# kiliant/zklaim

Hardware: AMD Instinct MI355X
Metric: Groth16 proofs/sec (zklaim gadget, alt_bn128) + G1 MSM GB/s vs HBM roofline (higher is better)
Workload: dtype u32 limbs, Montgomery (254-bit Fq/Fr: 9 x 29-bit in the accumulation, reduction and NTT kernels, 8 x 32-bit elsewhere)

## Files before the change

include/zkg.h:

```cpp
#ifndef ZKG_H
#define ZKG_H

#include <stddef.h>
#include <stdint.h>

#ifdef __cplusplus
extern "C" {
#endif

#define ZKG_OK 0
#define ZKG_ERROR 1
#define ZKG_UNSATISFIED 2
#define ZKG_PROOF_BYTES 134

typedef struct zkg_r1cs {
    uint32_t num_variables;
    uint32_t num_inputs;
    uint32_t num_constraints;
    uint32_t reserved;
    const uint32_t *a_rowptr, *a_col; const uint64_t *a_val;
    const uint32_t *b_rowptr, *b_col; const uint64_t *b_val;
    const uint32_t *c_rowptr, *c_col; const uint64_t *c_val;
} zkg_r1cs;

typedef struct zkg_pk {
    zkg_r1cs cs;
    uint32_t log_m;
    uint32_t domain_size;
    const uint64_t *alpha_g1, *beta_g1, *delta_g1;
    const uint64_t *beta_g2, *delta_g2;
    const uint64_t *A_query;
    const uint64_t *B_g1;
    const uint64_t *B_g2;
    const uint64_t *H_query;
    const uint64_t *L_query;
} zkg_pk;

typedef struct zkg_crs zkg_crs;

int  zkg_init(int device);
void zkg_shutdown(void);
const char *zkg_last_error(void);
int  zkg_device_info(char *name, size_t name_len, int *compute_units);

int zkg_ntt(uint64_t *a, unsigned logN, int inverse, int coset);
int zkg_ntt_dev(void *d_a, unsigned logN, int inverse, int coset, void *stream);

int zkg_evaluation_domain_size(size_t min_size, size_t *m, int *is_step);
int zkg_ntt_domain(uint64_t *a, size_t m, int inverse, int coset);
int zkg_ntt_domain_dev(void *d_a, size_t m, int inverse, int coset, void *stream);

typedef struct zkg_domain zkg_domain;
zkg_domain *zkg_domain_new(size_t m);
void   zkg_domain_free(zkg_domain *d);
size_t zkg_domain_size(const zkg_domain *d);
size_t zkg_domain_batch_max(const zkg_domain *d);
void   zkg_domain_set_batch_max(zkg_domain *d, size_t k);
int zkg_domain_ntt_async(zkg_domain *d, void *d_a, size_t stride , size_t count,
                         int inverse, int coset, void *stream);
int zkg_domain_lagrange_async(zkg_domain *d, const uint64_t t[4], void *d_u, void *d_z, void *stream);
void zkg_domain_stats(size_t out[3]);

typedef struct zkg_qap zkg_qap;
zkg_qap *zkg_qap_new(const zkg_r1cs *cs);
void     zkg_qap_free(zkg_qap *q);
size_t   zkg_qap_domain_size(const zkg_qap *q);
uint32_t zkg_qap_num_variables(const zkg_qap *q);
size_t   zkg_qap_batch_max(const zkg_qap *q);
void     zkg_qap_set_batch_max(zkg_qap *q, size_t k);
int      zkg_qap_witness_h_async(zkg_qap *q, const void *d_witnesses, size_t stride , size_t count,
                                 void *d_h, size_t h_stride , uint32_t *d_unsat ,
                                 void *stream);
void     zkg_qap_stats(size_t out[3]);
int      zkg_qap_instance_async(zkg_qap *q, const uint64_t t[4] , void *d_abc ,
                                size_t stride , void *d_z , void *stream);
void     zkg_qap_set_column_segment(zkg_qap *q, size_t k);
void     zkg_qap_instance_stats(size_t out[2]);

int zkg_msm_g1(const uint64_t *bases, const uint64_t *scalars, size_t n, uint64_t out_jac[12]);
int zkg_msm_g2(const uint64_t *bases, const uint64_t *scalars, size_t n, uint64_t out_jac[24]);
#define ZKG_SCALARS_MONT 1
#define ZKG_SCALARS_MOSTLY_BITS 2
int zkg_msm_g1_dev(const void *d_bases, const void *d_scalars, size_t n, int scalars_mont,
                   uint64_t out_jac[12], void *stream);
int zkg_msm_g2_dev(const void *d_bases, const void *d_scalars, size_t n, int scalars_mont,
                   uint64_t out_jac[24], void *stream);
int zkg_msm_g1_host_scalars(const void *d_bases, const uint64_t *scalars, size_t n, int scalars_mont, uint64_t out_jac[12], void *stream);
typedef struct zkg_msm_bases zkg_msm_bases;
zkg_msm_bases *zkg_msm_g1_bases_upload(const void *d_bases, size_t n);
int zkg_msm_g1_resident(zkg_msm_bases *bases, const void *d_scalars, size_t n, int scalars_mont, uint64_t out_jac[12], void *stream);
void zkg_msm_g1_bases_free(zkg_msm_bases *bases);
int zkg_msm_g1_resident_async(zkg_msm_bases *bases, const void *d_scalars, size_t n, size_t stride , size_t count,
                              int scalars_mont, void *d_out_jac , void *stream);
size_t zkg_msm_g1_resident_batch_max(const zkg_msm_bases *bases);
void zkg_msm_resident_async_stats(size_t out[3]);
int zkg_msm_combine_gpu(const uint64_t *records_jac, size_t cpw, int slots , int chunk_log, size_t vectors, uint64_t *out_jac);
typedef struct zkg_msm_g2_bases zkg_msm_g2_bases;
zkg_msm_g2_bases *zkg_msm_g2_bases_upload(const void *d_bases , size_t n);
void   zkg_msm_g2_bases_free(zkg_msm_g2_bases *bases);
int    zkg_msm_g2_resident(zkg_msm_g2_bases *bases, const void *d_scalars, size_t n, int scalars_mont, uint64_t out_jac[24], void *stream);
int    zkg_msm_g2_resident_async(zkg_msm_g2_bases *bases, const void *d_scalars, size_t n, size_t stride, size_t count,
                                 int scalars_mont, void *d_out_jac , void *stream);
size_t zkg_msm_g2_resident_batch_max(const zkg_msm_g2_bases *bases);
int    zkg_msm_combine_g2_gpu(const uint64_t *records_jac, size_t cpw, int chunk_log, size_t vectors, uint64_t *out_jac);
int zkg_msm_g1_windows_dev(const void *d_bases, const void *d_scalars, size_t n, int scalars_mont,
                           unsigned first_window, unsigned window_stride, uint64_t out_jac[12], void *stream);
int zkg_g1_sum(const uint64_t *points_jac, size_t count, uint64_t out_jac[12]);
int zkg_g2_sum(const uint64_t *points_jac, size_t count, uint64_t out_jac[24]);

typedef struct zkg_msm_shards zkg_msm_shards;
int zkg_init_multi(const int *devices, int ndev);
zkg_msm_shards *zkg_msm_g1_shards_upload(const uint64_t *bases, size_t n, const int *devices, int ndev);
void zkg_msm_g1_shards_free(zkg_msm_shards *shards);
size_t zkg_msm_g1_shards_count(const zkg_msm_shards *shards, size_t *points);
int zkg_msm_g1_multi(const zkg_msm_shards *shards, const uint64_t *scalars, uint64_t out_jac[12], uint64_t *partials_jac);
unsigned zkg_multi_rccl_calls(void);

int zkg_g1_fixed_base_dev(const uint64_t base[8], const void *d_scalars, size_t n, void *d_out_affine, void *stream);
int zkg_g2_fixed_base_dev(const uint64_t base[16], const void *d_scalars, size_t n, void *d_out_affine, void *stream);

zkg_crs *zkg_crs_upload(const zkg_pk *pk);
zkg_crs *zkg_crs_upload_blob(const void *pk_blob, size_t len);
int zkg_pk_blob_inspect(const void *pk_blob, size_t len, uint64_t out[8]);
void     zkg_crs_free(zkg_crs *crs);
int zkg_crs_shard_h(zkg_crs *crs, const int *devices, int ndev);
uint32_t zkg_crs_num_variables(const zkg_crs *crs);

int zkg_groth16_prove(const zkg_crs *crs, const uint64_t *witness, const uint64_t r[4],
                      const uint64_t s[4], int check_satisfied, uint8_t *proof_out, size_t *proof_len);
int zkg_groth16_prove_sparse(const zkg_crs *crs, const uint8_t *tags, const uint32_t *full_index, const uint64_t *full_values, size_t count,
                             const uint64_t r[4], const uint64_t s[4], int check_satisfied, uint8_t *proof_out, size_t *proof_len);
typedef struct zkg_prove_item {
    const uint64_t *witness;
    const uint8_t  *tags; const uint32_t *full_index; const uint64_t *full_values; size_t count;
    const uint64_t *r, *s;
} zkg_prove_item;
int zkg_groth16_prove_batch(const zkg_crs *crs, const zkg_prove_item *items, size_t count, int check_satisfied,
                            uint8_t *proofs_out , int *status );
void zkg_prove_batch_stats(size_t out[3]);
size_t zkg_prove_batch_chunk(const zkg_crs *crs);
int zkg_groth16_prove_dev(const zkg_crs *crs, const void *d_witness, const uint64_t r[4], const uint64_t s[4], int check_satisfied,
                          uint8_t *proof_out, size_t *proof_len, void *stream);
int zkg_groth16_prove_batch_dev(const zkg_crs *crs, const void *d_witnesses, size_t stride , size_t count,
                                const uint64_t *rs , int check_satisfied,
                                uint8_t *proofs_out , int *status , void *stream);
void zkg_prove_dev_stats(size_t out[2]);
struct zklaim_ctx;
int zkg_groth16_prove_batch_zklaim(const zkg_crs *crs, const struct zklaim_ctx *const *ctxs, size_t count, const uint64_t *rs ,
                                   int check_satisfied, uint8_t *proofs_out , int *status );
void zkg_zklaim_witness_stats(size_t out[2]);
size_t zkg_zklaim_witness_size(size_t payloads, size_t *cap_listed);
int zkg_zklaim_witness_gpu(const struct zklaim_ctx *const *ctxs, size_t count, uint8_t *tags_out , uint32_t *index_out,
                           uint64_t *values_out, size_t cap_listed , size_t *listed_counts);
int zkg_zklaim_witness_mirror(const struct zklaim_ctx *ctx, uint8_t *tags_out , uint32_t *index_out, uint64_t *values_out, size_t cap_listed,
                              size_t *listed_count);
int zkg_groth16_prove_zklaim(const zkg_crs *crs, const struct zklaim_ctx *ctx, const uint64_t r[4], const uint64_t s[4],
                             int check_satisfied, uint8_t *proof_out, size_t *proof_len);
void zkg_prove_zklaim_stats(size_t out[2]);
int zkg_zklaim_witness_gpu_parallel(const struct zklaim_ctx *const *ctxs, size_t count, uint8_t *tags_out , uint32_t *index_out,
                                    uint64_t *values_out, size_t cap_listed , size_t *listed_counts);
int zkg_zklaim_witness_mirror_parallel(const struct zklaim_ctx *ctx, uint8_t *tags_out , uint32_t *index_out, uint64_t *values_out,
                                       size_t cap_listed, size_t *listed_count);
int zkg_qap_witness_h(const zkg_crs *crs, const uint64_t *witness, uint64_t *h_out);
int zkg_prove_stage_ms(const zkg_crs *crs, float ms[8]);
int zkg_prover_peak_in_flight(int reset);

struct zklaim_ctx;
typedef struct zkg_circuit zkg_circuit;
#define ZKG_CIRCUIT_WITH_WITNESS 1
#define ZKG_CIRCUIT_REFERENCE_QUIRK 2
zkg_circuit *zkg_zklaim_circuit_new(const struct zklaim_ctx *ctx, int flags);
zkg_circuit *zkg_zklaim_witness_new(const struct zklaim_ctx *ctx);
uint32_t zkg_circuit_num_variables(const zkg_circuit *c);
void zkg_circuit_free(zkg_circuit *c);
int zkg_circuit_r1cs(const zkg_circuit *c, zkg_r1cs *out);
const uint64_t *zkg_circuit_witness(const zkg_circuit *c);
int zkg_circuit_sparse_witness(const zkg_circuit *c, const uint8_t **tags, const uint32_t **full_index, const uint64_t **full_values, size_t *count);
int zkg_circuit_is_satisfied(const zkg_circuit *c);
long zkg_circuit_first_unsatisfied(const zkg_circuit *c);
size_t zkg_zklaim_input_map(const struct zklaim_ctx *ctx, uint64_t *out, size_t cap_elems);

typedef struct zkg_keypair zkg_keypair;
zkg_keypair *zkg_groth16_setup(const zkg_r1cs *cs, const uint64_t *trapdoor);
zkg_keypair *zkg_groth16_setup_dev(const zkg_r1cs *cs, const uint64_t *trapdoor );
void zkg_keypair_free(zkg_keypair *kp);
const zkg_pk *zkg_keypair_pk(const zkg_keypair *kp);
int zkg_keypair_swapped(const zkg_keypair *kp);
size_t zkg_keypair_pk_blob(const zkg_keypair *kp, uint8_t *out, size_t cap);
size_t zkg_keypair_vk_blob(const zkg_keypair *kp, uint8_t *out, size_t cap);
int zkg_groth16_verify(const uint8_t *vk_blob, size_t vk_len, const uint64_t *primary_input, size_t n_inputs,
                       const uint8_t *proof, size_t proof_len);
int zkg_pairing_probe(const uint64_t a[4], const uint64_t b[4], uint8_t out[384]);
typedef struct zkg_verify_item {
    const uint8_t  *vk_blob;       size_t vk_len;
    const uint64_t *primary_input; size_t n_inputs;
    const uint8_t  *proof;         size_t proof_len;
} zkg_verify_item;
int zkg_groth16_verify_batch(const zkg_verify_item *items, size_t count, uint8_t *verdicts);
void zkg_verify_batch_stats(size_t out[3]);
int zkg_pairing_product(const uint64_t *g1_affine, const uint64_t *g2_affine, size_t n, uint8_t out[384]);
int  zkg_groth16_verify_each(const zkg_verify_item *items, size_t count, uint8_t *verdicts);
void zkg_verify_each_stats(size_t out[3]);
void zkg_verify_each_set_chunk(size_t positions);
int  zkg_pairing_each(const uint64_t *g1_affine, const uint64_t *g2_affine, size_t items, size_t pairs, uint8_t *out);
int  zkg_final_exp(const uint8_t *in, size_t n, int where, uint8_t *out);
int zkg_pairing_selfcheck(const uint32_t *e, int nlimbs);

int libsnark_trusted_setup(struct zklaim_ctx *ctx);
int libsnark_prove(struct zklaim_ctx *ctx);
int libsnark_verify(struct zklaim_ctx *ctx);
void zkg_compat_reset(void);
int zkg_zklaim_prove_batch(struct zklaim_ctx *const *ctxs, size_t count, int *rc);
int zkg_zklaim_verify_batch(struct zklaim_ctx *const *ctxs, size_t count, int *rc);
void zkg_zklaim_verify_batch_stats(size_t out[4]);
int zkg_proof_decode_gpu(const uint8_t *proofs, size_t count, uint64_t *A, uint64_t *B, uint64_t *C, uint8_t *ok);
int zkg_zklaim_input_sums_gpu(const struct zklaim_ctx *const *ctxs, size_t count, const uint32_t *weights, const uint8_t *mask,
                              size_t lo, size_t hi, uint64_t *sums_out, size_t cap_elems, size_t *n_elems);
size_t zkg_zklaim_input_map_mirror(const struct zklaim_ctx *ctx, uint64_t *out, size_t cap_elems);
int  zkg_zklaim_verify_each(struct zklaim_ctx *const *ctxs, size_t count, int *rc);
void zkg_zklaim_verify_each_stats(size_t out[4]);
int zkg_zklaim_ic_each(const uint64_t *ic0, const uint64_t *ic, const struct zklaim_ctx *const *ctxs, size_t count, int where, uint64_t *out);

int zkg_point_decompress(const uint8_t *records, size_t stride, size_t offset, size_t n, int g2, int where, uint64_t *out, uint32_t *flag);
int zkg_point_compress(const uint64_t *g1, const uint64_t *g2, const uint32_t *idx, size_t npoints, size_t n, int rec, int where, uint8_t *out,
                       uint8_t guard[16]);

int zkg_field_op(int field, int op, const uint64_t *a, const uint64_t *b, size_t n, uint64_t *out);

int zkg_fr29_op(int op, const uint32_t *in, size_t n, uint32_t *out);

int zkg_fq29_op(int op, const uint32_t *in, size_t n, uint32_t *out);
int zkg_fq29_op_chain(int op, int chain, const uint32_t *in, size_t n, uint32_t *out);

int zkg_fq12_op(int op, const uint32_t *a, const uint32_t *b, size_t n, int where, uint32_t *out);

int zkg_g1_add_quad29(const uint64_t *a_jac, const uint64_t *b_jac, size_t n, int chain, uint64_t *out_jac);
int zkg_g1_add_pair29(const uint64_t *a_jac, const uint64_t *b_jac, size_t n, int chain, uint64_t *out_jac);

int zkg_curve_op(int group, int op, const uint32_t *a, const uint32_t *b, const uint32_t *k, size_t n, int chain, uint32_t *out);

// ... 8 lines not shown
```

zklaim_amd/__init__.py:

```python
from .api import (ZkgError, device_info, evaluation_domain_size, fixed_base_g1_dev, fixed_base_g2_dev, g1_sum, g2_sum, init, lib, msm_g1, msm_g1_dev, msm_g1_windows_dev,
                  msm_g2, msm_g2_dev, ntt, ntt_dev, shutdown, timing_dominant_ms, timing_reset, Crs, PK, R1CS, make_r1cs, make_pk,
                  DECLARED_SYMBOLS, ZklaimCircuit, ZklaimCtx, make_ctx, zklaim_input_map, OPS, Keypair, groth16_verify, groth16_verify_batch, verify_batch_stats, groth16_prove_batch, prove_batch_stats, groth16_prove_batch_dev, prove_dev_stats, groth16_prove_batch_zklaim, zklaim_witness_stats, zklaim_witness_size, zklaim_witness_mirror, zklaim_witness_gpu, zklaim_witness_mirror_parallel, zklaim_witness_gpu_parallel, prove_zklaim_stats, pairing_product, pairing_probe, pairing_selfcheck,
                  libsnark_trusted_setup, libsnark_prove, libsnark_verify, zklaim_prove_batch, zklaim_verify_batch, zklaim_verify_batch_stats, proof_decode_gpu, zklaim_input_sums_gpu, zklaim_input_map_mirror, ctx_blob, COMPAT_SYMBOLS, field_op, fr29_op, FR29_OPS, fq29_op, FQ29_OPS, g1_add_quad29, g1_add_pair29, curve_op, CURVE_OPS, OK, ERROR, UNSATISFIED, init_multi, MsmShards, pk_blob_inspect, ResidentBases, msm_g1_host_scalars, msm_resident_async_stats, msm_combine_gpu, ResidentBasesG2, msm_combine_g2_gpu,
                  groth16_verify_each, verify_each_stats, verify_each_set_chunk, pairing_each, final_exp, fq12_op, FQ12_OPS,
                  point_decompress, point_compress, zklaim_verify_each, zklaim_verify_each_stats, zklaim_ic_each,
                  Domain, domain_stats, Qap, qap_stats, qap_instance_stats)
```

zklaim_amd/api.py:

```python
import ctypes as C
import os
import sys

import numpy as np

_HERE = os.path.dirname(os.path.abspath(__file__))
_SO = os.path.join(_HERE, "libzkg.so")

DECLARED_SYMBOLS = [
    "zkg_init", "zkg_shutdown", "zkg_last_error", "zkg_device_info", "zkg_ntt", "zkg_ntt_dev", "zkg_evaluation_domain_size", "zkg_ntt_domain", "zkg_ntt_domain_dev", "zkg_msm_g1", "zkg_msm_g2",
    "zkg_msm_g1_dev", "zkg_msm_g2_dev", "zkg_msm_g1_windows_dev", "zkg_g1_sum", "zkg_g2_sum", "zkg_g1_fixed_base_dev", "zkg_g2_fixed_base_dev",
    "zkg_groth16_prove_batch_zklaim", "zkg_zklaim_witness_stats", "zkg_zklaim_witness_size", "zkg_zklaim_witness_gpu", "zkg_zklaim_witness_mirror",
    "zkg_crs_upload", "zkg_crs_upload_blob", "zkg_pk_blob_inspect", "zkg_crs_free", "zkg_crs_num_variables", "zkg_groth16_prove", "zkg_groth16_prove_sparse", "zkg_circuit_sparse_witness", "zkg_qap_witness_h", "zkg_prove_stage_ms", "zkg_timing_reset",
    "zkg_timing_dominant_ms", "zkg_zklaim_circuit_new", "zkg_zklaim_witness_new", "zkg_circuit_num_variables", "zkg_circuit_free", "zkg_circuit_r1cs", "zkg_circuit_witness",
    "zkg_circuit_is_satisfied", "zkg_circuit_first_unsatisfied", "zkg_zklaim_input_map", "zkg_groth16_setup", "zkg_keypair_free",
    "zkg_keypair_pk", "zkg_keypair_swapped", "zkg_keypair_pk_blob", "zkg_keypair_vk_blob", "zkg_groth16_verify", "zkg_pairing_probe", "zkg_pairing_selfcheck",
    "zkg_compat_reset", "zkg_field_op", "zkg_init_multi", "zkg_msm_g1_shards_upload", "zkg_msm_g1_shards_free", "zkg_msm_g1_shards_count",
    "zkg_msm_g1_multi", "zkg_g1_add_quad29", "zkg_crs_shard_h", "zkg_msm_g1_bases_upload", "zkg_msm_g1_resident", "zkg_msm_g1_bases_free",
    "zkg_prover_peak_in_flight", "zkg_msm_g1_host_scalars", "zkg_multi_rccl_calls", "zkg_g1_add_pair29",
    "zkg_groth16_verify_batch", "zkg_pairing_product", "zkg_verify_batch_stats",
    "zkg_groth16_prove_batch", "zkg_prove_batch_stats", "zkg_prove_batch_chunk", "zkg_zklaim_prove_batch",
    "zkg_groth16_prove_zklaim", "zkg_prove_zklaim_stats", "zkg_zklaim_witness_gpu_parallel", "zkg_zklaim_witness_mirror_parallel",
    "zkg_fr29_op", "zkg_fq29_op", "zkg_fq29_op_chain",
    "zkg_zklaim_verify_batch", "zkg_zklaim_verify_batch_stats", "zkg_proof_decode_gpu", "zkg_zklaim_input_sums_gpu", "zkg_zklaim_input_map_mirror",
    "zkg_groth16_prove_dev", "zkg_groth16_prove_batch_dev", "zkg_prove_dev_stats",
    "zkg_msm_g1_resident_async", "zkg_msm_g1_resident_batch_max", "zkg_msm_resident_async_stats", "zkg_msm_combine_gpu",
    "zkg_groth16_verify_each", "zkg_verify_each_stats", "zkg_verify_each_set_chunk", "zkg_pairing_each", "zkg_final_exp",
    "zkg_fq12_op", "zkg_point_decompress", "zkg_point_compress",
    "zkg_zklaim_verify_each", "zkg_zklaim_verify_each_stats", "zkg_zklaim_ic_each",
    "zkg_curve_op",
    "zkg_domain_new", "zkg_domain_free", "zkg_domain_size", "zkg_domain_batch_max", "zkg_domain_set_batch_max", "zkg_domain_ntt_async",
    "zkg_domain_lagrange_async", "zkg_domain_stats",
    "zkg_msm_g2_bases_upload", "zkg_msm_g2_bases_free", "zkg_msm_g2_resident", "zkg_msm_g2_resident_async", "zkg_msm_g2_resident_batch_max",
    "zkg_msm_combine_g2_gpu",
    "zkg_qap_new", "zkg_qap_free", "zkg_qap_domain_size", "zkg_qap_num_variables", "zkg_qap_batch_max", "zkg_qap_set_batch_max",
    "zkg_qap_witness_h_async", "zkg_qap_stats",
    "zkg_qap_instance_async", "zkg_qap_set_column_segment", "zkg_qap_instance_stats", "zkg_groth16_setup_dev",
]
COMPAT_SYMBOLS = ["libsnark_trusted_setup", "libsnark_prove", "libsnark_verify"]


OK, ERROR, UNSATISFIED = 0, 1, 2


class ZkgError(RuntimeError):
    pass


class R1CS(C.Structure):
    _fields_ = [("num_variables", C.c_uint32), ("num_inputs", C.c_uint32), ("num_constraints", C.c_uint32), ("reserved", C.c_uint32)] + \
        [(f"{m}_{f}", C.c_void_p) for m in "abc" for f in ("rowptr", "col", "val")]


class PK(C.Structure):
    _fields_ = [("cs", R1CS), ("log_m", C.c_uint32), ("domain_size", C.c_uint32)] + \
        [(k, C.c_void_p) for k in ("alpha_g1", "beta_g1", "delta_g1", "beta_g2", "delta_g2", "A_query", "B_g1", "B_g2", "H_query", "L_query")]


_lib = None


def lib():
    global _lib
    if _lib is None:
        if not os.path.exists(_SO):
            raise ZkgError(f"{_SO} is missing: build it with `python -m zklaim_amd.build` (hipcc, gfx950)")
        if "torch" not in sys.modules and not os.environ.get("ZKG_NO_TORCH"):
            try:
                import torch
            except Exception:
                pass
        _lib = C.CDLL(_SO)
        _lib.zkg_last_error.restype = C.c_char_p
        _lib.zkg_timing_dominant_ms.restype = C.c_float
        _lib.zkg_crs_upload.restype = C.c_void_p
        _lib.zkg_crs_upload.argtypes = [C.c_void_p]
        _lib.zkg_crs_upload_blob.restype = C.c_void_p
        _lib.zkg_crs_upload_blob.argtypes = [C.c_void_p, C.c_size_t]
        _lib.zkg_crs_free.argtypes = [C.c_void_p]
    return _lib


def _check(rc, what):
    if rc != 0:
        raise ZkgError(f"{what} failed (rc={rc}): {lib().zkg_last_error().decode()}")


def _p(a):
    return None if a is None else a.ctypes.data_as(C.c_void_p)


def _u64(a):
    return np.ascontiguousarray(a, dtype=np.uint64)


def _vp(x):
    return C.c_void_p(int(x) if x else 0)


_initialised = False


def init(device=0):
    global _initialised
    _check(lib().zkg_init(int(device)), "zkg_init")
    _initialised = True


def shutdown():
    global _initialised
    if _initialised:
        lib().zkg_shutdown()
    _initialised = False


def device_info():
    name = C.create_string_buffer(128); cus = C.c_int(0)
    _check(lib().zkg_device_info(name, C.c_size_t(128), C.byref(cus)), "zkg_device_info")
    return name.value.decode(), cus.value


def field_op(field, op, a, b=None):
    a = _u64(a); limbs = 8 if field == 2 else 4
    out = np.zeros_like(a)
    bb = None if b is None else _u64(b)
    _check(lib().zkg_field_op(int(field), int(op), _p(a), _p(bb), C.c_size_t(a.size // limbs), _p(out)), "zkg_field_op")
    return out


FR29_OPS = {"mul": (0, 2, 1), "mul2": (1, 4, 2), "norm": (2, 1, 1), "add_norm": (3, 2, 1), "sub_norm": (4, 2, 1), "add_lazy": (5, 2, 1), "sub_lazy": (6, 2, 1),
            "slice": (7, 1, 1), "unslice_reduce": (8, 1, 1), "r4": (9, 7, 4), "r4_stage0": (10, 7, 4), "r4_norm_stores": (11, 7, 4),
            "r4_stage0_norm_stores": (12, 7, 4), "r2_tail": (13, 3, 2), "r2_tail_stage0": (14, 3, 2)}


def fr29_op(name, x):
    op, k, m = FR29_OPS[name]
    x = np.ascontiguousarray(x, dtype=np.uint32)
    if x.ndim != 3 or x.shape[1:] != (k, 9):
        raise ZkgError(f"fr29_op {name}: input must be (n, {k}, 9), got {x.shape}")
    out = np.zeros((x.shape[0], m, 9), np.uint32)
    _check(lib().zkg_fr29_op(int(op), _p(x), C.c_size_t(x.shape[0]), _p(out)), "zkg_fr29_op")
    return out


FQ29_OPS = {"mul": (0, 2, 1), "mul2": (1, 4, 2), "sqr": (2, 1, 1), "sqr2": (3, 2, 2), "norm": (4, 1, 1), "add": (5, 2, 1), "dbl": (6, 1, 1),
            "sub_S2_1": (7, 2, 1), "sub_S4_1": (8, 2, 1), "sub_S6_1": (9, 2, 1), "sub_S4_3": (10, 2, 1), "neg_S2_1": (11, 1, 1), "is_zero": (12, 1, 1),
            "unpack": (13, 1, 1), "to29": (14, 1, 1), "from29": (15, 1, 1), "rec64": (16, 3, 3), "bucket29": (17, 5, 4), "inverse": (18, 1, 1),
            "madd": (19, 7, 5), "add_lane": (20, 8, 4), "add_pair": (21, 8, 4), "add_quad": (22, 8, 4)}


def fq29_op(name, x, chain=0):
    op, k, m = FQ29_OPS[name]
    x = np.ascontiguousarray(x, dtype=np.uint32)
    if x.ndim != 3 or x.shape[1:] != (k, 9):
        raise ZkgError(f"fq29_op {name}: input must be (n, {k}, 9), got {x.shape}")
    out = np.zeros((x.shape[0], m, 9), np.uint32)
    _check(lib().zkg_fq29_op_chain(int(op), int(chain), _p(x), C.c_size_t(x.shape[0]), _p(out)), "zkg_fq29_op")
    return out


def g1_add_quad29(a_jac, b_jac, chain=0):
    a = _u64(a_jac); b = _u64(b_jac); out = np.zeros_like(a)
    _check(lib().zkg_g1_add_quad29(_p(a), _p(b), C.c_size_t(a.size // 12), int(chain), _p(out)), "zkg_g1_add_quad29")
    return out.reshape(-1, 12)


def g1_add_pair29(a_jac, b_jac, chain=0):
    a = _u64(a_jac); b = _u64(b_jac); out = np.zeros_like(a)
    _check(lib().zkg_g1_add_pair29(_p(a), _p(b), C.c_size_t(a.size // 12), int(chain), _p(out)), "zkg_g1_add_pair29")
    return out.reshape(-1, 12)


CURVE_OPS = {"madd": 0, "add": 1, "add_quad": 2, "dbl": 3, "dbl_affine": 4, "to_affine": 5, "mul": 6}


def curve_op(group, name, a, b=None, k=None, chain=0):
    op = CURVE_OPS[name]; w = 16 if group else 8
    a = np.ascontiguousarray(a, dtype=np.uint32)
    need_a = 2 if name == "dbl_affine" else 4
    if a.ndim != 3 or a.shape[1:] != (need_a, w):
        raise ZkgError(f"curve_op {name}: a must be (n, {need_a}, {w}), got {a.shape}")
    n = a.shape[0]
    if name in ("madd", "add", "add_quad"):
        need_b = 2 if name == "madd" else 4
        b = np.ascontiguousarray(b, dtype=np.uint32)
        if b.shape != (n, need_b, w):
            raise ZkgError(f"curve_op {name}: b must be ({n}, {need_b}, {w}), got {b.shape}")
    else:
        b = None
    if name == "mul":
# ... 66 lines not shown
        t = _u64(t).reshape(4)
        _check(lib().zkg_domain_lagrange_async(C.c_void_p(self._h), _p(t), _vp(d_u_ptr), _vp(d_z_ptr), _vp(stream)), "zkg_domain_lagrange_async")

    def batch_max(self):
        return int(lib().zkg_domain_batch_max(C.c_void_p(self._h)))

    def set_batch_max(self, k):
        lib().zkg_domain_set_batch_max(C.c_void_p(self._h), C.c_size_t(k))

    def size(self):
        return int(lib().zkg_domain_size(C.c_void_p(self._h)))

    def free(self):
        if self._h:
            lib().zkg_domain_free(C.c_void_p(self._h)); self._h = None


def domain_stats():
    out = (C.c_size_t * 3)()
    lib().zkg_domain_stats(out)
    return tuple(int(v) for v in out)


class Qap:

    def __init__(self, cs):
        L = lib()
        L.zkg_qap_new.restype = C.c_void_p
        L.zkg_qap_new.argtypes = [C.c_void_p]
        L.zkg_qap_free.argtypes = [C.c_void_p]
        for name in ("zkg_qap_domain_size", "zkg_qap_batch_max"):
            getattr(L, name).restype = C.c_size_t
            getattr(L, name).argtypes = [C.c_void_p]
        L.zkg_qap_num_variables.restype = C.c_uint32
        L.zkg_qap_num_variables.argtypes = [C.c_void_p]
        L.zkg_qap_set_batch_max.argtypes = [C.c_void_p, C.c_size_t]
        L.zkg_qap_witness_h_async.argtypes = [C.c_void_p, C.c_void_p, C.c_size_t, C.c_size_t, C.c_void_p, C.c_size_t, C.c_void_p, C.c_void_p]
        L.zkg_qap_instance_async.argtypes = [C.c_void_p, C.c_void_p, C.c_void_p, C.c_size_t, C.c_void_p, C.c_void_p]
        L.zkg_qap_set_column_segment.argtypes = [C.c_void_p, C.c_size_t]
        self._h = L.zkg_qap_new(C.byref(cs))
        if not self._h:
            raise ZkgError("zkg_qap_new failed: " + L.zkg_last_error().decode())
        self.m, self.n = self.domain_size(), self.num_variables()

    def witness_h_async(self, d_w_ptr, count, stride, d_h_ptr, h_stride, d_unsat_ptr=0, stream=0):
        _check(lib().zkg_qap_witness_h_async(C.c_void_p(self._h), _vp(d_w_ptr), C.c_size_t(stride), C.c_size_t(count), _vp(d_h_ptr), C.c_size_t(h_stride),
                                             _vp(d_unsat_ptr), _vp(stream)), "zkg_qap_witness_h_async")

    def instance_async(self, t, d_abc_ptr, stride=None, d_z_ptr=0, stream=0):
        tt = None if t is None else _u64(t).reshape(-1)
        if tt is not None and tt.size != 4:
            raise ZkgError("zkg_qap_instance_async: t is 4 limbs")
        _check(lib().zkg_qap_instance_async(C.c_void_p(self._h), _p(tt), _vp(d_abc_ptr), C.c_size_t(self.n + 1 if stride is None else stride), _vp(d_z_ptr),
                                            _vp(stream)), "zkg_qap_instance_async")

    def set_column_segment(self, k):
        lib().zkg_qap_set_column_segment(C.c_void_p(self._h), C.c_size_t(k))

    def domain_size(self):
        return int(lib().zkg_qap_domain_size(C.c_void_p(self._h)))

    def num_variables(self):
        return int(lib().zkg_qap_num_variables(C.c_void_p(self._h)))

    def batch_max(self):
        return int(lib().zkg_qap_batch_max(C.c_void_p(self._h)))

    def set_batch_max(self, k):
        lib().zkg_qap_set_batch_max(C.c_void_p(self._h), C.c_size_t(k))

    def free(self):
        if self._h:
            lib().zkg_qap_free(C.c_void_p(self._h)); self._h = None


def qap_stats():
    out = (C.c_size_t * 3)()
    lib().zkg_qap_stats(out)
    return tuple(int(v) for v in out)


def qap_instance_stats():
    out = (C.c_size_t * 2)()
    lib().zkg_qap_instance_stats(out)
    return tuple(int(v) for v in out)


def msm_g1(bases, scalars):
    bases = _u64(bases); scalars = _u64(scalars); out = np.zeros(12, np.uint64)
    _check(lib().zkg_msm_g1(_p(bases), _p(scalars), C.c_size_t(scalars.size // 4), _p(out)), "zkg_msm_g1")
    return out


def msm_g2(bases, scalars):
    bases = _u64(bases); scalars = _u64(scalars); out = np.zeros(24, np.uint64)
    _check(lib().zkg_msm_g2(_p(bases), _p(scalars), C.c_size_t(scalars.size // 4), _p(out)), "zkg_msm_g2")
    return out


def init_multi(devices):
    global _initialised
    d = (C.c_int * len(devices))(*devices)
    _check(lib().zkg_init_multi(d, len(devices)), "zkg_init_multi")
    _initialised = True


class MsmShards:

    def __init__(self, bases, devices):
        bases = _u64(bases)
        L = lib()
        L.zkg_msm_g1_shards_upload.restype = C.c_void_p
        L.zkg_msm_g1_shards_upload.argtypes = [C.c_void_p, C.c_size_t, C.c_void_p, C.c_int]
        L.zkg_msm_g1_shards_free.argtypes = [C.c_void_p]
        L.zkg_msm_g1_multi.argtypes = [C.c_void_p, C.c_void_p, C.c_void_p, C.c_void_p]
        d = (C.c_int * len(devices))(*devices)
        self.n = bases.size // 8; self.ndev = len(devices)
        self._h = L.zkg_msm_g1_shards_upload(_p(bases), self.n, d, len(devices))
        if not self._h:
            raise ZkgError("zkg_msm_g1_shards_upload failed: " + L.zkg_last_error().decode())

    def msm(self, scalars, with_partials=False):
        scalars = _u64(scalars); out = np.zeros(12, np.uint64); parts = np.zeros((self.ndev, 12), np.uint64)
        assert scalars.size // 4 == self.n
        _check(lib().zkg_msm_g1_multi(C.c_void_p(self._h), _p(scalars), _p(out), _p(parts)), "zkg_msm_g1_multi")
        return (out, parts) if with_partials else out

    def free(self):
        if self._h:
            lib().zkg_msm_g1_shards_free(C.c_void_p(self._h)); self._h = None

    def __del__(self):
        try:
            self.free()
        except Exception:
            pass


SCALARS_MONT, SCALARS_MOSTLY_BITS = 1, 2


def msm_g1_dev(d_bases, d_scalars, n, scalars_mont=False, stream=0, mostly_bits=False):
    out = np.zeros(12, np.uint64)
    flags = (SCALARS_MONT if scalars_mont else 0) | (SCALARS_MOSTLY_BITS if mostly_bits else 0)
    _check(lib().zkg_msm_g1_dev(_vp(d_bases), _vp(d_scalars), C.c_size_t(n), flags, _p(out), _vp(stream)), "zkg_msm_g1_dev")
    return out


def msm_g1_host_scalars(d_bases, scalars_host_ptr, n, scalars_mont=False, stream=0):
    out = np.zeros(12, np.uint64)
    lib().zkg_msm_g1_host_scalars.argtypes = [C.c_void_p, C.c_void_p, C.c_size_t, C.c_int, C.c_void_p, C.c_void_p]
    _check(lib().zkg_msm_g1_host_scalars(_vp(d_bases), _vp(scalars_host_ptr), C.c_size_t(n), SCALARS_MONT if scalars_mont else 0, _p(out), _vp(stream)), "zkg_msm_g1_host_scalars")
    return out


class _ResidentBases:
    _PREFIX = None
    _LIMBS = 0

    def _fn(self, suffix, argtypes, restype=C.c_int):
        fn = getattr(lib(), self._PREFIX + suffix)
        fn.argtypes = argtypes; fn.restype = restype
        return fn

    def __init__(self, d_bases, n):
        self._h = self._fn("_bases_upload", [C.c_void_p, C.c_size_t], C.c_void_p)(_vp(d_bases), C.c_size_t(n))
        if not self._h:
            raise ZkgError(self._PREFIX + "_bases_upload failed: " + last_error())
        self.n = n

    def msm(self, d_scalars, scalars_mont=False, stream=0):
        out = np.zeros(self._LIMBS, np.uint64)
        fn = self._fn("_resident", [C.c_void_p, C.c_void_p, C.c_size_t, C.c_int, C.c_void_p, C.c_void_p])
        _check(fn(C.c_void_p(self._h), _vp(d_scalars), C.c_size_t(self.n), SCALARS_MONT if scalars_mont else 0, _p(out), _vp(stream)), self._PREFIX + "_resident")
        return out

    def msm_async(self, d_scalars_ptr, d_out_ptr, count=1, stride=None, scalars_mont=False, stream=0):
        fn = self._fn("_resident_async", [C.c_void_p, C.c_void_p, C.c_size_t, C.c_size_t, C.c_size_t, C.c_int, C.c_void_p, C.c_void_p])
        _check(fn(C.c_void_p(self._h), _vp(d_scalars_ptr), C.c_size_t(self.n), C.c_size_t(self.n if stride is None else stride),
                  C.c_size_t(count), SCALARS_MONT if scalars_mont else 0, _vp(d_out_ptr), _vp(stream)), self._PREFIX + "_resident_async")

    def batch_max(self):
        return int(self._fn("_resident_batch_max", [C.c_void_p], C.c_size_t)(C.c_void_p(self._h)))

    def free(self):
        if self._h:
            self._fn("_bases_free", [C.c_void_p], None)(C.c_void_p(self._h)); self._h = None


class ResidentBases(_ResidentBases):
    _PREFIX = "zkg_msm_g1"
    _LIMBS = 12


class ResidentBasesG2(_ResidentBases):
    _PREFIX = "zkg_msm_g2"
    _LIMBS = 24


def msm_resident_async_stats():
    out = (C.c_size_t * 3)()
    lib().zkg_msm_resident_async_stats(out)
    return tuple(int(v) for v in out)


def _msm_combine(name, limbs, records_jac, cpw, slots, chunk_log, vectors, slot_args):
    rec = _u64(records_jac)
    if rec.size != vectors * cpw * slots * limbs:
        raise ZkgError("%s: records_jac must hold vectors x cpw x %s points of %d limbs" % (name, "slots" if slot_args else slots, limbs))
    out = np.zeros((vectors, limbs), np.uint64)
    fn = getattr(lib(), "zkg_" + name)
    fn.argtypes = [C.c_void_p, C.c_size_t] + [C.c_int] * len(slot_args) + [C.c_int, C.c_size_t, C.c_void_p]
    _check(fn(_p(rec), C.c_size_t(cpw), *slot_args, int(chunk_log), C.c_size_t(vectors), _p(out)), "zkg_" + name)
    return out


def msm_combine_gpu(records_jac, cpw, slots, chunk_log, vectors=1):
    return _msm_combine("msm_combine_gpu", 12, records_jac, cpw, slots, chunk_log, vectors, [int(slots)])


def msm_combine_g2_gpu(records_jac, cpw, chunk_log, vectors=1):
    return _msm_combine("msm_combine_g2_gpu", 24, records_jac, cpw, 2, chunk_log, vectors, [])


def msm_g1_windows_dev(d_bases, d_scalars, n, first_window, window_stride, scalars_mont=False, stream=0):
    out = np.zeros(12, np.uint64)
    _check(lib().zkg_msm_g1_windows_dev(_vp(d_bases), _vp(d_scalars), C.c_size_t(n), int(scalars_mont), C.c_uint(first_window), C.c_uint(window_stride),
                                        _p(out), _vp(stream)), "zkg_msm_g1_windows_dev")
    return out


def msm_g2_dev(d_bases, d_scalars, n, scalars_mont=False, stream=0, mostly_bits=False):
    out = np.zeros(24, np.uint64)
    flags = (SCALARS_MONT if scalars_mont else 0) | (SCALARS_MOSTLY_BITS if mostly_bits else 0)
    _check(lib().zkg_msm_g2_dev(_vp(d_bases), _vp(d_scalars), C.c_size_t(n), flags, _p(out), _vp(stream)), "zkg_msm_g2_dev")
    return out


def g1_sum(points_jac):
    pts = _u64(points_jac); out = np.zeros(12, np.uint64)
    _check(lib().zkg_g1_sum(_p(pts), C.c_size_t(pts.size // 12), _p(out)), "zkg_g1_sum")
    return out


def g2_sum(points_jac):
    pts = _u64(points_jac); out = np.zeros(24, np.uint64)
    _check(lib().zkg_g2_sum(_p(pts), C.c_size_t(pts.size // 24), _p(out)), "zkg_g2_sum")
    return out


def fixed_base_g1_dev(base, d_scalars, n, d_out, stream=0):
    base = _u64(base)
    _check(lib().zkg_g1_fixed_base_dev(_p(base), _vp(d_scalars), C.c_size_t(n), _vp(d_out), _vp(stream)), "zkg_g1_fixed_base_dev")


def fixed_base_g2_dev(base, d_scalars, n, d_out, stream=0):
    base = _u64(base)
    _check(lib().zkg_g2_fixed_base_dev(_p(base), _vp(d_scalars), C.c_size_t(n), _vp(d_out), _vp(stream)), "zkg_g2_fixed_base_dev")


def timing_reset():
    lib().zkg_timing_reset()


def timing_dominant_ms():
    n = C.c_int(0)
    ms = lib().zkg_timing_dominant_ms(C.byref(n))
    return float(ms), n.value


def make_r1cs(n, l, A, B, Cm, keep):
    cs = R1CS()
    cs.num_variables, cs.num_inputs, cs.num_constraints = n, l, len(A[0]) - 1
    for name, (rp, col, val) in zip("abc", (A, B, Cm)):
        rp = np.ascontiguousarray(rp, np.uint32); col = np.ascontiguousarray(col, np.uint32); val = _u64(val)
        keep += [rp, col, val]
        setattr(cs, f"{name}_rowptr", rp.ctypes.data); setattr(cs, f"{name}_col", col.ctypes.data); setattr(cs, f"{name}_val", val.ctypes.data)
    return cs


def make_pk(cs, arrays, log_m, keep, domain_size=0):
    pk = PK(); pk.cs = cs; pk.log_m = log_m; pk.domain_size = domain_size
    for k in ("alpha_g1", "beta_g1", "delta_g1", "beta_g2", "delta_g2", "A_query", "B_g1", "B_g2", "H_query", "L_query"):
        a = _u64(arrays[k]); keep.append(a)
        setattr(pk, k, a.ctypes.data)
    return pk


class Crs:

    def __init__(self, pk=None, blob=None, m=None):
        if blob is not None:
            buf = (C.c_ubyte * len(blob)).from_buffer_copy(blob)
            self._h = lib().zkg_crs_upload_blob(C.cast(buf, C.c_void_p), C.c_size_t(len(blob)))
            self.m = m
        else:
            self._h = lib().zkg_crs_upload(C.byref(pk))
            self.m = pk.domain_size or (1 << pk.log_m)
        if not self._h:
            raise ZkgError("zkg_crs_upload failed: " + lib().zkg_last_error().decode())

    def prove(self, witness, r, s, check_satisfied=True):
        out = np.zeros(256, np.uint8); ln = C.c_size_t(0)
        rc = lib().zkg_groth16_prove(C.c_void_p(self._h), _p(_u64(witness)), _p(_u64(r)), _p(_u64(s)), int(check_satisfied), _p(out), C.byref(ln))
        if rc not in (OK, UNSATISFIED):
            _check(rc, "zkg_groth16_prove")
# ... 664 lines not shown
```

zklaim_amd/csrc/capi.hip:

```cpp
#include "common.hpp"
#include "fq29.hip.hpp"
#include "fr29.hip.hpp"
#include "../../include/zkg.h"
#include <atomic>
#include <condition_variable>
#include <cstring>
#include <memory>
#include <mutex>
#include <thread>
#include <dlfcn.h>
#include <rccl/rccl.h>

namespace zk {

static thread_local std::string t_error;
static std::string g_error;
static std::mutex g_err_mu;
void set_error(const std::string &msg) { t_error = msg; std::lock_guard<std::mutex> lk(g_err_mu); g_error = msg; }
bool hip_ok(hipError_t e, const char *what, const char *file, int line) {
    if (e == hipSuccess) return true;
    set_error(std::string(what) + ": " + hipGetErrorString(e) + " at " + file + ":" + std::to_string(line));
    return false;
}

// ... 583 lines not shown
        zkg_ntt_dev(buf.p, logN, inverse, coset, nullptr) == ZKG_OK &&
        hip_ok(hipDeviceSynchronize(), "sync", __FILE__, __LINE__) &&
        hip_ok(hipMemcpy(a, buf.p, bytes, hipMemcpyDeviceToHost), "D2H", __FILE__, __LINE__)) rc = ZKG_OK;
    buf.release();
    return rc;
}

int zkg_evaluation_domain_size(size_t min_size, size_t *m, int *is_step) {
    DomainShape sh;
    if (!evaluation_domain_shape(min_size, sh)) { set_error("zkg_evaluation_domain_size: no radix-2 or step domain for that size"); return ZKG_ERROR; }
    if (m) *m = sh.m;
    if (is_step) *is_step = sh.step ? 1 : 0;
    return ZKG_OK;
}
int zkg_ntt_domain_dev(void *d_a, size_t m, int inverse, int coset, void *stream) {
    REQUIRE_INIT();
    DomainShape sh;
    if (!domain_shape_of(m, sh)) { set_error("zkg_ntt_domain: m is neither 2^k nor 2^a + 2^b (get_evaluation_domain would not return it)"); return ZKG_ERROR; }
    if (!sh.step) return zkg_ntt_dev(d_a, sh.log_m, inverse, coset, stream);
    hipStream_t s = (hipStream_t)stream;
    StepDomain *d = step_domain(m, s);
    if (!d) return ZKG_ERROR;
    DevBuf scratch;
    if (scratch.reserve(m * NTT_SCRATCH_BYTES)) return ZKG_ERROR;
    int rc = step_ntt_run(d, (Fr *)d_a, inverse != 0, coset != 0, s, scratch.as<Fr>());
    if (!hip_ok(hipStreamSynchronize(s), "sync", __FILE__, __LINE__)) rc = ZKG_ERROR;
    scratch.release();
    return rc;
}
int zkg_ntt_domain(uint64_t *a, size_t m, int inverse, int coset) {
    REQUIRE_INIT();
    if (!a || m < 2) { set_error("zkg_ntt_domain: bad argument"); return ZKG_ERROR; }
    std::lock_guard<std::mutex> lk(g_host_ntt_mu);
    size_t bytes = m * 32;
    DevBuf buf;
    if (buf.reserve(bytes)) return ZKG_ERROR;
    int rc = ZKG_ERROR;
    if (hip_ok(hipMemcpy(buf.p, a, bytes, hipMemcpyHostToDevice), "H2D", __FILE__, __LINE__) &&
        zkg_ntt_domain_dev(buf.p, m, inverse, coset, nullptr) == ZKG_OK &&
        hip_ok(hipDeviceSynchronize(), "sync", __FILE__, __LINE__) &&
        hip_ok(hipMemcpy(a, buf.p, bytes, hipMemcpyDeviceToHost), "D2H", __FILE__, __LINE__)) rc = ZKG_OK;
    buf.release();
    return rc;
}

static constexpr size_t DOMAIN_WORKSPACE_CAP = (size_t)1 << 30;
static constexpr size_t DOMAIN_MAX_GROUP = 65535;
struct zkg_domain {
    DomainShape sh; int device = 0; std::mutex mu;
    DevBuf scratch;
    HandleOrder order;
    size_t bmax_default = 1, bmax = 1;
};
static thread_local size_t t_domain_stats[3];
static zkg_domain *domain_new_impl(size_t m) {
    if (g_device < 0) { set_error("zkg_init not called"); return nullptr; }
    DomainShape sh;
    if (m < 2 || !domain_shape_of(m, sh)) { set_error("zkg_domain_new: m is neither 2^k (k <= 28) nor 2^a + 2^b (get_evaluation_domain would not return it)"); return nullptr; }
    if (wrong_device_refused("zkg_domain_new", g_device, "zkg_init selected (the domain tables live there)")) return nullptr;
    std::unique_ptr<zkg_domain> d(new zkg_domain());
    d->sh = sh; d->device = g_device;
    d->bmax_default = d->bmax = std::max<size_t>(1, std::min(DOMAIN_MAX_GROUP, DOMAIN_WORKSPACE_CAP / (m * NTT_SCRATCH_BYTES)));
    const bool tables = sh.step ? step_domain(m, nullptr) != nullptr : ntt_domain(sh.log_m, nullptr) != nullptr;
    if (!tables || !hip_ok(hipStreamSynchronize(nullptr), "hipStreamSynchronize", __FILE__, __LINE__) || d->order.create()) return nullptr;
    return d.release();
}
static int domain_ntt_async_impl(zkg_domain *d, void *d_a, size_t stride, size_t count, int inverse, int coset, void *stream) {
    static const char *who = "zkg_domain_ntt_async";
    for (size_t &v : t_domain_stats) v = 0;
    if (count == 0) return ZKG_OK;
    REQUIRE_INIT();
    if (!d || !d_a) { set_error(std::string(who) + ": bad argument (null handle or pointer)"); return ZKG_ERROR; }
    const size_t m = d->sh.m;
    if (async_vectors_refused(who, m, "m", stride, count, d->device, "the handle was made on") ||
        dev_range_refused(d_a, ((count - 1) * stride + m) * 32, 16, d->device, who, "d_a", "handle")) return ZKG_ERROR;
    hipStream_t s = (hipStream_t)stream;
    std::lock_guard<std::mutex> lk(d->mu);
    NttDomain *nd = nullptr; StepDomain *sd = nullptr;
    if (d->sh.step) sd = step_domain(m, s); else nd = ntt_domain(d->sh.log_m, s);
    if (!nd && !sd) return ZKG_ERROR;
    size_t waits = 0, groups = 0, done = 0;
    const size_t need = std::min(d->bmax, count) * m * NTT_SCRATCH_BYTES;
    if (d->order.grow(d->scratch, need, waits) || d->order.order_behind(s)) return ZKG_ERROR;
    Fr *a = (Fr *)d_a;
    int rc = ZKG_OK;
    while (done < count && rc == ZKG_OK) {
        const size_t g = std::min(d->bmax, count - done);
        Fr *ag = a + done * stride;
        const hipEvent_t ev = done + g == count ? d->order.ev : nullptr;
        rc = sd ? step_ntt_run(sd, ag, inverse != 0, coset != 0, s, d->scratch.as<Fr>(), (unsigned)g, stride, m, ev)
                : ntt_run(nd, ag, inverse, coset, s, d->scratch.as<Fr>(), (unsigned)g, stride, m, ev);
        if (rc == ZKG_OK) { done += g; ++groups; }
    }
    t_domain_stats[0] = done; t_domain_stats[1] = groups; t_domain_stats[2] = waits;
    if (rc == ZKG_OK) { d->order.carried(s); return ZKG_OK; }
    d->order.record(s);
    return ZKG_ERROR;
}
static int domain_lagrange_async_impl(zkg_domain *d, const uint64_t t[4], void *d_u, void *d_z, void *stream) {
    static const char *who = "zkg_domain_lagrange_async";
    REQUIRE_INIT();
    if (!d || !t || !d_u) { set_error(std::string(who) + ": bad argument (null handle or pointer)"); return ZKG_ERROR; }
    if (wrong_device_refused(who, d->device, "the handle was made on") || dev_range_refused(d_u, d->sh.m * 32, 16, d->device, who, "d_u", "handle") ||
        (d_z && dev_range_refused(d_z, 32, 16, d->device, who, "d_z", "handle"))) return ZKG_ERROR;
    Fr tf; memcpy(tf.v, t, 32);
    hipStream_t s = (hipStream_t)stream;
    std::lock_guard<std::mutex> lk(d->mu);
    if (d->order.order_behind(s) || domain_lagrange_dev(d->sh, tf, (Fr *)d_u, (Fr *)d_z, s, d->order.ev)) return ZKG_ERROR;
    d->order.carried(s);
    return ZKG_OK;
}
zkg_domain *zkg_domain_new(size_t m) { return c_boundary<zkg_domain *>("zkg_domain_new", nullptr, [&] { return domain_new_impl(m); }); }
void zkg_domain_free(zkg_domain *d) {
    if (!d) return;
    c_boundary("zkg_domain_free", 0, [&] {
        int cur = 0; (void)hipGetDevice(&cur);
        if (cur != d->device) (void)hipSetDevice(d->device);
        d->order.destroy();
        d->scratch.release();
        if (cur != d->device) (void)hipSetDevice(cur);
        delete d;
        return 0;
    });
}
size_t zkg_domain_size(const zkg_domain *d) { return d ? d->sh.m : 0; }
size_t zkg_domain_batch_max(const zkg_domain *d) { return d ? d->bmax : 0; }
void zkg_domain_set_batch_max(zkg_domain *d, size_t k) {
    if (!d) return;
    c_boundary("zkg_domain_set_batch_max", 0, [&] { std::lock_guard<std::mutex> lk(d->mu); d->bmax = clamp_batch_max(k, d->bmax_default); return 0; });
}
int zkg_domain_ntt_async(zkg_domain *d, void *d_a, size_t stride, size_t count, int inverse, int coset, void *stream) {
    return c_boundary("zkg_domain_ntt_async", ZKG_ERROR, [&] { return domain_ntt_async_impl(d, d_a, stride, count, inverse, coset, stream); });
}
int zkg_domain_lagrange_async(zkg_domain *d, const uint64_t t[4], void *d_u, void *d_z, void *stream) {
    return c_boundary("zkg_domain_lagrange_async", ZKG_ERROR, [&] { return domain_lagrange_async_impl(d, t, d_u, d_z, stream); });
}
void zkg_domain_stats(size_t out[3]) { if (out) for (int i = 0; i < 3; ++i) out[i] = t_domain_stats[i]; }

int zkg_msm_g1_dev(const void *d_bases, const void *d_scalars, size_t n, int scalars_mont, uint64_t out_jac[12], void *stream) {
    REQUIRE_INIT();
    G1 r;
    if (msm_g1((const G1Affine *)d_bases, (const uint32_t *)d_scalars, n, (scalars_mont & ZKG_SCALARS_MONT) != 0, &r, (hipStream_t)stream, (scalars_mont & ZKG_SCALARS_MOSTLY_BITS) != 0)) return ZKG_ERROR;
    store_norm(out_jac, r);
    return ZKG_OK;
}
int zkg_msm_g1_host_scalars(const void *d_bases, const uint64_t *scalars, size_t n, int scalars_mont, uint64_t out_jac[12], void *stream) {
    REQUIRE_INIT();
    if (!out_jac || (n && (!d_bases || !scalars))) { set_error("zkg_msm_g1_host_scalars: bad argument"); return ZKG_ERROR; }
    G1 r;
    if (msm_g1_host_scalars((const G1Affine *)d_bases, (const uint32_t *)scalars, n, (scalars_mont & ZKG_SCALARS_MONT) != 0, &r, (hipStream_t)stream)) return ZKG_ERROR;
    store_norm(out_jac, r);
    return ZKG_OK;
}
int zkg_msm_g1_windows_dev(const void *d_bases, const void *d_scalars, size_t n, int scalars_mont, unsigned first_window, unsigned window_stride,
                           uint64_t out_jac[12], void *stream) {
    REQUIRE_INIT();
    if (!window_stride) { set_error("zkg_msm_g1_windows_dev: window_stride must be positive"); return ZKG_ERROR; }
    G1 r; const G1Affine *b = (const G1Affine *)d_bases;
    if (msm_shared(&b, 1, nullptr, (const uint32_t *)d_scalars, n, (scalars_mont & ZKG_SCALARS_MONT) != 0, &r, nullptr, (hipStream_t)stream, first_window, window_stride,
                   (scalars_mont & ZKG_SCALARS_MOSTLY_BITS) != 0)) return ZKG_ERROR;
    store_norm(out_jac, r);
    return ZKG_OK;
}
struct MsmResident { WindowTable table; MsmJob *job = nullptr; std::mutex mu; int device = 0; hipEvent_t ev_in = nullptr, ev_out = nullptr; };
struct zkg_msm_bases : MsmResident {};
struct zkg_msm_g2_bases : MsmResident {};
struct MsmResidentG1 { using Handle = zkg_msm_bases; using Point = G1; static constexpr bool g2 = false; static constexpr size_t limbs = 12; static constexpr unsigned n_log = 27; static constexpr const char *prefix = "zkg_msm_g1"; };
struct MsmResidentG2 { using Handle = zkg_msm_g2_bases; using Point = G2; static constexpr bool g2 = true; static constexpr size_t limbs = 24; static constexpr unsigned n_log = 25; static constexpr const char *prefix = "zkg_msm_g2"; };
static constexpr size_t G2_RESIDENT_BUCKET_CAP = (size_t)1 << 30;

extern "C++" {
static void resident_free(MsmResident *h) {
    int cur = 0; (void)hipGetDevice(&cur);
    if (cur != h->device) (void)hipSetDevice(h->device);
    if (h->job) { (void)hipStreamSynchronize(msm_job_stream(h->job)); msm_job_destroy(h->job); }
    if (h->ev_in) (void)hipEventDestroy(h->ev_in);
    if (h->ev_out) (void)hipEventDestroy(h->ev_out);
    h->table.release();
    if (cur != h->device) (void)hipSetDevice(cur);
}
template <class G> static typename G::Handle *resident_upload(const void *d_bases, size_t n) {
    const std::string who = std::string(G::prefix) + "_bases_upload";
    if (g_device < 0) { set_error("zkg_init not called"); return nullptr; }
    if (!d_bases || n == 0 || n >= ((size_t)1 << G::n_log)) { set_error(who + ": bad argument (1 <= n < 2^" + std::to_string(G::n_log) + ")"); return nullptr; }
    typename G::Handle *h = new (std::nothrow) typename G::Handle();
    if (!h) { set_error(who + ": out of memory"); return nullptr; }
    (void)hipGetDevice(&h->device);
    h->job = msm_job_create(nullptr, true);
    bool ok = h->job != nullptr && hip_ok(hipEventCreateWithFlags(&h->ev_in, hipEventDisableTiming), "hipEventCreate", __FILE__, __LINE__) &&
              hip_ok(hipEventCreateWithFlags(&h->ev_out, hipEventDisableTiming), "hipEventCreate", __FILE__, __LINE__);
    if constexpr (G::g2) ok = ok && window_table_build_g2(h->table, (const G2Affine *)d_bases, n, table_window_bits(n), nullptr) == 0;
    else ok = ok && window_table_build_g1(h->table, (const G1Affine *)d_bases, n, table_window_bits(n), nullptr) == 0 && window_table_records29(h->table, nullptr) == 0;
    if (!ok || !hip_ok(hipDeviceSynchronize(), "sync", __FILE__, __LINE__)) { resident_free(h); delete h; return nullptr; }
    msm_job_set_window(h->job, h->table.c);
    if constexpr (!G::g2) msm_job_set_row_merge(h->job, n >= 49152 ? 2u : 1u);
    return h;
}
static MsmBases resident_table_set(const MsmResident *h) { MsmBases b; b.p = h->table.buf.p; b.g2 = h->table.g2; b.level_stride = h->table.n; b.p29 = h->table.rec29.p; return b; }
template <class G> static int resident_sync(MsmResident *h, const void *d_scalars, size_t n, int scalars_mont, uint64_t *out_jac, void *stream) {
    const std::string who = std::string(G::prefix) + "_resident";
    REQUIRE_INIT();
    if (!h || !d_scalars || !out_jac || n != h->table.n) { set_error(who + ": bad argument (n must be the handle's point count)"); return ZKG_ERROR; }
    if (wrong_device_refused(who.c_str(), h->device, "the bases were uploaded on")) return ZKG_ERROR;
    std::lock_guard<std::mutex> lk(h->mu);
    ZK_HIP(hipEventRecord(h->ev_in, (hipStream_t)stream));
    ZK_HIP(hipStreamWaitEvent(msm_job_stream(h->job), h->ev_in, 0));
    const MsmBases b = resident_table_set(h);
    typename G::Point r;
    msm_job_set_device_finish(h->job, false);
    int rc;
    {
        ReserveGuard guard(msm_job_stream(h->job));
        rc = msm_job_launch(h->job, &b, 1, (const uint32_t *)d_scalars, n, (scalars_mont & ZKG_SCALARS_MONT) != 0, nullptr);
    }
    if constexpr (G::g2) rc = rc || msm_job_finish(h->job, nullptr, &r); else rc = rc || msm_job_finish(h->job, &r, nullptr);
    if (rc) return ZKG_ERROR;
    store_norm(out_jac, r);
    return ZKG_OK;
}
static thread_local size_t t_resident_async_stats[3];
template <class G> static size_t resident_batch_max(const MsmResident *h) {
    size_t p = MSM_MULTI_MAX_VECTORS;
    if constexpr (G::g2) p = std::min<size_t>(p, std::max<size_t>(1, G2_RESIDENT_BUCKET_CAP / msm_table_bucket_bytes(h->table.c, true)));
    while (p > 1 && !msm_multi_supported(h->table.n, h->table.c, (uint32_t)p)) --p;
    return p;
}
template <class G> static int resident_async(MsmResident *h, const void *d_scalars, size_t n, size_t stride, size_t count, int scalars_mont, void *d_out_jac, void *stream) {
    const std::string who_s = std::string(G::prefix) + "_resident_async"; const char *who = who_s.c_str();
    for (size_t &v : t_resident_async_stats) v = 0;
    if (count == 0) return ZKG_OK;
    REQUIRE_INIT();
    if (!h || !d_scalars || !d_out_jac || n != h->table.n) { set_error(who_s + ": bad argument (n must be the handle's point count)"); return ZKG_ERROR; }
    if (async_vectors_refused(who, n, "n", stride, count, h->device, "the bases were uploaded on")) return ZKG_ERROR;
    if (dev_range_refused(d_scalars, ((count - 1) * stride + n) * 32, 16, h->device, who, "d_scalars", "handle") ||
        dev_range_refused(d_out_jac, count * G::limbs * 8, 8, h->device, who, "d_out_jac", "handle")) return ZKG_ERROR;
    const size_t bmax = resident_batch_max<G>(h);
    const bool mont = (scalars_mont & ZKG_SCALARS_MONT) != 0;
    const uint32_t *sc = (const uint32_t *)d_scalars; uint64_t *out = (uint64_t *)d_out_jac;
    std::lock_guard<std::mutex> lk(h->mu);
    hipStream_t js = msm_job_stream(h->job);
    ZK_HIP(hipEventRecord(h->ev_in, (hipStream_t)stream));
    ZK_HIP(hipStreamWaitEvent(js, h->ev_in, 0));
    const MsmBases b = resident_table_set(h);
    msm_job_set_device_finish(h->job, true);
    int rc = ZKG_OK;
    size_t groups = 0, waits = 0, done = 0;
    while (done < count && rc == ZKG_OK) {
        const size_t g = std::min(bmax, count - done);
        ReserveGuard guard(js);
        const uint32_t *sg = sc + done * stride * 8;
        rc = g > 1 ? msm_job_launch_multi(h->job, &b, 1, sg, n, stride * 8, (uint32_t)g, mont) : msm_job_launch(h->job, &b, 1, sg, n, mont, nullptr);
        if (rc == ZKG_OK) rc = msm_job_finish_dev(h->job, out + done * G::limbs);
        waits += guard.drains;
        if (rc == ZKG_OK) { done += g; ++groups; }
    }
    const bool ordered = hip_ok(hipEventRecord(h->ev_out, js), "hipEventRecord", __FILE__, __LINE__) &&
                         hip_ok(hipStreamWaitEvent((hipStream_t)stream, h->ev_out, 0), "hipStreamWaitEvent", __FILE__, __LINE__);
    t_resident_async_stats[0] = done; t_resident_async_stats[1] = groups; t_resident_async_stats[2] = waits;
    return rc == ZKG_OK && ordered ? ZKG_OK : ZKG_ERROR;
}
}
void zkg_msm_resident_async_stats(size_t out[3]) { if (out) for (int i = 0; i < 3; ++i) out[i] = t_resident_async_stats[i]; }
#define ZKG_RESIDENT_ENTRIES(NAME, G)                                                                                                                       \
    G::Handle *NAME##_bases_upload(const void *d_bases, size_t n) {                                                                                         \
        return c_boundary<G::Handle *>(#NAME "_bases_upload", nullptr, [&] { return resident_upload<G>(d_bases, n); });                                    \
    }                                                                                                                                                       \
    void NAME##_bases_free(G::Handle *h) {                                                                                                                  \
        if (h) c_boundary(#NAME "_bases_free", 0, [&] { resident_free(h); delete h; return 0; });                                                           \
    }                                                                                                                                                       \
    int NAME##_resident(G::Handle *h, const void *d_scalars, size_t n, int scalars_mont, uint64_t *out_jac, void *stream) {                                \
        return c_boundary(#NAME "_resident", ZKG_ERROR, [&] { return resident_sync<G>(h, d_scalars, n, scalars_mont, out_jac, stream); });                  \
    }                                                                                                                                                       \
    int NAME##_resident_async(G::Handle *h, const void *d_scalars, size_t n, size_t stride, size_t count, int scalars_mont, void *d_out_jac, void *stream) { \
        return c_boundary(#NAME "_resident_async", ZKG_ERROR, [&] { return resident_async<G>(h, d_scalars, n, stride, count, scalars_mont, d_out_jac, stream); }); \
    }                                                                                                                                                       \
    size_t NAME##_resident_batch_max(const G::Handle *h) {                                                                                                  \
        return h ? c_boundary<size_t>(#NAME "_resident_batch_max", 0, [&] { return resident_batch_max<G>(h); }) : 0;                                        \
    }
ZKG_RESIDENT_ENTRIES(zkg_msm_g1, MsmResidentG1)
ZKG_RESIDENT_ENTRIES(zkg_msm_g2, MsmResidentG2)
#undef ZKG_RESIDENT_ENTRIES
int zkg_msm_combine_gpu(const uint64_t *records_jac, size_t cpw, int slots, int chunk_log, size_t vectors, uint64_t *out_jac) {
    return c_boundary("zkg_msm_combine_gpu", ZKG_ERROR, [&]() -> int { REQUIRE_INIT(); return msm_combine_records(false, records_jac, cpw, slots, chunk_log, vectors, out_jac); });
}
int zkg_msm_combine_g2_gpu(const uint64_t *records_jac, size_t cpw, int chunk_log, size_t vectors, uint64_t *out_jac) {
    return c_boundary("zkg_msm_combine_g2_gpu", ZKG_ERROR, [&]() -> int { REQUIRE_INIT(); return msm_combine_records(true, records_jac, cpw, 2, chunk_log, vectors, out_jac); });
}
int zkg_msm_g2_dev(const void *d_bases, const void *d_scalars, size_t n, int scalars_mont, uint64_t out_jac[24], void *stream) {
    REQUIRE_INIT();
    G2 r;
    if (msm_g2((const G2Affine *)d_bases, (const uint32_t *)d_scalars, n, (scalars_mont & ZKG_SCALARS_MONT) != 0, &r, (hipStream_t)stream, (scalars_mont & ZKG_SCALARS_MOSTLY_BITS) != 0)) return ZKG_ERROR;
    store_norm(out_jac, r);
    return ZKG_OK;
}
static int msm_host(const uint64_t *bases, const uint64_t *scalars, size_t n, uint64_t *out, int g2) {
    REQUIRE_INIT();
    if (n && (!bases || !scalars)) { set_error("zkg_msm: null input"); return ZKG_ERROR; }
    size_t bb = n * (g2 ? 128 : 64), sb = n * 32;
    DevBuf db, ds;
    if (db.reserve(bb + 16) || ds.reserve(sb + 16)) return ZKG_ERROR;
    int rc = ZKG_ERROR;
    if ((!n || (hip_ok(hipMemcpy(db.p, bases, bb, hipMemcpyHostToDevice), "H2D", __FILE__, __LINE__) &&
                hip_ok(hipMemcpy(ds.p, scalars, sb, hipMemcpyHostToDevice), "H2D", __FILE__, __LINE__))))
        rc = g2 ? zkg_msm_g2_dev(db.p, ds.p, n, 0, out, nullptr) : zkg_msm_g1_dev(db.p, ds.p, n, 0, out, nullptr);
    db.release(); ds.release();
    return rc;
// ... 301 lines not shown
```

zklaim_amd/csrc/common.hpp:

```cpp
#pragma once
#include <hip/hip_runtime.h>
#include <stdint.h>
#include <stddef.h>
#include <string>
#include <vector>
#include <functional>
#include <map>
#include <mutex>
#include "curve.hip.hpp"
#include "c_boundary.hpp"

struct zklaim_ctx;

namespace zk {

bool hip_ok(hipError_t e, const char *what, const char *file, int line);
#define ZK_HIP(expr) do { if (!::zk::hip_ok((expr), #expr, __FILE__, __LINE__)) return ZKG_ERROR; } while (0)
#define ZK_HIP_V(expr) do { if (!::zk::hip_ok((expr), #expr, __FILE__, __LINE__)) return; } while (0)

struct DevBuf {
    void *p = nullptr; size_t cap = 0;
    int reserve(size_t bytes);
    void release();
    template <class T> T *as() const { return reinterpret_cast<T *>(p); }
};

struct ReserveGuard;
extern thread_local ReserveGuard *t_reserve_guard;
struct ReserveGuard {
    hipStream_t stream; size_t drains = 0; ReserveGuard *prev;
    explicit ReserveGuard(hipStream_t s) : stream(s), prev(t_reserve_guard) { t_reserve_guard = this; }
    ReserveGuard(const ReserveGuard &) = delete;
    ReserveGuard &operator=(const ReserveGuard &) = delete;
    ~ReserveGuard() { t_reserve_guard = prev; }
};

struct ScopedDevBuf : DevBuf {
    ScopedDevBuf() = default;
    ScopedDevBuf(const ScopedDevBuf &) = delete;
    ScopedDevBuf &operator=(const ScopedDevBuf &) = delete;
    ~ScopedDevBuf() { release(); }
};

struct HandleOrder {
    hipEvent_t ev = nullptr; bool pending = false; hipStream_t last = nullptr;
    int create();
    int order_behind(hipStream_t s);
    int wait_host();
    int grow(DevBuf &ws, size_t need, size_t &waits);
    void carried(hipStream_t s) { pending = true; last = s; }
    void record(hipStream_t s);
    void destroy();
};
inline size_t clamp_batch_max(size_t k, size_t dflt) { return k == 0 || k > dflt ? dflt : k; }

struct KernelTimer {
    std::vector<std::pair<hipEvent_t, hipEvent_t>> pairs; size_t used = 0; bool enabled = true, pending = false;
    size_t calls = 0, calls_seen = 0, calls_timed = 0; bool sample = true;
    void new_call();
    void begin(hipStream_t s); void end(hipStream_t s);
    float drain(int *launches);
    void reset();
};
extern KernelTimer g_dominant_timer;

void host_parallel_for(int n, const std::function<void(int)> &fn);
void host_parallel_for_wait(int n, const std::function<void(int)> &fn);
void host_parallel_for_spawn(int n, const std::function<void(int)> &fn);

struct NttDomain {
    unsigned logn = 0;
    DevBuf tw_fwd, tw_inv;
    DevBuf coset_pre;
    DevBuf icoset_post;
    DevBuf tw_fwd29, tw_inv29, coset_pre29, icoset_post29;
    DevBuf scratch;
    Fr n_inv;
    std::mutex mu; bool first_stream_set = false; hipStream_t first_stream = nullptr;
    std::map<hipStream_t, DevBuf> stream_scratch;
    Fr *scratch_for(hipStream_t s);
    int init(unsigned logn, hipStream_t s);
    void release();
};
NttDomain *ntt_domain(unsigned logn, hipStream_t s);
int ntt_run(NttDomain *d, Fr *d_a, int inverse, int coset, hipStream_t s, Fr *scratch = nullptr, unsigned batch = 1, size_t batch_stride = 0,
            size_t scratch_stride = 0, hipEvent_t done = nullptr);
static constexpr size_t NTT_SCRATCH_BYTES = 40;
int ntt_run_ex(NttDomain *d, Fr *d_a, bool inverse, const Fr *pre, const Fr *post, const Fr *post_scalar, hipStream_t s, Fr *scratch = nullptr,
               unsigned batch = 1, size_t batch_stride = 0, const void *pre29 = nullptr, const void *post29 = nullptr, size_t scratch_stride = 0, hipEvent_t done = nullptr);
int ntt_table29(DevBuf &out, const Fr *d_in, size_t n, hipStream_t s);

struct DomainShape { size_t m = 0, big = 0, small = 0; bool step = false; unsigned log_m = 0;  };
bool evaluation_domain_shape(size_t min_size, DomainShape &d);
bool domain_shape_of(size_t m, DomainShape &d);
Fr fr_root_of_unity_pow2(unsigned logn);
int domain_lagrange(const DomainShape &d, const Fr &t, std::vector<Fr> &u, Fr &Zt);
Fr domain_vanishing_at(const DomainShape &d, const Fr &t);
int domain_lagrange_dev(const DomainShape &d, const Fr &t, Fr *d_u, Fr *d_z, hipStream_t s, hipEvent_t done = nullptr);

struct StepDomain {
    DomainShape shape;
    NttDomain *dbig = nullptr, *dsmall = nullptr;
    DevBuf w;
    DevBuf winv_half;
    DevBuf g_pow, ginv_pow;
    DevBuf zinv;
    Fr zinv_small;
    Fr big_inv, small_inv, half;
    int init(const DomainShape &sh, hipStream_t s);
    void release();
};
StepDomain *step_domain(size_t m, hipStream_t s);
int step_ntt_run(StepDomain *d, Fr *d_a, bool inverse, bool coset, hipStream_t s, Fr *scratch, unsigned batch = 1, size_t batch_stride = 0,
                 size_t scratch_stride = 0, hipEvent_t done = nullptr);
int powers_table(Fr *d_out, size_t n, const Fr &base, const Fr &scale, hipStream_t s);
void ntt_release_all();
int ntt_configure();

static constexpr int MSM_MAX_SETS = 4;
struct MsmBases { const void *p = nullptr; bool g2 = false; size_t level_stride = 0; uint32_t index_sub = 0; const uint32_t *remap = nullptr; const void *p29 = nullptr; };
struct OwnedCsr { std::vector<uint32_t> rp[3], col[3]; std::vector<uint64_t> val[3]; };
struct WindowTable { DevBuf buf, rec29; size_t n = 0; int c = 0, W = 0; bool g2 = false; void release() { buf.release(); rec29.release(); n = 0; } };
int window_table_records29(WindowTable &t, hipStream_t s);
int window_table_build_g1(WindowTable &t, const G1Affine *d_bases, size_t n, int c, hipStream_t s);
int table_window_bits(size_t n);
int window_table_build_g2(WindowTable &t, const G2Affine *d_bases, size_t n, int c, hipStream_t s);
struct MsmJob;
MsmJob *msm_job_create(hipStream_t s, bool own_stream, bool high_priority = false);
hipStream_t msm_job_stream(MsmJob *j);
void msm_job_set_window_subset(MsmJob *j, uint32_t w0, uint32_t ws);
void msm_job_set_skewed(MsmJob *j, bool skewed);
void msm_job_set_row_merge(MsmJob *j, uint32_t f);
void msm_job_set_window(MsmJob *j, int c);
void msm_job_set_critical(MsmJob *j, bool critical);
static constexpr unsigned CRIT_PRIORITY_MIN_LOG = 20;
bool crit_priority_for(int part, unsigned log_m);
bool crit_priority_enabled();
void msm_job_destroy(MsmJob *j);
int msm_job_launch(MsmJob *job, const MsmBases *sets, int nsets, const uint32_t *d_scalars, size_t n, bool scalars_mont, const uint32_t *d_gather = nullptr);
int msm_job_finish(MsmJob *job, G1 *out_g1, G2 *out_g2);
bool msm_multi_supported(size_t n, int c, uint32_t count);
static constexpr uint32_t MSM_MULTI_MAX_VECTORS = 16;
static constexpr size_t ZKG_MSM_ASYNC_MAX_COUNT = (size_t)1 << 24, ZKG_MSM_ASYNC_MAX_STRIDE = (size_t)1 << 32;
int msm_job_launch_multi(MsmJob *job, const MsmBases *sets, int nsets, const uint32_t *d_scalars, size_t n, size_t scalar_stride, uint32_t count, bool scalars_mont);
int msm_job_finish_multi(MsmJob *job, G1 *out_g1, G2 *out_g2);
void msm_job_set_device_finish(MsmJob *j, bool on);
int msm_job_finish_dev(MsmJob *job, uint64_t *d_out);
int msm_combine_records(bool g2, const uint64_t *records_jac, size_t cpw, int slots, int chunk_log, size_t vectors, uint64_t *out_jac);
size_t msm_table_bucket_bytes(int c, bool g2);
static constexpr uint32_t SUBSET_NONE = 0xffffffffu;
int witness_classify(const Fr *d_z, size_t n1, uint8_t *d_tags, uint32_t *d_listed, uint32_t *d_count, hipStream_t s, const uint32_t *d_subset_pos = nullptr);
int gather_points_g1(const G1Affine *d_src, const uint32_t *d_idx, size_t count, uint32_t index_sub, G1Affine *d_out, hipStream_t s);
int gather_points_g2(const G2Affine *d_src, const uint32_t *d_idx, size_t count, uint32_t index_sub, G2Affine *d_out, hipStream_t s);
int scatter_points_g1(const G1Affine *d_src, const uint32_t *d_idx, size_t count, G1Affine *d_out, hipStream_t s);
int scatter_points_g2(const G2Affine *d_src, const uint32_t *d_idx, size_t count, G2Affine *d_out, hipStream_t s);
struct OnesSum {
    DevBuf partials; void *host = nullptr; size_t host_bytes = 0; bool g2 = false; int nsets = 0; void release();
    const G1 &g1(int i) const { return reinterpret_cast<const G1 *>(host)[i]; }
    const G2 &g2pt(int i) const { return reinterpret_cast<const G2 *>(host)[i]; }
};
int ones_sum_launch(OnesSum &o, const MsmBases *sets, int nsets, const uint8_t *d_tags, size_t n1, hipStream_t s);
int ones_sum_launch_multi(OnesSum &o, const MsmBases *sets, int nsets, const uint8_t *d_tags, size_t tag_stride, size_t n1, uint32_t count, hipStream_t s);
int msm_g1(const G1Affine *d_bases, const uint32_t *d_scalars, size_t n, bool scalars_mont, G1 *out, hipStream_t s, bool mostly_bits = false);
int msm_g2(const G2Affine *d_bases, const uint32_t *d_scalars, size_t n, bool scalars_mont, G2 *out, hipStream_t s, bool mostly_bits = false);
int msm_g1_host_scalars(const G1Affine *d_bases, const uint32_t *h_scalars, size_t n, bool scalars_mont, G1 *out, hipStream_t s);
int msm_shared(const G1Affine *const *d_g1_bases, int n_g1, const G2Affine *d_g2_bases, const uint32_t *d_scalars, size_t n,
               bool scalars_mont, G1 *out_g1, G2 *out_g2, hipStream_t s, uint32_t w0 = 0, uint32_t ws = 1,
               bool mostly_bits = false);
int fixed_base_g1(const G1Affine &base, const uint32_t *d_scalars, size_t n, G1Affine *d_out, hipStream_t s, bool scalars_mont = false);
int fixed_base_g2(const G2Affine &base, const uint32_t *d_scalars, size_t n, G2Affine *d_out, hipStream_t s, bool scalars_mont = false);
void msm_release_all();
int msm_configure();

int compress_g1_records(const G1Affine *d_in, size_t n, uint8_t *d_out, hipStream_t s);
int compress_kc_records(const G2Affine *d_g2, const G1Affine *d_g1, const uint32_t *d_idx, size_t nidx, uint8_t *d_out, hipStream_t s);

static constexpr size_t VERIFY_PROD_BLOCKS = 64;
int verify_g2_subgroup(const G2Affine *d_B, size_t n, uint8_t *d_ok, hipStream_t s);
int verify_g1_mul128(const G1Affine *d_in, const uint32_t *d_w, size_t nw, size_t n, G1Affine *d_out, hipStream_t s);
int verify_miller(const G1Affine *d_P, const G2Affine *d_Q, const uint8_t *d_use, size_t n, void *d_out, hipStream_t s);
int verify_fq12_product(const void *d_in, size_t lo, size_t hi, void *d_partial, void *d_out, hipStream_t s);
int verify_proof_decode_b(const uint8_t *d_rec, size_t n, G2Affine *d_B, uint8_t *d_dec, hipStream_t s);
int verify_proof_decode_ac(const uint8_t *d_rec, size_t n, G1Affine *d_AC, uint8_t *d_dec, hipStream_t s);
int verify_use_mask(size_t n, const uint8_t *d_in_g2, const uint8_t *d_dec_b, const uint8_t *d_dec_ac, uint8_t *d_use, hipStream_t s);
static constexpr size_t ZV_SUM_SLICES = 16;
int verify_zklaim_input_sums(const uint8_t *d_pub, uint32_t npl, size_t base, const uint32_t *d_w, const uint8_t *d_mask, size_t lo, size_t hi,
                             void *d_part, void *d_out, hipStream_t s);
size_t zklaim_bit_table_entries(uint32_t npl);
size_t zklaim_bit_table_tmp_bytes(uint32_t npl);
int verify_zklaim_bit_table(const G1Affine *d_ic, uint32_t npl, void *d_tmp, G1Affine *d_T, hipStream_t s);
int verify_zklaim_ic_each(const G1Affine *d_ic0, const G1Affine *d_T, const uint8_t *d_pub, uint32_t npl, size_t n, G1Affine *d_out,
                          const G1Affine *d_c, G1Affine *d_negc, hipStream_t s);
void zklaim_ic_each_device_code_on_host(const G1Affine &ic0, const G1Affine *ic, const uint8_t *pub, uint32_t npl, size_t n, G1Affine *out);
void verify_keys_release_all();
int initialised_device();
int dev_range_refused(const void *d, size_t bytes, size_t align, int device, const char *who, const char *what, const char *owner);
int wrong_device_refused(const char *who, int device, const char *made);
int async_vectors_refused(const char *who, size_t n, const char *n_name, size_t stride, size_t count, int device, const char *made);
int verify_ic_each(const G1Affine *d_ic0, const G1Affine *d_ic, uint32_t nidx, const void *d_x, size_t n, G1Affine *d_out, hipStream_t s);
int verify_g2_replicate(const G2Affine *d_key2, size_t n, G2Affine *d_Q, hipStream_t s);
size_t verify_final_exp_ws_bytes(size_t n);
int verify_final_exp_check(const void *d_M, size_t n, uint32_t pairs, void *d_ws, const void *d_ab, uint8_t *d_verdict, void *d_gt, hipStream_t s);
void final_exp_device_code_on_host(const uint8_t in[384], uint8_t out[384]);
enum { FQ12_MUL = 0, FQ12_SQR, FQ12_LINE, FQ12_CSQR, FQ12_INV, FQ12_CONJ, FQ12_FROB1, FQ12_FROB2, FQ12_FROB3, FQ12_MUL_BY_V, FQ12_OPS };
int verify_fq12_op(int op, const void *d_a, const void *d_b, size_t n, void *d_out, hipStream_t s);
void fq12_op_device_code_on_host(int op, const uint32_t a[96], const uint32_t b[96], uint32_t out[96]);
struct VerifyWorkspace { DevBuf buf; hipStream_t s = nullptr, s2 = nullptr; hipEvent_t ev = nullptr, ev2 = nullptr; };
VerifyWorkspace *verify_workspace_acquire();
void verify_workspace_release(VerifyWorkspace *w);
void verify_workspace_destroy(VerifyWorkspace *w);
void verify_release_all();

struct ZwPlan { uint32_t k = 0, per = 0, n = 0, cap = 0; };
uint32_t zklaim_payload_vars_host();
bool zklaim_witness_plan(uint32_t k, ZwPlan &pl);
bool zklaim_witness_plan_for_n(size_t n, ZwPlan &pl);
size_t zklaim_witness_input_bytes(const ZwPlan &pl, uint32_t P);
void zklaim_witness_pack(const ZwPlan &pl, const struct ::zklaim_ctx *const *ctxs, uint32_t P, uint8_t *host_in, uint8_t *ok);
extern thread_local size_t t_zklaim_witness_stats[2];
extern thread_local size_t t_prove_zklaim_stats[2];
int zklaim_witness_launch(const ZwPlan &pl, uint32_t P, uint8_t *d_in, uint32_t *d_desc, Fr *d_vals, uint32_t *d_idx, uint8_t *d_tags, size_t tag_stride, hipStream_t s);
bool zklaim_witness_par_ready(const ZwPlan &pl);
size_t zklaim_witness_par_input_bytes(const ZwPlan &pl, uint32_t P);
void zklaim_witness_par_pack(const ZwPlan &pl, const struct ::zklaim_ctx *const *ctxs, uint32_t P, uint8_t *host_in, uint8_t *ok);
int zklaim_witness_par_launch(const ZwPlan &pl, uint32_t P, uint8_t *d_in, uint32_t *d_desc, Fr *d_vals, uint32_t *d_idx, uint8_t *d_tags, size_t tag_stride, hipStream_t s);
void zklaim_witness_release_all();

void store_norm(uint64_t *out, const G1 &p);
void store_norm(uint64_t *out, const G2 &p);
G1 load_norm_g1(const uint64_t *in);
G2 load_norm_g2(const uint64_t *in);

}
```

zklaim_amd/csrc/msm.hip:

```cpp
#include "common.hpp"
#include "fq29.hip.hpp"
#include "host/horner_jac.hpp"
#include "../../include/zkg.h"
#include <algorithm>
#include <chrono>
#include <cstdio>
#include <cstdlib>
#include <cstring>
#include <mutex>

#define ZK_VGPR_CAP(n) __attribute__((amdgpu_num_vgpr((n) / 2)))
static constexpr int ACC29_VGPRS = 192;

namespace zk {

static constexpr int SCALAR_BITS = 255;
template <class F> struct RedGeom { static constexpr int LANES_LOG = sizeof(F) == sizeof(Fq) ? 7 : 6, LANES = 1 << LANES_LOG, THREADS = 4 * LANES; };
static constexpr int RED_L_LOG_TINY = 0, RED_L_LOG_SMALL = 2, RED_L_LOG_LARGE = 4;
static constexpr size_t RED_SMALL_BUCKETS = (size_t)1 << 16, RED_LARGE_BUCKETS = (size_t)1 << 18;
static constexpr int MAX_C = 16;
static constexpr uint32_t HEAVY_S = 512;
static constexpr uint32_t HEAVY_T_MAX = 1024;
static constexpr uint32_t CLASS_HIST_COPIES = 8;
static constexpr int HEAVY_PART_BLOCKS = 512, HEAVY_MERGE_BLOCKS = 128;
// ... 346 lines not shown
    const bool vec = (n & 3) == 0;
    auto elem = [&](uint32_t j) -> size_t { return vec ? lo + 4 * (size_t)t + (size_t)(j >> 2) * (4 * T) + (j & 3) : lo + t + (size_t)j * T; };
    if (vec) {
#pragma unroll
        for (uint32_t j = 0; j < RX_PER_THREAD; j += 4) {
            const size_t i = elem(j);
            uint4 q = make_uint4(0, 0, 0, 0);
            if (i < hi) q = *reinterpret_cast<const uint4 *>(d + i);
            code[j] = q.x; code[j + 1] = q.y; code[j + 2] = q.z; code[j + 3] = q.w;
        }
    } else {
#pragma unroll
        for (uint32_t j = 0; j < RX_PER_THREAD; ++j) { const size_t i = elem(j); code[j] = i < hi ? d[i] : 0; }
    }
#pragma unroll
    for (uint32_t j = 0; j < RX_PER_THREAD; ++j) if (code[j]) atomicAdd(&c[((code[j] >> 1) - 1) >> fbits], 1u);
    __syncthreads();
    if (b0 < CB) { off[b0] = c[b0]; gb[b0] = g0; }
    if (b1 < CB) { off[b1] = c[b1]; gb[b1] = g1; }
    __syncthreads();
    for (uint32_t dd = 1; dd < CB; dd <<= 1) {
        const bool in0 = b0 < CB && b0 >= dd, in1 = b1 < CB && b1 >= dd;
        const uint32_t x0 = in0 ? off[b0 - dd] : 0, x1 = in1 ? off[b1 - dd] : 0, y0 = in0 ? gb[b0 - dd] : 0, y1 = in1 ? gb[b1 - dd] : 0;
        __syncthreads();
        if (b0 < CB) { off[b0] += x0; gb[b0] += y0; }
        if (b1 < CB) { off[b1] += x1; gb[b1] += y1; }
        __syncthreads();
    }
    if (t == 0) off[CB] = off[CB - 1];
    if (t == 0 && sl == 0 && w == 0) *grand_total = wsum[1];
    __syncthreads();
    const uint32_t wstart = wsum[0];
    if (b0 < CB) { off[b0] -= c[b0]; gb[b0] = c[b0] ? wstart + (gb[b0] - g0) + atomicAdd(&cursor[w * CB + b0], c[b0]) : 0; cur[b0] = 0; }
    if (b1 < CB) { off[b1] -= c[b1]; gb[b1] = c[b1] ? wstart + (gb[b1] - g1) + atomicAdd(&cursor[w * CB + b1], c[b1]) : 0; cur[b1] = 0; }
    __syncthreads();
    const uint32_t fmask = (1u << fbits) - 1;
#pragma unroll
    for (uint32_t j = 0; j < RX_PER_THREAD; ++j) {
        if (!code[j]) continue;
        uint32_t i = (uint32_t)elem(j), b = (code[j] >> 1) - 1, k = b >> fbits;
        uint32_t pos = off[k] + atomicAdd(&cur[k], 1u);
        stage[pos] = ((b & fmask) << (32 - fbits)) | (i << 1) | (code[j] & 1u);
    }
    __syncthreads();
    const uint32_t wave = t >> 6, lane = t & 63;
    for (uint32_t k = wave; k < CB; k += T / 64) {
        const uint32_t a = off[k], b = off[k + 1], g = gb[k];
        for (uint32_t p = a + lane; p < b; p += 64) tmp[g + (p - a)] = stage[p];
    }
}
ZK_D void rx_fine_offsets(uint32_t *cf, uint32_t *of, uint32_t FB, uint32_t t, uint32_t start, size_t gb0, uint32_t *counts, uint32_t *offsets, uint32_t *h, uint32_t heavy_t,
                          uint32_t *class_hist) {
    const uint32_t T = blockDim.x;
    if (t < FB) { const uint32_t c = cf[t]; of[t] = c; atomicAdd(&h[c > heavy_t ? heavy_t + 1 : c], 1u); }
    __syncthreads();
    for (uint32_t d = 1; d < FB; d <<= 1) {
        uint32_t x = (t < FB && t >= d) ? of[t - d] : 0;
        __syncthreads();
        if (t < FB) of[t] += x;
        __syncthreads();
    }
    if (t < FB) of[t] -= cf[t];
    __syncthreads();
    for (uint32_t f = t; f < FB; f += T) { counts[gb0 + f] = cf[f]; offsets[gb0 + f] = start + of[f]; }
    uint32_t *copy = class_hist + ((blockIdx.x + blockIdx.y) % CLASS_HIST_COPIES) * (HEAVY_T_MAX + 2);
    for (uint32_t i = t; i < heavy_t + 2; i += T) if (h[i]) atomicAdd(&copy[i], h[i]);
}
ZK_D void rx_fine_big_bin(const uint32_t *tmp, uint32_t fbits, uint32_t start, uint32_t cnt, size_t gb0, uint32_t *cf, uint32_t *of, uint32_t *cur, uint32_t *counts,
                          uint32_t *offsets, uint32_t *sorted, uint32_t *h, uint32_t heavy_t, uint32_t *class_hist) {
    const uint32_t FB = 1u << fbits, sh = 32 - fbits, low = (1u << sh) - 1, t = threadIdx.x, T = blockDim.x;
    const bool giant = cnt > 8 * RX_FINE_MAX;
    if (!giant) {
        for (uint32_t p = t; p < cnt; p += T) atomicAdd(&cf[tmp[start + p] >> sh], 1u);
    } else
    for (uint32_t p0 = 0; p0 < cnt; p0 += T) {
        uint32_t p = p0 + t; bool live = p < cnt; uint32_t f = live ? tmp[start + p] >> sh : 0;
        while (__any(live)) {
            uint32_t lf = __shfl(f, __ffsll((long long)__ballot(live)) - 1, 64);
            unsigned long long same = __ballot(live && f == lf);
            if (live && f == lf) { if ((same & ((1ull << (threadIdx.x & 63)) - 1)) == 0) atomicAdd(&cf[lf], (uint32_t)__popcll(same)); live = false; }
        }
    }
    __syncthreads();
    rx_fine_offsets(cf, of, FB, t, start, gb0, counts, offsets, h, heavy_t, class_hist);
    if (!giant) {
        for (uint32_t p = t; p < cnt; p += T) { uint32_t e = tmp[start + p], f = e >> sh; sorted[start + of[f] + atomicAdd(&cur[f], 1u)] = e & low; }
        return;
    }
    for (uint32_t p0 = 0; p0 < cnt; p0 += T) {
        uint32_t p = p0 + t; bool live = p < cnt; uint32_t e = live ? tmp[start + p] : 0, f = e >> sh;
        while (__any(live)) {
            uint32_t lf = __shfl(f, __ffsll((long long)__ballot(live)) - 1, 64);
            unsigned long long same = __ballot(live && f == lf), below = same & ((1ull << (threadIdx.x & 63)) - 1);
            uint32_t basepos = 0;
            if (live && f == lf && below == 0) basepos = atomicAdd(&cur[lf], (uint32_t)__popcll(same));
            basepos = __shfl(basepos, __ffsll((long long)same) - 1, 64);
            if (live && f == lf) { sorted[start + of[lf] + basepos + (uint32_t)__popcll(below)] = e & low; live = false; }
        }
    }
}
template <int T>
__global__ __launch_bounds__(T) void k_rx_fine(const uint32_t *tmp, uint32_t fbits, uint32_t cbits, uint32_t B, const uint32_t *bin_cnt, const uint32_t *wtot, uint32_t *counts,
                                                uint32_t *offsets, size_t total, uint32_t *class_hist, uint32_t *sorted) {
    sort_wave_priority();
    extern __shared__ uint32_t lds_u32[];
    const uint32_t FB = 1u << fbits, sh = 32 - fbits, low = (1u << sh) - 1;
    uint32_t *bufB = lds_u32, *cf = bufB + RX_FINE_MAX, *of = cf + FB, *cur = of + FB, *h = bufB, *before = h + HEAVY_T_MAX + 2;
    const uint32_t cb = blockIdx.x, w = blockIdx.y, t = threadIdx.x, bin = (w << cbits) + cb;
    const size_t gb0 = (size_t)w * B + (size_t)cb * FB;
    for (uint32_t f = t; f < FB; f += T) { cf[f] = 0; cur[f] = 0; }
    for (uint32_t i = t; i < HEAVY_T_MAX + 2; i += T) h[i] = 0;
    if (t == 0) { before[0] = 0; before[1] = heavy_threshold_dev(offsets, total, 1); }
    __syncthreads();
    {
        const uint32_t v = wave_sum(rx_entries_before(bin_cnt, wtot, w, cb, cbits));
        if ((t & 63) == 0 && v) atomicAdd(&before[0], v);
    }
    __syncthreads();
    const uint32_t start = before[0], heavy_t = before[1], cnt = bin_cnt[bin];
    if (cnt > RX_FINE_MAX) { rx_fine_big_bin(tmp, fbits, start, cnt, gb0, cf, of, cur, counts, offsets, sorted, h, heavy_t, class_hist); return; }
    uint32_t ent[RX_FINE_MAX / T];
#pragma unroll
    for (uint32_t j = 0; j < RX_FINE_MAX / T; ++j) {
        uint32_t p = t + j * T;
        ent[j] = p < cnt ? tmp[start + p] : 0xffffffffu;
        if (p < cnt) atomicAdd(&cf[ent[j] >> sh], 1u);
    }
    __syncthreads();
    rx_fine_offsets(cf, of, FB, t, start, gb0, counts, offsets, h, heavy_t, class_hist);
    __syncthreads();
#pragma unroll
    for (uint32_t j = 0; j < RX_FINE_MAX / T; ++j) {
        if (t + j * T >= cnt) continue;
        uint32_t e = ent[j], f = e >> sh;
        bufB[of[f] + atomicAdd(&cur[f], 1u)] = e & low;
    }
    __syncthreads();
    for (uint32_t p = t; p < cnt; p += T) sorted[start + p] = bufB[p];
}

__global__ __launch_bounds__(1024) void k_class_hist(const uint32_t *counts, const uint32_t *offsets, size_t total, uint32_t *class_hist) {
    sort_wave_priority();
    __shared__ uint32_t h[HEAVY_T_MAX + 2];
    const uint32_t heavy_t = heavy_threshold_dev(offsets, total, 1);
    const uint32_t t = threadIdx.x, nc = heavy_t + 2;
    for (uint32_t i = t; i < nc; i += 1024) h[i] = 0;
    __syncthreads();
    size_t gb = (size_t)blockIdx.x * 1024 + t;
    if (gb < total) { uint32_t c = counts[gb]; atomicAdd(&h[c > heavy_t ? heavy_t + 1 : c], 1u); }
    __syncthreads();
    for (uint32_t i = t; i < nc; i += 1024) if (h[i]) atomicAdd(&class_hist[i], h[i]);
}
__global__ __launch_bounds__(1024) void k_order_place(const uint32_t *counts, const uint32_t *offsets, size_t total, const uint32_t *class_hist, uint32_t *class_cursor,
                                                       uint32_t *order) {
    sort_wave_priority();
    __shared__ uint32_t h[HEAVY_T_MAX + 2], first[HEAVY_T_MAX + 2], wave_total[16], threshold;
    const uint32_t t = threadIdx.x, wave = t >> 6, lane = t & 63;
    for (uint32_t i = t; i < HEAVY_T_MAX + 2; i += 1024) h[i] = 0;
    if (t == 0) threshold = heavy_threshold_dev(offsets, total, 1);
    __syncthreads();
    const uint32_t heavy_t = threshold, nc = heavy_t + 2;
    size_t gb = (size_t)blockIdx.x * 1024 + t;
    uint32_t cls = 0, rank = 0;
    if (gb < total) { uint32_t c = counts[gb]; cls = c > heavy_t ? heavy_t + 1 : c; rank = atomicAdd(&h[cls], 1u); }
    uint32_t v0 = 0, v1 = 0, incl = 0;
    if (128 * wave < nc) {
        for (uint32_t k = 0; k < CLASS_HIST_COPIES; ++k) {
            const uint32_t *copy = class_hist + k * (HEAVY_T_MAX + 2);
            if (2 * t < nc) v0 += copy[nc - 1 - 2 * t];
            if (2 * t + 1 < nc) v1 += copy[nc - 2 - 2 * t];
        }
        incl = v0 + v1;
        for (uint32_t d = 1; d < 64; d <<= 1) { const uint32_t y = __shfl_up(incl, d, 64); if (lane >= d) incl += y; }
    }
    if (lane == 63) wave_total[wave] = incl;
    __syncthreads();
    if (128 * wave < nc) {
        uint32_t before = incl - v0 - v1;
        for (uint32_t k = 0; k < wave; ++k) before += wave_total[k];
        if (2 * t < nc) first[nc - 1 - 2 * t] = before;
        if (2 * t + 1 < nc) first[nc - 2 - 2 * t] = before + v0;
    }
    __syncthreads();
    for (uint32_t i = t; i < nc; i += 1024) if (h[i]) h[i] = first[i] + atomicAdd(&class_cursor[i], h[i]);
    __syncthreads();
    if (gb < total) order[h[cls] + rank] = (uint32_t)gb;
}

template <class F, bool PLAIN>
__global__ __launch_bounds__(256) void k_bucket_accum(const ViewSet<F> views, const uint32_t *sorted, const uint32_t *offsets, const uint32_t *order,
                                                       size_t lanes , XYZZ<F> *buckets, HeavyItem *items,
                                                       HeavyBucket *heavy, uint32_t *counters , SetLayout L) {
    size_t tid = (size_t)blockIdx.x * blockDim.x + threadIdx.x;
    if (tid >= lanes) return;
    const size_t total_buckets = L.buckets;
    const uint32_t set = blockIdx.y;
    const BaseView<F> bases = views.v[set];
    buckets += set * L.buckets; items += set * L.items; heavy += set * L.heavy; counters += 2 * set;
    const uint32_t heavy_t = heavy_threshold_dev(offsets, total_buckets, sizeof(F) > sizeof(Fq) ? 3 : 1);
    const uint32_t gb = order[tid];
    uint32_t k = offsets[gb], end = offsets[gb + 1];
    if (end - k > heavy_t) {
        uint32_t nparts = (end - k + HEAVY_S - 1) / HEAVY_S;
        uint32_t first = atomicAdd(&counters[0], nparts);
        for (uint32_t p = 0; p < nparts; ++p) { uint32_t a = k + p * HEAVY_S; items[first + p] = {a, a + HEAVY_S < end ? a + HEAVY_S : end, gb, nparts == 1}; }
        if (nparts > 1) heavy[atomicAdd(&counters[1], 1u)] = {gb, first, nparts};
        return;
    }
    XYZZ<F> acc = XYZZ<F>::inf();
    if (k < end) {
        uint32_t e = sorted[k], e_next = k + 1 < end ? sorted[k + 1] : 0;
        Affine<F> p = bases.template load<PLAIN>(e, gb);
        while (true) {
            Affine<F> cur = p; uint32_t ce = e;
            ++k;
            if (k < end) { e = e_next; p = bases.template load<PLAIN>(e, gb); if (k + 1 < end) e_next = sorted[k + 1]; }
            if (ce & 1u) cur.y = cur.y.neg();
            acc.madd(cur);
            if (k >= end) break;
        }
    }
    buckets[gb] = acc.normalized();
}

__global__ __launch_bounds__(256) void k_bases_to29(const Affine<Fq> *in, size_t n, Rec64 *out) {
    size_t i = (size_t)blockIdx.x * blockDim.x + threadIdx.x;
    if (i >= n) return;
    const Affine<Fq> a = in[i];
    store_rec64(out + i, f29::to29(a.x), f29::to29(a.y), a.is_inf());
}
ZK_D Affine29 load29(const Rec64 *bases, uint32_t e) { return load_rec64(bases + (e >> 1)); }
ZK_D Rec64 load29_raw(const Rec64 *bases, uint32_t e) { return load_rec64_raw(bases + (e >> 1)); }
template <int WAVES, bool OUT29>
__global__ __launch_bounds__(256, WAVES) ZK_VGPR_CAP(ACC29_VGPRS) void k_bucket_accum29(const Rec64 *bases, size_t level_stride, uint32_t B, const uint32_t *sorted, const uint32_t *offsets, const uint32_t *order,
                                                         size_t lanes, void *buckets_, HeavyItem *items, HeavyBucket *heavy, uint32_t *counters, SetLayout L, int flags ) {
    crit_wave_priority(flags & 2);
    const int resume = flags & 1;
    size_t tid = (size_t)blockIdx.x * blockDim.x + threadIdx.x;
    if (tid >= lanes) return;
    const uint32_t heavy_t = heavy_threshold_dev(offsets, L.buckets, 1);
    const uint32_t gb = order[tid];
    if (level_stride) bases += (size_t)(gb / B) * level_stride;
    uint32_t k = offsets[gb], end = offsets[gb + 1];
    if (end - k > heavy_t) {
        uint32_t nparts = (end - k + HEAVY_S - 1) / HEAVY_S;
        uint32_t first = atomicAdd(&counters[0], nparts);
        const bool single = nparts == 1 && !resume;
        for (uint32_t p = 0; p < nparts; ++p) { uint32_t a = k + p * HEAVY_S; items[first + p] = {a, a + HEAVY_S < end ? a + HEAVY_S : end, gb, single}; }
        if (!single) heavy[atomicAdd(&counters[1], 1u)] = {gb, first, nparts};
        return;
    }
    XYZZ29 acc; bool inf = true;
    acc.x = acc.y = acc.zz = acc.zzz = Fq29::zero();
    if constexpr (OUT29) {
        if (resume) {
            if (k >= end) return;
            const Bucket29 old = load_bucket29_raw(reinterpret_cast<const Bucket29 *>(buckets_) + gb);
            uint32_t any = 0;
#pragma unroll
            for (int j = 0; j < 9; ++j) { acc.x.v[j] = old.x[j]; acc.y.v[j] = old.y[j]; acc.zz.v[j] = old.zz[j]; acc.zzz.v[j] = old.zzz[j]; any |= old.zz[j]; }
            inf = any == 0;
        }
    }
    if (k < end) {
        uint32_t e = sorted[k], e_next = k + 1 < end ? sorted[k + 1] : 0;
        Rec64 p = load29_raw(bases, e);
        while (true) {
            const Rec64 curw = p; const uint32_t ce = e;
            ++k;
            if (k < end) { e = e_next; p = load29_raw(bases, e); if (k + 1 < end) e_next = sorted[k + 1]; }
            const Affine29 cur = unpack_rec64(curw);
            if (!cur.inf) {
                Fq29 bx, by;
#pragma unroll
                for (int j = 0; j < 9; ++j) { bx.v[j] = cur.x[j]; by.v[j] = cur.y[j]; }
                if (ce & 1u) by = f29::neg(f29::S2_1, by);
                if (__builtin_expect(!acc.madd(bx, by, inf), 0)) {
                    XYZZ<Fq> a32 = {f29::from29(acc.x), f29::from29(acc.y), f29::from29(acc.zz), f29::from29(acc.zzz)};
                    a32.madd(Affine<Fq>{f29::from29(bx), f29::from29(f29::norm(by))});
                    if (a32.is_inf()) inf = true;
                    else { acc.x = f29::to29(a32.x.normalized()); acc.y = f29::to29(a32.y.normalized()); acc.zz = f29::to29(a32.zz.normalized()); acc.zzz = f29::to29(a32.zzz.normalized()); }
                }
            }
            if (k >= end) break;
        }
    }
    if constexpr (OUT29) store_bucket29(reinterpret_cast<Bucket29 *>(buckets_) + gb, acc, inf);
    else {
        XYZZ<Fq> *buckets = reinterpret_cast<XYZZ<Fq> *>(buckets_);
        if (inf) buckets[gb] = XYZZ<Fq>::inf().normalized();
        else buckets[gb] = XYZZ<Fq>{f29::from29(acc.x), f29::from29(acc.y), f29::from29(acc.zz), f29::from29(acc.zzz)};
    }
}

template <class F> struct alignas(16) LdsPoint {
    XYZZ<F> p; uint32_t pad[4];
    ZK_D LdsPoint &operator=(const XYZZ<F> &v) { p = v; return *this; }
    ZK_D operator const XYZZ<F> &() const { return p; }
    ZK_D XYZZ<F> normalized() const { return p.normalized(); }
};

template <class F, class Barrier>
ZK_D void lds_tree_reduce(LdsPoint<F> *seg, uint32_t n, uint32_t tid, uint32_t nthreads, Barrier barrier) {
    for (uint32_t d = n / 2; d >= 1; d >>= 1) {
        if (4 * d <= nthreads) {
            uint32_t t = tid >> 2, q = tid & 3;
            if (t < d) { XYZZ<F> a = seg[t]; xyzz_add_quad(a, seg[t + d].p, q); if (q == 0) seg[t] = a; }
        } else if (tid < d) { XYZZ<F> a = seg[tid]; a.add(seg[tid + d]); seg[tid] = a; }
        barrier();
    }
}

template <class F> ZK_D void put_bucket(XYZZ<F> *buckets, uint32_t gb, const XYZZ<F> &v, int out29) {
    if constexpr (sizeof(F) == sizeof(Fq)) { if (out29) { store_bucket29(reinterpret_cast<Bucket29 *>(buckets) + gb, v); return; } }
    buckets[gb] = v;
}
template <class F>
__global__ __launch_bounds__(256) void k_heavy_parts(const ViewSet<F> views, const uint32_t *sorted, const HeavyItem *items,
                                                      const uint32_t *counters, XYZZ<F> *partials, XYZZ<F> *buckets, SetLayout L, int out29) {
    extern __shared__ unsigned char red_smem[];
    LdsPoint<F> *sh = reinterpret_cast<LdsPoint<F> *>(red_smem);
    const uint32_t set = blockIdx.y;
    const BaseView<F> bases = views.v[set];
    items += set * L.items; partials += set * L.partials; buckets += set * L.buckets;
// ... 340 lines not shown
    if constexpr (std::is_same<F, Fq>::value) return f29::from29(f29::inverse(f29::to29(x.normalized())));
    else { const Fq d = inverse_fast<Fq>(x.c0.sqr() + x.c1.sqr()); return F{x.c0 * d, (x.c1 * d).neg()}; }
}
template <class F, int K>
__global__ __launch_bounds__(256) void k_table_levels(const Affine<F> *in, Affine<F> *out, size_t n, uint32_t c, int levels) {
    size_t i = (size_t)blockIdx.x * blockDim.x + threadIdx.x;
    if (i >= n) return;
    Affine<F> a = in[i];
    if (a.is_inf()) { for (int l = 0; l < levels; ++l) out[(size_t)l * n + i] = a; return; }
    F x[K], y[K], zz[K], zzz[K];
    XYZZ<F> p = XYZZ<F>::dbl_affine_inl(a);
#pragma unroll
    for (int l = 0; l < K; ++l) {
        if (l < levels) {
            for (uint32_t k = (l == 0 ? 1u : 0u); k < c; ++k) p = p.dbl();
            x[l] = p.x; y[l] = p.y; zz[l] = p.zz; zzz[l] = p.zzz;
        } else { x[l] = F::zero(); y[l] = F::zero(); zz[l] = F::zero(); zzz[l] = F::zero(); }
    }
    F pre[K], run = F::one();
#pragma unroll
    for (int l = 0; l < K; ++l) { pre[l] = run; if (!zzz[l].is_zero()) run = run * zzz[l]; }
    F inv = inverse_fast(run);
#pragma unroll
    for (int l = K - 1; l >= 0; --l) {
        if (l >= levels) continue;
        if (zzz[l].is_zero()) { out[(size_t)l * n + i] = Affine<F>::inf(); continue; }
        F zi = inv * pre[l];
        inv = inv * zzz[l];
        F t = zi * zz[l];
        F zi2 = t.sqr();
        out[(size_t)l * n + i] = Affine<F>{x[l] * zi2, y[l] * zi}.normalized();
    }
}

__global__ __launch_bounds__(256) void k_classify(const Fr *z, size_t n1, uint8_t *tags, uint32_t *listed, uint32_t *count, const uint32_t *subset_pos) {
    size_t i = (size_t)blockIdx.x * blockDim.x + threadIdx.x;
    uint32_t tag = 0;
    if (i < n1) {
        Fr v = z[i];
        uint32_t any = 0, diff = 0;
#pragma unroll
        for (int j = 0; j < 8; ++j) { any |= v.v[j]; diff |= v.v[j] ^ FrParams::ONE[j]; }
        tag = any == 0 ? 0u : (diff == 0 ? 1u : 2u);
        tags[i] = (uint8_t)tag;
    }
    const unsigned long long mask = __ballot(tag == 2);
    if (!mask) return;
    const uint32_t lane = threadIdx.x & 63;
    uint32_t base = 0;
    if (lane == (uint32_t)(__ffsll((long long)mask) - 1)) base = atomicAdd(count, (uint32_t)__popcll(mask));
    base = __shfl(base, __ffsll((long long)mask) - 1, 64);
    if (tag == 2) {
        listed[base + (uint32_t)__popcll(mask & ((1ull << lane) - 1))] = (uint32_t)i;
        if (subset_pos && subset_pos[i] == SUBSET_NONE) count[1] = 1;
    }
}
template <class F>
__global__ __launch_bounds__(256) void k_gather_points(const Affine<F> *src, const uint32_t *idx, size_t count, uint32_t index_sub, Affine<F> *out) {
    size_t j = (size_t)blockIdx.x * blockDim.x + threadIdx.x;
    if (j >= count) return;
    const uint32_t i = idx[j];
    out[j] = i >= index_sub ? src[i - index_sub] : Affine<F>::inf();
}
template <class F>
__global__ __launch_bounds__(256) void k_scatter_points(const Affine<F> *src, const uint32_t *idx, size_t count, Affine<F> *out) {
    size_t j = (size_t)blockIdx.x * blockDim.x + threadIdx.x;
    if (j < count) out[idx[j]] = src[j];
}
template <class F>
__global__ __launch_bounds__(256) void k_ones_sum(const ViewSet<F> views, const uint8_t *tags, size_t n1, uint32_t span, XYZZ<F> *partials,
                                                   size_t tag_stride, size_t vec_stride ) {
    extern __shared__ unsigned char red_smem[];
    LdsPoint<F> *sh = reinterpret_cast<LdsPoint<F> *>(red_smem);
    uint32_t *list = reinterpret_cast<uint32_t *>(red_smem + 256 * sizeof(LdsPoint<F>));
    __shared__ uint32_t seg_count[4];
    const Affine<F> *bases = views.v[blockIdx.y].p; const uint32_t index_sub = views.v[blockIdx.y].index_sub;
    tags += (size_t)blockIdx.z * tag_stride;
    partials += (size_t)blockIdx.z * vec_stride + (size_t)blockIdx.y * (gridDim.x + 1);
    const uint32_t tid = threadIdx.x, lane = tid & 63, wv = tid >> 6, cap = span >> 2;
    const size_t first = (size_t)blockIdx.x * span + (size_t)wv * cap;
    uint32_t count = 0;
    for (uint32_t o = 0; o < cap; o += 64) {
        const size_t i = first + o + lane;
        const bool one = i < n1 && i >= index_sub && tags[i] == 1;
        const unsigned long long mask = __ballot(one);
        if (one) list[wv * cap + count + (uint32_t)__popcll(mask & ((1ull << lane) - 1))] = (uint32_t)(i - index_sub);
        count += (uint32_t)__popcll(mask);
    }
    if (lane == 0) seg_count[wv] = count;
    __syncthreads();
    const uint32_t c0 = seg_count[0], c1 = c0 + seg_count[1], c2 = c1 + seg_count[2], total = c2 + seg_count[3];
    XYZZ<F> acc = XYZZ<F>::inf();
    for (uint32_t k = tid; k < total; k += 256) {
        const uint32_t seg = (k >= c0) + (k >= c1) + (k >= c2), off = seg == 0 ? 0u : (seg == 1 ? c0 : (seg == 2 ? c1 : c2));
        acc.madd(bases[list[seg * cap + (k - off)]]);
    }
    sh[tid] = acc;
    __syncthreads();
    lds_tree_reduce<F>(sh, 256, tid, 256, [] { __syncthreads(); });
    if (tid == 0) partials[blockIdx.x] = sh[0].normalized();
}
template <class F>
__global__ __launch_bounds__(256) void k_sum_partials(XYZZ<F> *partials_all, uint32_t count, size_t vec_stride) {
    extern __shared__ unsigned char red_smem[];
    LdsPoint<F> *sh = reinterpret_cast<LdsPoint<F> *>(red_smem);
    XYZZ<F> *partials = partials_all + (size_t)blockIdx.y * vec_stride + (size_t)blockIdx.x * (count + 1), *out = partials + count;
    XYZZ<F> acc = XYZZ<F>::inf();
    for (uint32_t i = threadIdx.x; i < count; i += 256) acc.add(partials[i]);
    sh[threadIdx.x] = acc;
    __syncthreads();
    lds_tree_reduce<F>(sh, 256, threadIdx.x, 256, [] { __syncthreads(); });
    if (threadIdx.x == 0) out[0] = sh[0].normalized();
}

struct MsmGroup {
    DevBuf buckets, folded, red_out, heavy_items, heavy_buckets, heavy_counters, heavy_partials;
    DevBuf bases29;
    void *host_red = nullptr; size_t host_cap = 0; bool g2 = false, table = false; int nsets = 0;
    int out_index[MSM_MAX_SETS] = {0};
    int red_slots = 2; size_t red_stride = 0;
    uint32_t cpw = 0, red_windows = 0; size_t nred = 0; int chunk_log = 0;
    int host_reserve(size_t bytes) {
        if (bytes <= host_cap) return 0;
        if (host_red) (void)hipHostFree(host_red);
        host_red = nullptr; host_cap = 0;
        if (!hip_ok(hipHostMalloc(&host_red, bytes + 4096, hipHostMallocDefault), "hipHostMalloc", __FILE__, __LINE__)) return 1;
        host_cap = bytes + 4096;
        return 0;
    }
    void release() {
        for (DevBuf *b : {&buckets, &folded, &red_out, &heavy_items, &heavy_buckets, &heavy_counters, &heavy_partials, &bases29}) b->release();
        if (host_red) (void)hipHostFree(host_red);
        host_red = nullptr; host_cap = 0;
    }
};
struct MsmJob {
    hipStream_t stream = nullptr; bool own_stream = false;
    DevBuf digits, hist, counts, offsets, scan_sums, class_hist, order, sorted, rx_tmp, rx_meta;
    MsmGroup group[2];
    MsmGeom g{}; size_t n = 0;
    int window_hint = 0;
    uint32_t merge_hint = 1, merge = 1;
    hipStream_t aux = nullptr; hipEvent_t ev_fork = nullptr, ev_join = nullptr; bool converted_aside = false;
    bool one_pass_sort = false;
    bool resume = false, defer_reduce = false;
    bool critical = false;
    MsmJob *bucket_owner = nullptr;
    hipStream_t sort_stream = nullptr; hipEvent_t ev_sorted = nullptr, ev_acc_done = nullptr;
    uint32_t w0 = 0, ws = 1;
    bool empty = false;
    bool dev_finish = false;
    uint32_t multi = 1; size_t multi_stride = 0;
    DevBuf hs_scalars; hipStream_t copy = nullptr; hipEvent_t ev_piece[8] = {nullptr};
    std::mutex mu;
};

template <class F>
static int launch_accumulate(MsmJob *job, MsmGroup &gr, const MsmBases *sets, const uint32_t *d_gather, bool time_it) {
    const MsmGeom g = job->g; const size_t n = job->n, total_buckets = (size_t)g.W * g.B; const unsigned ns = (unsigned)gr.nsets;
    const uint32_t P = job->multi, BP = g.B * P, Wp = g.W / P;
    hipStream_t s = job->stream;
    size_t n_entries_max = n * g.W;
    const size_t max_heavy = std::min(total_buckets, n_entries_max / (sizeof(F) != sizeof(Fq) ? 4 : 8)) + 1,
                 max_items = max_heavy + n_entries_max / HEAVY_S + 1;
    typedef RedGeom<F> RG;
    gr.table = sets[0].level_stride != 0;
    gr.red_windows = gr.table ? P : g.W;
    const size_t red_buckets = (size_t)gr.red_windows * g.B;
    static const char *force_l = getenv("ZKG_RED_L_LOG");
    const int red_l_log = force_l ? atoi(force_l) : red_buckets >= RED_LARGE_BUCKETS ? RED_L_LOG_LARGE : red_buckets > RED_SMALL_BUCKETS ? RED_L_LOG_SMALL : RED_L_LOG_TINY;
    gr.chunk_log = RG::LANES_LOG + red_l_log;
    gr.cpw = (g.B + (1u << gr.chunk_log) - 1) >> gr.chunk_log; gr.nred = (size_t)gr.red_windows * gr.cpw;
    DevBuf &bucket_buf = job->bucket_owner ? job->bucket_owner->group[sizeof(F) != sizeof(Fq) ? 1 : 0].buckets : gr.buckets;
    gr.red_slots = 2;
    SetLayout L; L.buckets = total_buckets; L.items = max_items; L.heavy = max_heavy; L.partials = max_items; L.folded = BP; L.red_out = gr.nred * 3;
    if (gr.heavy_items.reserve(ns * max_items * sizeof(HeavyItem)) || gr.heavy_buckets.reserve(ns * max_heavy * sizeof(HeavyBucket)) ||
        gr.heavy_counters.reserve(8 * MSM_MAX_SETS) || gr.heavy_partials.reserve(ns * max_items * sizeof(XYZZ<F>)) ||
        bucket_buf.reserve(ns * total_buckets * std::max(sizeof(XYZZ<F>), sizeof(Bucket29))) || (job->dev_finish && gr.red_out.reserve(ns * L.red_out * sizeof(XYZZ<F>))) || ((gr.red_stride = L.red_out), false) ||
        (gr.table && gr.folded.reserve(ns * (size_t)BP * std::max(sizeof(XYZZ<F>), sizeof(Bucket29)))) || (!job->dev_finish && gr.host_reserve(ns * L.red_out * sizeof(XYZZ<F>)))) return ZKG_ERROR;
    XYZZ<F> *buckets = bucket_buf.as<XYZZ<F>>();
    ViewSet<F> views;
    for (unsigned i = 0; i < (unsigned)MSM_MAX_SETS; ++i) {
        const MsmBases &b = sets[i < ns ? i : 0];
        views.v[i] = BaseView<F>{reinterpret_cast<const Affine<F> *>(b.p), b.level_stride, d_gather, b.index_sub, BP, b.remap};
    }
    const size_t lanes = gr.table ? std::min(total_buckets, n_entries_max) : total_buckets;
    bool plain = !d_gather;
    for (unsigned i = 0; i < ns; ++i) plain = plain && sets[i].level_stride == 0 && sets[i].index_sub == 0 && !sets[i].remap;
    bool use29 = false; const Rec64 *rec29 = nullptr; size_t stride29 = 0;
    if constexpr (sizeof(F) == sizeof(Fq)) {
        if (ns == 1 && plain) {
            use29 = true;
            if (sets[0].p29) rec29 = reinterpret_cast<const Rec64 *>(sets[0].p29);
            else {
                ZK_HIP(hipStreamWaitEvent(s, job->ev_join, 0));
                rec29 = gr.bases29.as<Rec64>();
            }
        } else if (ns == 1 && !d_gather && sets[0].p29 && !sets[0].remap && sets[0].index_sub == 0) {
            use29 = true; rec29 = reinterpret_cast<const Rec64 *>(sets[0].p29); stride29 = sets[0].level_stride;
        }
    }
    const bool out29 = use29 && (stride29 == 0 ? !gr.table : (gr.table && ns == 1 && Wp <= 8));
    const int resume = job->resume ? 1 : 0;
    if (time_it) g_dominant_timer.begin(s);
    if constexpr (sizeof(F) == sizeof(Fq)) {
        static const int waves_env = getenv("ZKG_ACC29_WAVES") ? atoi(getenv("ZKG_ACC29_WAVES")) : 0;
        const int waves29 = waves_env ? waves_env : (job->sort_stream || gr.table || job->bucket_owner) ? 2 : 3;
        auto launch29 = [&](auto kern) {
            hipLaunchKernelGGL(kern, dim3((unsigned)((lanes + 255) / 256)), dim3(256), 0, s, rec29, stride29, BP, job->sorted.as<uint32_t>(),
                               job->offsets.as<uint32_t>(), job->order.as<uint32_t>(), lanes, (void *)buckets, gr.heavy_items.as<HeavyItem>(),
                               gr.heavy_buckets.as<HeavyBucket>(), gr.heavy_counters.as<uint32_t>(), L, resume | (job->critical ? 2 : 0));
        };
        if (use29 && waves29 == 3) { if (out29) launch29(k_bucket_accum29<3, true>); else launch29(k_bucket_accum29<3, false>); }
        else if (use29) { if (out29) launch29(k_bucket_accum29<2, true>); else launch29(k_bucket_accum29<2, false>); }
    }
    if (use29) {}
    else if (plain)
        hipLaunchKernelGGL((k_bucket_accum<F, true>), dim3((unsigned)((lanes + 255) / 256), ns), dim3(256), 0, s,
                           views, job->sorted.as<uint32_t>(), job->offsets.as<uint32_t>(), job->order.as<uint32_t>(), lanes, buckets,
                           gr.heavy_items.as<HeavyItem>(), gr.heavy_buckets.as<HeavyBucket>(), gr.heavy_counters.as<uint32_t>(), L);
    else
        hipLaunchKernelGGL((k_bucket_accum<F, false>), dim3((unsigned)((lanes + 255) / 256), ns), dim3(256), 0, s,
                           views, job->sorted.as<uint32_t>(), job->offsets.as<uint32_t>(), job->order.as<uint32_t>(), lanes, buckets,
                           gr.heavy_items.as<HeavyItem>(), gr.heavy_buckets.as<HeavyBucket>(), gr.heavy_counters.as<uint32_t>(), L);
    if (time_it) g_dominant_timer.end(s);
    hipLaunchKernelGGL(k_heavy_parts<F>, dim3(HEAVY_PART_BLOCKS, ns), dim3(256), 256 * sizeof(LdsPoint<F>), s,
                       views, job->sorted.as<uint32_t>(), gr.heavy_items.as<HeavyItem>(), gr.heavy_counters.as<uint32_t>(), gr.heavy_partials.as<XYZZ<F>>(), buckets, L, (int)out29);
    hipLaunchKernelGGL(k_heavy_merge<F>, dim3(HEAVY_MERGE_BLOCKS, ns), dim3(256), 256 * sizeof(LdsPoint<F>), s,
                       gr.heavy_buckets.as<HeavyBucket>(), gr.heavy_counters.as<uint32_t>(), gr.heavy_partials.as<XYZZ<F>>(), buckets, L, (int)out29, resume);
    if (job->defer_reduce) {
        if (hipGetLastError() != hipSuccess) { set_error("msm kernel launch failed"); return ZKG_ERROR; }
        return ZKG_OK;
    }
    const XYZZ<F> *red_in = buckets; size_t in_stride = L.buckets;
    XYZZ<F> *red_dst = job->dev_finish ? gr.red_out.as<XYZZ<F>>() : reinterpret_cast<XYZZ<F> *>(gr.host_red);
    bool folded29 = false;
    if constexpr (sizeof(F) == sizeof(Fq)) {
        if (gr.table && out29) {
            hipLaunchKernelGGL(k_bucket_fold29, dim3((2 * BP + 255) / 256), dim3(256), 0, s, reinterpret_cast<const Bucket29 *>(buckets), job->counts.as<uint32_t>(), Wp, BP,
                               gr.folded.as<Bucket29>(), job->critical ? 1 : 0);
            red_in = gr.folded.as<XYZZ<F>>(); in_stride = L.folded; folded29 = true;
        }
    }
    if (gr.table && !folded29) {
        uint32_t slots = 1; while (slots < Wp && slots < 32) slots <<= 1;
        uint32_t fold_b_log = 0; while ((FOLD_THREADS >> (fold_b_log + 1)) >= slots) ++fold_b_log;
        hipLaunchKernelGGL(k_bucket_fold<F>, dim3((BP + (1u << fold_b_log) - 1) >> fold_b_log, ns), dim3(FOLD_THREADS), FOLD_THREADS * sizeof(LdsPoint<F>), s,
                           buckets, job->counts.as<uint32_t>(), Wp, BP, fold_b_log, gr.folded.as<XYZZ<F>>(), L);
        red_in = gr.folded.as<XYZZ<F>>(); in_stride = L.folded;
    }
    if constexpr (sizeof(F) == sizeof(Fq)) {
        const size_t lds = 2 * RG::LANES * sizeof(LdsPoint29);
        const void *rin = red_in; XYZZ<Fq> *rout = reinterpret_cast<XYZZ<Fq> *>(red_dst);
        auto launch_red = [&](auto kern, unsigned threads) { hipLaunchKernelGGL(kern, dim3((unsigned)gr.nred, ns), dim3(threads), lds, s, rin, g.B, gr.cpw, rout, in_stride, L.red_out, job->critical ? 1 : 0); };
        if (out29 && red_l_log == RED_L_LOG_LARGE) {
            gr.red_slots = 3;
            hipLaunchKernelGGL(k_bucket_reduce29l, dim3((unsigned)gr.nred, ns), dim3(2 * RG::LANES), 4 * RG::LANES * sizeof(LdsPoint29), s,
                               reinterpret_cast<const Bucket29 *>(rin), g.B, gr.cpw, rout, in_stride, L.red_out, job->critical ? 1 : 0);
        } else if (red_l_log != RED_L_LOG_TINY) {
            if (red_l_log == RED_L_LOG_LARGE) launch_red(k_bucket_reduce29p<RED_L_LOG_LARGE, false>, 2 * RG::LANES);
            else if (out29) launch_red(k_bucket_reduce29p<RED_L_LOG_SMALL, true>, 2 * RG::LANES);
            else launch_red(k_bucket_reduce29p<RED_L_LOG_SMALL, false>, 2 * RG::LANES);
        } else {
            if (out29) launch_red(k_bucket_reduce29<RED_L_LOG_TINY, true>, RG::THREADS);
            else launch_red(k_bucket_reduce29<RED_L_LOG_TINY, false>, RG::THREADS);
        }
    } else {
        if (red_l_log == RED_L_LOG_LARGE)
            hipLaunchKernelGGL((k_bucket_reduce<F, RED_L_LOG_LARGE>), dim3((unsigned)gr.nred, ns), dim3(RG::THREADS), 2 * RG::LANES * sizeof(LdsPoint<F>), s,
                               red_in, g.B, gr.cpw, red_dst, in_stride, L.red_out);
        else if (red_l_log == RED_L_LOG_SMALL)
            hipLaunchKernelGGL((k_bucket_reduce<F, RED_L_LOG_SMALL>), dim3((unsigned)gr.nred, ns), dim3(RG::THREADS), 2 * RG::LANES * sizeof(LdsPoint<F>), s,
                               red_in, g.B, gr.cpw, red_dst, in_stride, L.red_out);
        else
            hipLaunchKernelGGL((k_bucket_reduce<F, RED_L_LOG_TINY>), dim3((unsigned)gr.nred, ns), dim3(RG::THREADS), 2 * RG::LANES * sizeof(LdsPoint<F>), s,
                               red_in, g.B, gr.cpw, red_dst, in_stride, L.red_out);
    }
    if (hipGetLastError() != hipSuccess) { set_error("msm kernel launch failed"); return ZKG_ERROR; }
    return ZKG_OK;
}

template <class F>
static XYZZ<F> host_combine(const MsmJob *job, const MsmGroup &gr, int set, int vec = 0 ) {
    const MsmGeom g = job->g; const uint32_t cpw = gr.cpw, W = gr.red_windows;
    const bool multi = gr.table && job->multi > 1;
    const XYZZ<F> *red = reinterpret_cast<const XYZZ<F> *>(gr.host_red) + (size_t)set * gr.red_stride;
    const size_t sl = (size_t)gr.red_slots;
    std::vector<XYZZ<F>> V(W);
    auto window = [&](int w) {
        XYZZ<F> Usum = XYZZ<F>::inf(), suffix = XYZZ<F>::inf(), weighted = XYZZ<F>::inf(), Asum = XYZZ<F>::inf();
        for (int ch = (int)cpw - 1; ch >= 0; --ch) {
            const XYZZ<F> &P = red[sl * ((size_t)w * cpw + ch)], &U = red[sl * ((size_t)w * cpw + ch) + 1];
            Usum.add(U);
            if (sl == 3) Asum.add(red[sl * ((size_t)w * cpw + ch) + 2]);
            if (ch >= 1) { suffix.add(P); weighted.add(suffix); }
            else suffix.add(P);
        }
        if (sl == 3 && !Asum.is_inf()) Usum.add(xyzz_times_pow2(Asum, 3));
        weighted = xyzz_times_pow2(weighted, (uint32_t)gr.chunk_log);
        Usum.add(weighted); Usum.add(suffix);
        V[w] = Usum;
    };
    if (multi) { window(vec); return V[vec]; }
    if (gr.table) {
        const int SEG = 16, nseg = ((int)cpw + SEG - 1) / SEG;
        if (nseg <= 1) { window(0); return V[0]; }
        std::vector<XYZZ<F>> Us(nseg), Ps(nseg), Wt(nseg);
        host_parallel_for(nseg, [&](int sg) {
            XYZZ<F> Usum = XYZZ<F>::inf(), suffix = XYZZ<F>::inf(), weighted = XYZZ<F>::inf();
            const int lo = sg * SEG, hi = std::min<int>((int)cpw, lo + SEG);
            for (int ch = hi - 1; ch >= lo; --ch) {
                Usum.add(red[2 * (size_t)ch + 1]);
                suffix.add(red[2 * (size_t)ch]);
                if (ch > lo) weighted.add(suffix);
            }
            Us[sg] = Usum; Ps[sg] = suffix; Wt[sg] = weighted;
        });
        XYZZ<F> Usum = XYZZ<F>::inf(), suffix = XYZZ<F>::inf(), seg_weighted = XYZZ<F>::inf(), weighted = XYZZ<F>::inf();
        for (int sg = nseg - 1; sg >= 0; --sg) { Usum.add(Us[sg]); weighted.add(Wt[sg]); suffix.add(Ps[sg]); if (sg >= 1) seg_weighted.add(suffix); }
        weighted.add(xyzz_times_pow2(seg_weighted, 4));
        weighted = xyzz_times_pow2(weighted, (uint32_t)gr.chunk_log);
        Usum.add(weighted); Usum.add(suffix);
        return Usum;
    }
    host_parallel_for((int)W, window);
    XYZZ<F> acc = XYZZ<F>::inf();
    for (int w = (int)W - 1; w >= 0; --w) {
        acc = xyzz_times_pow2(acc, g.c * g.ws);
        acc.add(V[w]);
    }
    return xyzz_times_pow2(acc, g.c * g.w0);
}

template <class F> constexpr int COMBINE_THREADS = 256;
template <> constexpr int COMBINE_THREADS<Fq2> = 128;
template <class F> constexpr int COMBINE_MAX_SLOTS = 3;
template <> constexpr int COMBINE_MAX_SLOTS<Fq2> = 2;
template <class F> constexpr int POINT_WORDS = 3 * sizeof(F) / 4;
template <class F> static __host__ __device__ uint32_t combine_lanes(uint32_t cpw) { uint32_t n = 1; while (n < cpw && n < (uint32_t)COMBINE_THREADS<F>) n <<= 1; return n; }
template <class F> static size_t combine_lds_bytes(uint32_t cpw) { return combine_lanes<F>(cpw) * sizeof(LdsPoint<F>); }
ZK_D void store_limbs(uint32_t *out, const Fq &a) { for (int i = 0; i < 8; ++i) out[i] = a.v[i]; }
ZK_D void store_limbs(uint32_t *out, const Fq2 &a) { store_limbs(out, a.c0); store_limbs(out + 8, a.c1); }
ZK_D void load_limbs(Fq &a, const uint32_t *in) { for (int i = 0; i < 8; ++i) a.v[i] = in[i]; }
ZK_D void load_limbs(Fq2 &a, const uint32_t *in) { load_limbs(a.c0, in); load_limbs(a.c1, in + 8); }
template <class F> ZK_D void store_norm_dev(uint32_t *out , const XYZZ<F> &v) {
    F X = F::zero(), Y = F::one(), Z = F::zero();
    if (!v.is_inf()) { const Affine<F> a = v.to_affine().normalized(); X = a.x; Y = a.y; Z = F::one(); }
    store_limbs(out, X); store_limbs(out + sizeof(F) / 4, Y); store_limbs(out + 2 * (sizeof(F) / 4), Z);
}
template <class F, int THREADS>
__global__ __launch_bounds__(THREADS) void k_msm_combine(const XYZZ<F> *red, uint32_t cpw, int slots, int chunk_log, size_t set_stride, uint32_t *out) {
    extern __shared__ unsigned char red_smem[];
    LdsPoint<F> *sh = reinterpret_cast<LdsPoint<F> *>(red_smem);
    const uint32_t t = threadIdx.x, w = blockIdx.x, set = blockIdx.y;
    const uint32_t n = combine_lanes<F>(cpw);
    int l_log = 0; while (((uint64_t)n << l_log) < cpw) ++l_log;
    const XYZZ<F> *rec = red + (size_t)set * set_stride + (size_t)slots * w * cpw;
    const uint64_t first = (uint64_t)t << l_log, end = first + ((uint64_t)1 << l_log) < cpw ? first + ((uint64_t)1 << l_log) : cpw;
    XYZZ<F> U = XYZZ<F>::inf(), Q = XYZZ<F>::inf(), T0 = XYZZ<F>::inf();
    {
        const bool has_a = COMBINE_MAX_SLOTS<F> == 3 && slots == 3;
        XYZZ<F> A = XYZZ<F>::inf();
        for (uint64_t ch = end; ch > first; --ch) {
            const XYZZ<F> *r = rec + (size_t)slots * (ch - 1);
            Q.add(r[0]); U.add(r[1]);
            if (has_a) A.add(r[2]);
            if (ch - 1 > first) T0.add(Q);
        }
        if (has_a) { for (int i = 0; i < 3; ++i) A = A.dbl(); U.add(A); }
    }
    for (uint32_t d = 1; d < n; d <<= 1) {
        if (t < n) sh[t] = Q;
        __syncthreads();
        if (t + d < n) Q.add(sh[t + d]);
        __syncthreads();
    }
    if (t == 0) { U.add(Q); Q = XYZZ<F>::inf(); }
    for (int i = 0; i < l_log; ++i) Q = Q.dbl();
    Q.add(T0);
    for (int i = 0; i < chunk_log; ++i) Q = Q.dbl();
    U.add(Q);
    if (t < n) sh[t] = U;
    __syncthreads();
    lds_tree_reduce<F>(sh, n, t, THREADS, [] { __syncthreads(); });
    if (t == 0) store_norm_dev<F>(out + POINT_WORDS<F> * ((size_t)w * gridDim.y + set), sh[0]);
}
template <class F> static void launch_combine(dim3 grid, hipStream_t s, const XYZZ<F> *red, uint32_t cpw, int slots, int chunk_log, size_t set_stride, uint32_t *out) {
    hipLaunchKernelGGL((k_msm_combine<F, COMBINE_THREADS<F>>), grid, dim3(COMBINE_THREADS<F>), combine_lds_bytes<F>(cpw), s, red, cpw, slots, chunk_log, set_stride, out);
}
template <class F> __global__ __launch_bounds__(64) void k_msm_store_inf(uint32_t *out, uint32_t count) {
    const uint32_t i = blockIdx.x * blockDim.x + threadIdx.x;
    if (i < count) store_norm_dev(out + POINT_WORDS<F> * (size_t)i, XYZZ<F>::inf());
}
template <class F> __global__ __launch_bounds__(256) void k_jac_to_records(const uint32_t *jac, size_t count, XYZZ<F> *rec) {
    const size_t i = (size_t)blockIdx.x * blockDim.x + threadIdx.x;
    if (i >= count) return;
    const uint32_t *in = jac + POINT_WORDS<F> * i;
    F X, Y, Z;
    load_limbs(X, in); load_limbs(Y, in + sizeof(F) / 4); load_limbs(Z, in + 2 * (sizeof(F) / 4));
    rec[i] = Z.is_zero() ? XYZZ<F>::inf() : XYZZ<F>{X, Y, F::one(), F::one()};
}

static int sort_digits(MsmJob *job, const uint32_t *d_scalars, bool mont, const uint32_t *d_gather) {
    const MsmGeom g0 = job->g; const size_t n0 = job->n;
    if (job->merge > 1) { job->g.W /= job->merge; job->g.Wt = job->g.W; job->n *= job->merge; }
    if (job->multi > 1) { job->g.W *= job->multi; job->g.Wt = job->g.W; }
    const MsmGeom g = job->g; const size_t n = job->n;
    hipStream_t s = job->sort_stream ? job->sort_stream : job->stream;
    const size_t total = (size_t)g.W * g.B;
    uint32_t slice_len = (uint32_t)std::min<size_t>(65536, std::max<size_t>(4096, ((n + 15) / 16 + 1023) / 1024 * 1024));
    uint32_t S = (uint32_t)std::max<size_t>(1, (n + slice_len - 1) / slice_len);
    size_t nblk = (total + 1024 * SCAN_ITEMS - 1) / (1024 * SCAN_ITEMS);
    if (nblk > 1024) { set_error("msm: too many buckets for the block scan"); return ZKG_ERROR; }
    if (job->digits.reserve(std::max<size_t>(1, n * g.W) * 4) || job->hist.reserve((size_t)g.W * S * g.B * 4) || job->counts.reserve(total * 4) ||
        job->offsets.reserve((total + 1) * 4) || job->scan_sums.reserve(1024 * 4) || job->class_hist.reserve((CLASS_HIST_COPIES + 1) * (HEAVY_T_MAX + 2) * 4) ||
        job->order.reserve(total * 4) || job->sorted.reserve(std::max<size_t>(1, n * g.W) * 4)) return ZKG_ERROR;
    uint32_t *digits = job->digits.as<uint32_t>(), *hist = job->hist.as<uint32_t>(), *counts = job->counts.as<uint32_t>(),
             *offsets = job->offsets.as<uint32_t>(), *sums = job->scan_sums.as<uint32_t>(), *chist = job->class_hist.as<uint32_t>();
    uint32_t cbits = 6;
    static const uint32_t bin_avg = getenv("ZKG_RX_AVG") ? (uint32_t)atoi(getenv("ZKG_RX_AVG")) : RX_BIN_AVG;
    while (cbits < RX_MAX_CBITS && cbits + 1 < g.c - 1 && (n >> cbits) > bin_avg) ++cbits;
    const bool two_pass = !job->one_pass_sort && g.c >= 12 && n >= 49152 && (n >> cbits) <= RX_FINE_MAX && n <= ((size_t)1 << (31 - (g.c - 1 - cbits)));
    {
        ZeroList zl{};
        int k = 0;
        zl.p[k] = chist; zl.words[k++] = (CLASS_HIST_COPIES + 1) * (HEAVY_T_MAX + 2);
        for (MsmGroup &gr : job->group) if (gr.nsets) {
            if (gr.heavy_counters.reserve(8 * MSM_MAX_SETS)) return ZKG_ERROR;
            zl.p[k] = gr.heavy_counters.as<uint32_t>(); zl.words[k++] = 2 * MSM_MAX_SETS;
        }
        if (two_pass) {
            const uint32_t nbins = g.W << cbits;
            if (job->rx_meta.reserve((2 * (size_t)nbins + g.W) * 4)) return ZKG_ERROR;
            zl.p[k] = job->rx_meta.as<uint32_t>(); zl.words[k++] = 2 * nbins + g.W;
        }
        const dim3 dg((unsigned)((n0 + 255) / 256));
        const bool four = !d_gather && (n0 & 3) == 0 && g0.w0 == 0 && g0.ws == 1 && g0.W == g0.Wt;
        const dim3 dg4((unsigned)((n0 / 4 + 255) / 256));
        if (job->multi > 1) {
            const dim3 dgm(dg.x, job->multi);
            if (g0.c == 16) hipLaunchKernelGGL(k_digits_multi<16>, dgm, dim3(256), 0, s, d_scalars, job->multi_stride, n0, (int)mont, job->merge, digits, zl);
            else if (g0.c == 12) hipLaunchKernelGGL(k_digits_multi<12>, dgm, dim3(256), 0, s, d_scalars, job->multi_stride, n0, (int)mont, job->merge, digits, zl);
            else hipLaunchKernelGGL(k_digits_multi_any, dgm, dim3(256), 0, s, d_scalars, job->multi_stride, n0, (int)mont, g0, job->merge, digits, zl);
        }
        else if (four && g0.c == 16) hipLaunchKernelGGL(k_digits_c4<16>, dg4, dim3(256), 0, s, d_scalars, n0, (int)mont, g0, digits, zl);
        else if (four && g0.c == 12) hipLaunchKernelGGL(k_digits_c4<12>, dg4, dim3(256), 0, s, d_scalars, n0, (int)mont, g0, digits, zl);
        else if (g0.c == 16) hipLaunchKernelGGL(k_digits_c<16>, dg, dim3(256), 0, s, d_scalars, d_gather, n0, (int)mont, g0, digits, zl);
        else if (g0.c == 12) hipLaunchKernelGGL(k_digits_c<12>, dg, dim3(256), 0, s, d_scalars, d_gather, n0, (int)mont, g0, digits, zl);
        else hipLaunchKernelGGL(k_digits, dg, dim3(256), 0, s, d_scalars, d_gather, n0, (int)mont, g0, digits, zl);
    }
    if (two_pass) {
        const uint32_t fbits = g.c - 1 - cbits, CB = 1u << cbits, nbins = g.W * CB, S1 = (uint32_t)((n + RX_SLICE - 1) / RX_SLICE);
        if (job->rx_tmp.reserve(n * g.W * 4)) return ZKG_ERROR;
        uint32_t *cnt = job->rx_meta.as<uint32_t>(), *cursor = cnt + nbins, *wtot = cursor + nbins, *tmp = job->rx_tmp.as<uint32_t>();
        const size_t fine_lds = (RX_FINE_MAX + 3 * (1u << fbits)) * 4;
        hipLaunchKernelGGL(k_rx_count, dim3(S1, g.W), dim3(1024), 0, s, digits, n, fbits, cbits, cnt, wtot);
        static const int wg_env = getenv("ZKG_SORT_WG") ? atoi(getenv("ZKG_SORT_WG")) : 0;
        const bool half = (wg_env ? wg_env == 512 : job->sort_stream != nullptr) && fbits <= 9;
        if (half) {
            const uint32_t S2 = (uint32_t)((n + 512 * RX_PER_THREAD - 1) / (512 * RX_PER_THREAD));
            hipLaunchKernelGGL(k_rx_scatter<512>, dim3(S2, g.W), dim3(512), (512 * RX_PER_THREAD + 4 * RX_MAX_CB + 8) * 4, s, digits, n, fbits, cbits, cnt, wtot, g.W, cursor, tmp, offsets + total);
            hipLaunchKernelGGL(k_rx_fine<512>, dim3(CB, g.W), dim3(512), fine_lds, s, tmp, fbits, cbits, g.B, cnt, wtot, counts, offsets, total, chist,
                               job->sorted.as<uint32_t>());
        } else {
            hipLaunchKernelGGL(k_rx_scatter<1024>, dim3(S1, g.W), dim3(1024), (RX_SLICE + 4 * RX_MAX_CB + 8) * 4, s, digits, n, fbits, cbits, cnt, wtot, g.W, cursor, tmp, offsets + total);
            hipLaunchKernelGGL(k_rx_fine<1024>, dim3(CB, g.W), dim3(1024), fine_lds, s, tmp, fbits, cbits, g.B, cnt, wtot, counts, offsets, total, chist,
                               job->sorted.as<uint32_t>());
        }
    } else {
    hipLaunchKernelGGL(k_hist, dim3(S, g.W), dim3(SORT_THREADS), g.B * 4, s, digits, n, g.B, S, slice_len, hist);
    hipLaunchKernelGGL(k_colscan, dim3((unsigned)((total + 255) / 256)), dim3(256), 0, s, hist, g.B, S, total, counts);
    hipLaunchKernelGGL(k_scan_blocks, dim3((unsigned)nblk), dim3(1024), 0, s, counts, offsets, sums, total);
    hipLaunchKernelGGL(k_scan_sums, dim3(1), dim3(1024), 0, s, sums, (uint32_t)nblk, offsets + total);
    hipLaunchKernelGGL(k_scan_apply, dim3((unsigned)nblk), dim3(1024), 0, s, offsets, sums, total);
    hipLaunchKernelGGL(k_place, dim3(S, g.W), dim3(SORT_THREADS), g.B * 4, s, digits, n, g.B, S, slice_len, hist, offsets, job->sorted.as<uint32_t>());
    hipLaunchKernelGGL(k_class_hist, dim3((unsigned)((total + 1023) / 1024)), dim3(1024), 0, s, counts, offsets, total, chist);
    }
    hipLaunchKernelGGL(k_order_place, dim3((unsigned)((total + 1023) / 1024)), dim3(1024), 0, s, counts, offsets, total, chist, chist + CLASS_HIST_COPIES * (HEAVY_T_MAX + 2), job->order.as<uint32_t>());
    if (hipGetLastError() != hipSuccess) { set_error("msm sort launch failed"); return ZKG_ERROR; }
    return ZKG_OK;
}

MsmJob *msm_job_create(hipStream_t s, bool own_stream, bool high_priority) {
    MsmJob *j = new MsmJob();
    j->stream = s;
    if (own_stream) {
        int prio_lo = 0, prio_hi = 0;
        (void)hipDeviceGetStreamPriorityRange(&prio_lo, &prio_hi);
        if (!hip_ok(hipStreamCreateWithPriority(&j->stream, hipStreamNonBlocking, high_priority ? prio_hi : prio_lo), "hipStreamCreate", __FILE__, __LINE__)) { delete j; return nullptr; }
        j->own_stream = true;
    }
    return j;
}
void msm_job_set_window(MsmJob *j, int c) { if (j) j->window_hint = c; }
bool crit_priority_enabled() { static const bool on = !(getenv("ZKG_CRIT_PRIO") && atoi(getenv("ZKG_CRIT_PRIO")) == 0); return on; }
void msm_job_set_critical(MsmJob *j, bool critical) { if (j) j->critical = critical && crit_priority_enabled(); }
void msm_job_set_row_merge(MsmJob *j, uint32_t f) { if (j) j->merge_hint = f ? f : 1; }
void msm_job_set_skewed(MsmJob *j, bool skewed) { if (j) j->one_pass_sort = skewed; }
void msm_job_set_window_subset(MsmJob *j, uint32_t w0, uint32_t ws) { if (j) { j->w0 = w0; j->ws = ws ? ws : 1; } }
hipStream_t msm_job_stream(MsmJob *j) { return j->stream; }
void msm_job_destroy(MsmJob *j) {
    if (!j) return;
    for (DevBuf *b : {&j->digits, &j->hist, &j->counts, &j->offsets, &j->scan_sums, &j->class_hist, &j->order, &j->sorted, &j->rx_tmp, &j->rx_meta}) b->release();
    for (auto &gr : j->group) gr.release();
    if (j->aux) { (void)hipStreamSynchronize(j->aux); (void)hipStreamDestroy(j->aux); }
    if (j->ev_fork) (void)hipEventDestroy(j->ev_fork);
    if (j->ev_join) (void)hipEventDestroy(j->ev_join);
    if (j->own_stream) (void)hipStreamDestroy(j->stream);
    delete j;
}

static MsmJob g_default_job;
static MsmJob g_piece_job;
static hipStream_t g_sort_hi = nullptr;

int msm_job_launch(MsmJob *job, const MsmBases *sets, int nsets, const uint32_t *d_scalars, size_t n, bool scalars_mont, const uint32_t *d_gather) {
    static const bool dbg = getenv("ZKG_DEBUG_TIMING") != nullptr;
    auto t0 = std::chrono::steady_clock::now();
    auto lap = [&](const char *w) { if (dbg) fprintf(stderr, "[zkg]     %-18s %8.3f ms\n", w, std::chrono::duration<float, std::milli>(std::chrono::steady_clock::now() - t0).count()); };
    if (n >= ((size_t)1 << 31) || nsets < 0 || nsets > MSM_MAX_SETS) { set_error("msm: bad size"); return ZKG_ERROR; }
    bool any_table = false;
    for (int i = 0; i < nsets; ++i) any_table = any_table || sets[i].level_stride != 0;
    for (int i = 0; i < nsets; ++i) if ((sets[i].level_stride != 0) != any_table) { set_error("msm: table and plain base sets cannot share a launch"); return ZKG_ERROR; }
    if (any_table && (job->w0 != 0 || job->ws != 1 || job->window_hint <= 0)) { set_error("msm: a table launch covers all windows at the table's window size"); return ZKG_ERROR; }
    job->g = pick_geom(n, job->window_hint, job->w0, job->ws); job->n = n;
    job->empty = false; job->multi = 1;
    MsmBases by_field[2][MSM_MAX_SETS];
    for (MsmGroup &gr : job->group) gr.nsets = 0;
    job->group[0].g2 = false; job->group[1].g2 = true;
    for (int i = 0; i < nsets; ++i) { MsmGroup &gr = job->group[sets[i].g2 ? 1 : 0]; by_field[sets[i].g2 ? 1 : 0][gr.nsets] = sets[i]; gr.out_index[gr.nsets] = gr.nsets; ++gr.nsets; }
    if (job->g.W == 0 || n == 0) { job->empty = true; return ZKG_OK; }
    if ((uint64_t)n * job->g.W >= ((uint64_t)1 << 32)) { set_error("msm: n * windows exceeds the 32-bit index space of the sorted list (n < 2^28)"); return ZKG_ERROR; }
    job->merge = 1;
    if (any_table && job->merge_hint > 1 && !d_gather && job->g.W % job->merge_hint == 0 && (uint64_t)n * job->merge_hint < ((uint64_t)1 << 31)) {
        bool ok = true;
        for (int i = 0; i < nsets; ++i) ok = ok && sets[i].level_stride == n && sets[i].index_sub == 0 && !sets[i].remap;
        if (ok) job->merge = job->merge_hint;
    }
    job->converted_aside = false;
    {
        MsmGroup &g1 = job->group[0];
        if (!any_table && !d_gather && g1.nsets == 1 && by_field[0][0].index_sub == 0 && !by_field[0][0].remap && !by_field[0][0].p29) {
            if (!job->aux && (hipStreamCreateWithFlags(&job->aux, hipStreamNonBlocking) != hipSuccess || hipEventCreateWithFlags(&job->ev_fork, hipEventDisableTiming) != hipSuccess ||
                              hipEventCreateWithFlags(&job->ev_join, hipEventDisableTiming) != hipSuccess)) { set_error("msm: side stream"); return ZKG_ERROR; }
            if (g1.bases29.reserve(n * sizeof(Rec64))) return ZKG_ERROR;
            ZK_HIP(hipEventRecord(job->ev_fork, job->stream));
            ZK_HIP(hipStreamWaitEvent(job->aux, job->ev_fork, 0));
            hipLaunchKernelGGL(k_bases_to29, dim3((unsigned)((n + 255) / 256)), dim3(256), 0, job->aux, reinterpret_cast<const Affine<Fq> *>(by_field[0][0].p), n, g1.bases29.as<Rec64>());
            ZK_HIP(hipEventRecord(job->ev_join, job->aux));
            job->converted_aside = true;
        }
    }
    auto fail = [&] { if (job->converted_aside) { (void)hipStreamSynchronize(job->aux); job->converted_aside = false; } return ZKG_ERROR; };
    if (sort_digits(job, d_scalars, scalars_mont, d_gather)) return fail();
    if (job->sort_stream && job->sort_stream != job->stream) {
        if (hipEventRecord(job->ev_sorted, job->sort_stream) != hipSuccess || hipStreamWaitEvent(job->stream, job->ev_sorted, 0) != hipSuccess) return fail();
    }
    if (job->merge > 1) {
        for (int k = 0; k < 2; ++k) for (int i = 0; i < job->group[k].nsets; ++i) by_field[k][i].level_stride *= job->merge;
    }
    lap("sort enqueued");
    const bool timed_field_g2 = job->group[0].nsets == 0;
    if (job->group[1].nsets && launch_accumulate<Fq2>(job, job->group[1], by_field[1], d_gather, job == &g_default_job && timed_field_g2)) return fail();
    if (job->group[0].nsets && launch_accumulate<Fq>(job, job->group[0], by_field[0], d_gather, job == &g_default_job || job == &g_piece_job)) return fail();
    lap("accum enqueued");
    return ZKG_OK;
}
bool msm_multi_supported(size_t n, int c, uint32_t count) {
    const MsmGeom g = pick_geom(n, c);
    return c > 0 && count >= 1 && n >= 1 && (uint64_t)n * g.W * count < ((uint64_t)1 << 31) &&
           ((uint64_t)g.W * g.B * count + 1024 * SCAN_ITEMS - 1) / (1024 * SCAN_ITEMS) <= 1024;
}
int msm_job_launch_multi(MsmJob *job, const MsmBases *sets, int nsets, const uint32_t *d_scalars, size_t n, size_t scalar_stride, uint32_t count, bool scalars_mont) {
    bool ok = job->w0 == 0 && job->ws == 1 && nsets >= 1 && nsets <= MSM_MAX_SETS && msm_multi_supported(n, job->window_hint, count);
    for (int i = 0; i < nsets && ok; ++i) ok = sets[i].level_stride != 0 && !sets[i].remap && sets[i].index_sub == 0;
    if (!ok) { set_error("msm: unsupported multi launch"); return ZKG_ERROR; }
    job->g = pick_geom(n, job->window_hint); job->n = n;
    job->empty = false; job->converted_aside = false;
    MsmBases by_field[2][MSM_MAX_SETS];
    for (MsmGroup &gr : job->group) gr.nsets = 0;
    job->group[0].g2 = false; job->group[1].g2 = true;
    for (int i = 0; i < nsets; ++i) { MsmGroup &gr = job->group[sets[i].g2 ? 1 : 0]; by_field[sets[i].g2 ? 1 : 0][gr.nsets] = sets[i]; gr.out_index[gr.nsets] = gr.nsets; ++gr.nsets; }
    job->merge = 1;
    if (job->merge_hint > 1 && job->g.W % job->merge_hint == 0) {
        bool m = true;
        for (int i = 0; i < nsets; ++i) m = m && sets[i].level_stride == n;
        if (m) job->merge = job->merge_hint;
    }
    job->multi = count; job->multi_stride = scalar_stride;
    if (sort_digits(job, d_scalars, scalars_mont, nullptr)) return ZKG_ERROR;
    for (int k = 0; k < 2; ++k) for (int i = 0; i < job->group[k].nsets; ++i) by_field[k][i].level_stride *= job->merge;
    if (job->group[1].nsets && launch_accumulate<Fq2>(job, job->group[1], by_field[1], nullptr, false)) return ZKG_ERROR;
    if (job->group[0].nsets && launch_accumulate<Fq>(job, job->group[0], by_field[0], nullptr, false)) return ZKG_ERROR;
    return ZKG_OK;
}
int msm_job_finish_multi(MsmJob *job, G1 *out_g1, G2 *out_g2) {
    ZK_HIP(hipStreamSynchronize(job->stream));
    const int n1 = job->group[0].nsets, n2 = job->group[1].nsets;
    host_parallel_for((int)job->multi, [&](int p) {
        for (int k = 0; k < n1; ++k) out_g1[p * n1 + k] = host_combine<Fq>(job, job->group[0], k, p);
        for (int k = 0; k < n2; ++k) out_g2[p * n2 + k] = host_combine<Fq2>(job, job->group[1], k, p);
    });
    return ZKG_OK;
}
int msm_job_finish(MsmJob *job, G1 *out_g1, G2 *out_g2) {
    static const bool dbg = getenv("ZKG_DEBUG_TIMING") != nullptr;
    const auto t0 = std::chrono::steady_clock::now();
    ZK_HIP(hipStreamSynchronize(job->stream));
    const auto t1 = std::chrono::steady_clock::now();
    struct Lap { bool on; std::chrono::steady_clock::time_point a, b; ~Lap() { if (on) fprintf(stderr, "[zkg]     job finish: waited %.3f ms, host combine %.3f ms\n", std::chrono::duration<float, std::milli>(b - a).count(), std::chrono::duration<float, std::milli>(std::chrono::steady_clock::now() - b).count()); } } lap_{dbg, t0, t1};
    for (int k = 0; k < job->group[0].nsets; ++k) out_g1[k] = job->empty ? G1::inf() : host_combine<Fq>(job, job->group[0], k);
    for (int k = 0; k < job->group[1].nsets; ++k) out_g2[k] = job->empty ? G2::inf() : host_combine<Fq2>(job, job->group[1], k);
    return ZKG_OK;
}

void msm_job_set_device_finish(MsmJob *j, bool on) { if (j) j->dev_finish = on; }
template <class F> static int finish_dev(MsmJob *job, const MsmGroup &gr, uint32_t *out) {
    const uint32_t vectors = job->multi > 1 ? job->multi : 1;
    if (job->empty) {
        const uint32_t count = vectors * (uint32_t)gr.nsets;
        hipLaunchKernelGGL(k_msm_store_inf<F>, dim3((count + 63) / 64), dim3(64), 0, job->stream, out, count);
    } else {
        if (!gr.table || gr.red_windows != vectors || gr.red_slots > COMBINE_MAX_SLOTS<F>) { set_error("msm_job_finish_dev: table sets only (a plain set's windows need the Horner doublings)"); return ZKG_ERROR; }
        launch_combine<F>(dim3(vectors, (unsigned)gr.nsets), job->stream, gr.red_out.as<XYZZ<F>>(), gr.cpw, gr.red_slots, gr.chunk_log, gr.red_stride, out);
    }
    if (hipGetLastError() != hipSuccess) { set_error("msm combine launch failed"); return ZKG_ERROR; }
    return ZKG_OK;
}
int msm_job_finish_dev(MsmJob *job, uint64_t *d_out) {
    const bool g2 = job->group[0].nsets == 0;
    const MsmGroup &gr = job->group[g2 ? 1 : 0];
    if (!job->dev_finish || (job->group[0].nsets && job->group[1].nsets) || gr.nsets < 1) { set_error("msm_job_finish_dev: a device-finish launch of G1 sets only, or of G2 sets only"); return ZKG_ERROR; }
    uint32_t *out = reinterpret_cast<uint32_t *>(d_out);
    return g2 ? finish_dev<Fq2>(job, gr, out) : finish_dev<Fq>(job, gr, out);
}
template <class F> static int combine_records(const uint64_t *records_jac, size_t cpw, int slots, int chunk_log, size_t vectors, uint64_t *out_jac) {
    constexpr size_t point_bytes = POINT_WORDS<F> * 4;
    const size_t count = vectors * cpw * (size_t)slots;
    ScopedDevBuf in, rec, out;
    if (in.reserve(count * point_bytes) || rec.reserve(count * sizeof(XYZZ<F>)) || out.reserve(vectors * point_bytes)) return ZKG_ERROR;
    ZK_HIP(hipMemcpy(in.p, records_jac, count * point_bytes, hipMemcpyHostToDevice));
    hipLaunchKernelGGL(k_jac_to_records<F>, dim3((unsigned)((count + 255) / 256)), dim3(256), 0, nullptr, in.as<uint32_t>(), count, rec.as<XYZZ<F>>());
    launch_combine<F>(dim3((unsigned)vectors, 1), nullptr, rec.as<XYZZ<F>>(), (uint32_t)cpw, slots, chunk_log, (size_t)0, out.as<uint32_t>());
    if (hipGetLastError() != hipSuccess) { set_error("msm combine launch failed"); return ZKG_ERROR; }
    ZK_HIP(hipMemcpy(out_jac, out.p, vectors * point_bytes, hipMemcpyDeviceToHost));
    return ZKG_OK;
}
int msm_combine_records(bool g2, const uint64_t *records_jac, size_t cpw, int slots, int chunk_log, size_t vectors, uint64_t *out_jac) {
    const bool args = records_jac && out_jac && cpw >= 1 && cpw <= ((size_t)1 << 16) && chunk_log >= 0 && chunk_log <= 24 && vectors >= 1 && vectors <= 1024;
    if (g2) {
        if (!args || slots != 2) { set_error("zkg_msm_combine_g2_gpu: bad argument (1 <= cpw <= 2^16, 0 <= chunk_log <= 24, 1 <= vectors <= 1024)"); return ZKG_ERROR; }
        return combine_records<Fq2>(records_jac, cpw, slots, chunk_log, vectors, out_jac);
    }
    if (!args || (slots != 2 && slots != 3)) { set_error("zkg_msm_combine_gpu: bad argument (1 <= cpw <= 2^16, slots 2 or 3, 0 <= chunk_log <= 24, 1 <= vectors <= 1024)"); return ZKG_ERROR; }
    return combine_records<Fq>(records_jac, cpw, slots, chunk_log, vectors, out_jac);
}
size_t msm_table_bucket_bytes(int c, bool g2) {
    const MsmGeom g = pick_geom(1, c);
    return (size_t)g.W * g.B * (g2 ? std::max(sizeof(XYZZ<Fq2>), sizeof(Bucket29)) : std::max(sizeof(XYZZ<Fq>), sizeof(Bucket29)));
}


int msm_shared(const G1Affine *const *d_g1_bases, int n_g1, const G2Affine *d_g2_bases, const uint32_t *d_scalars, size_t n,
               bool scalars_mont, G1 *out_g1, G2 *out_g2, hipStream_t s, uint32_t w0, uint32_t ws, bool mostly_bits) {
    if (n_g1 < 0 || n_g1 + (d_g2_bases ? 1 : 0) > MSM_MAX_SETS) { set_error("msm: too many base sets"); return ZKG_ERROR; }
    std::lock_guard<std::mutex> lk(g_default_job.mu);
    g_dominant_timer.new_call();
    g_default_job.stream = s; g_default_job.w0 = w0; g_default_job.ws = ws ? ws : 1; g_default_job.one_pass_sort = mostly_bits;
    MsmBases sets[MSM_MAX_SETS]; int nsets = 0;
    for (int i = 0; i < n_g1; ++i) { sets[nsets] = MsmBases(); sets[nsets].p = d_g1_bases[i]; ++nsets; }
    if (d_g2_bases) { sets[nsets] = MsmBases(); sets[nsets].p = d_g2_bases; sets[nsets].g2 = true; ++nsets; }
    if (n >= ((size_t)1 << 28)) { set_error("msm: at most 2^28 - 1 points per call"); return ZKG_ERROR; }
    const size_t PIECE = (size_t)1 << 23;
    if (n <= PIECE || w0 != 0 || g_default_job.ws != 1) {
        if (msm_job_launch(&g_default_job, sets, nsets, d_scalars, n, scalars_mont, nullptr)) return ZKG_ERROR;
        return msm_job_finish(&g_default_job, out_g1, out_g2);
    }
    G1 acc1[MSM_MAX_SETS]; G2 acc2[MSM_MAX_SETS];
    for (int i = 0; i < MSM_MAX_SETS; ++i) { acc1[i] = G1::inf(); acc2[i] = G2::inf(); }
    for (size_t lo = 0; lo < n; lo += PIECE) {
        const size_t cnt = std::min(PIECE, n - lo);
        MsmBases piece[MSM_MAX_SETS];
        for (int i = 0; i < nsets; ++i) { piece[i] = sets[i]; piece[i].p = (const char *)sets[i].p + lo * (sets[i].g2 ? sizeof(G2Affine) : sizeof(G1Affine)); }
        G1 p1[MSM_MAX_SETS]; G2 p2[MSM_MAX_SETS];
        if (msm_job_launch(&g_default_job, piece, nsets, d_scalars + 8 * lo, cnt, scalars_mont, nullptr) || msm_job_finish(&g_default_job, p1, p2)) return ZKG_ERROR;
        for (int i = 0; i < n_g1; ++i) acc1[i].add(p1[i]);
        if (d_g2_bases) acc2[0].add(p2[0]);
    }
    for (int i = 0; i < n_g1; ++i) out_g1[i] = acc1[i];
    if (d_g2_bases) out_g2[0] = acc2[0];
    return ZKG_OK;
}

int msm_g1_host_scalars(const G1Affine *d_bases, const uint32_t *h_scalars, size_t n, bool mont, G1 *out, hipStream_t s) {
    if (n >= ((size_t)1 << 28)) { set_error("msm: at most 2^28 - 1 points per call"); return ZKG_ERROR; }
    if (!n) { *out = G1::inf(); return ZKG_OK; }
    static const int max_pieces = getenv("ZKG_MSM_PIECES") ? std::max(1, std::min(8, atoi(getenv("ZKG_MSM_PIECES")))) : 4;
    const bool pieces = max_pieces > 1 && n >= ((size_t)1 << 19) && n <= ((size_t)1 << 23);
    if (n > ((size_t)1 << 23)) {
        ScopedDevBuf tmp;
        if (tmp.reserve(n * 32)) return ZKG_ERROR;
        ZK_HIP(hipMemcpyAsync(tmp.p, h_scalars, n * 32, hipMemcpyHostToDevice, s));
        return msm_g1(d_bases, tmp.as<uint32_t>(), n, mont, out, s, false);
    }
    MsmJob &J = g_default_job;
    std::lock_guard<std::mutex> lk(J.mu);
    g_dominant_timer.new_call();
    if (J.hs_scalars.reserve(n * 32)) return ZKG_ERROR;
    if (!J.copy) {
        if (hipStreamCreateWithFlags(&J.copy, hipStreamNonBlocking) != hipSuccess) { J.copy = nullptr; set_error("msm: copy stream"); return ZKG_ERROR; }
        for (auto &e : J.ev_piece) if (hipEventCreateWithFlags(&e, hipEventDisableTiming) != hipSuccess) { set_error("msm: event"); return ZKG_ERROR; }
    }
    uint32_t *d_sc = J.hs_scalars.as<uint32_t>();
    J.stream = s; J.w0 = 0; J.ws = 1; J.one_pass_sort = false;
    MsmBases set; set.p = d_bases;
    if (!pieces) {
        ZK_HIP(hipMemcpyAsync(d_sc, h_scalars, n * 32, hipMemcpyHostToDevice, s));
        if (msm_job_launch(&J, &set, 1, d_sc, n, mont, nullptr)) return ZKG_ERROR;
        return msm_job_finish(&J, out, nullptr);
    }
    size_t cut[9]; int P = max_pieces;
    cut[P] = n;
    for (int k = P - 1; k >= 1; --k) cut[k] = (cut[k + 1] / 2) & ~(size_t)255;
    cut[0] = 0;
    if (const char *e = getenv("ZKG_MSM_CUTS")) {
        int k = 1; const char *q = e;
        while (*q && k < 8) { const long v = strtol(q, const_cast<char **>(&q), 10); if (v <= 0 || v >= 64) break; cut[k++] = (n * (size_t)v / 64) & ~(size_t)255; if (*q == ',') ++q; }
        if (k > 1) { P = k; cut[P] = n; for (int i = 1; i < P; ++i) if (cut[i] < cut[i - 1]) cut[i] = cut[i - 1]; }
    }
    for (int k = 0; k < P; ++k) {
        ZK_HIP(hipMemcpyAsync(d_sc + 8 * cut[k], h_scalars + 8 * cut[k], (cut[k + 1] - cut[k]) * 32, hipMemcpyHostToDevice, J.copy));
        ZK_HIP(hipEventRecord(J.ev_piece[k], J.copy));
    }
    MsmJob &K = g_piece_job;
    if (!g_sort_hi) {
        int lo = 0, hi = 0; (void)hipDeviceGetStreamPriorityRange(&lo, &hi);
        bool ok = hipStreamCreateWithPriority(&g_sort_hi, hipStreamNonBlocking, hi) == hipSuccess;
        for (MsmJob *w : {&J, &K}) ok = ok && hipEventCreateWithFlags(&w->ev_sorted, hipEventDisableTiming) == hipSuccess && hipEventCreateWithFlags(&w->ev_acc_done, hipEventDisableTiming) == hipSuccess;
        if (!ok) { g_sort_hi = nullptr; set_error("msm: sort stream"); return ZKG_ERROR; }
    }
    hipStream_t s_hi = g_sort_hi;
    if (!J.aux && (hipStreamCreateWithFlags(&J.aux, hipStreamNonBlocking) != hipSuccess || hipEventCreateWithFlags(&J.ev_fork, hipEventDisableTiming) != hipSuccess ||
                   hipEventCreateWithFlags(&J.ev_join, hipEventDisableTiming) != hipSuccess)) { set_error("msm: side stream"); return ZKG_ERROR; }
    if (J.group[0].bases29.reserve(n * sizeof(Rec64))) return ZKG_ERROR;
    ZK_HIP(hipEventRecord(J.ev_fork, s));
    ZK_HIP(hipStreamWaitEvent(J.aux, J.ev_fork, 0));
    hipLaunchKernelGGL(k_bases_to29, dim3((unsigned)((n + 255) / 256)), dim3(256), 0, J.aux, reinterpret_cast<const Affine<Fq> *>(d_bases), n, J.group[0].bases29.as<Rec64>());
    ZK_HIP(hipEventRecord(J.ev_join, J.aux));
    ZK_HIP(hipStreamWaitEvent(s, J.ev_join, 0));
    ZK_HIP(hipStreamWaitEvent(s_hi, J.ev_fork, 0));
    const int c = (int)pick_geom(n, J.window_hint).c;
    const int saved_hint = J.window_hint, saved_hint_k = K.window_hint;
    J.window_hint = c; K.window_hint = c; K.bucket_owner = &J; K.w0 = 0; K.ws = 1; K.one_pass_sort = false; K.stream = s;
    int rc = ZKG_OK; bool started = false; bool used[2] = {false, false};
    for (int k = 0; k < P && rc == ZKG_OK; ++k) {
        if (cut[k + 1] == cut[k] && k + 1 < P) continue;
        const int which = (P - 1 - k) & 1;
        MsmJob &W = which ? K : J;
        MsmBases piece = set; piece.p = reinterpret_cast<const char *>(d_bases) + cut[k] * sizeof(G1Affine);
        piece.p29 = J.group[0].bases29.as<Rec64>() + cut[k];
        W.resume = started; W.defer_reduce = k + 1 < P; started = true;
        W.sort_stream = s_hi;
        if (hipStreamWaitEvent(s_hi, J.ev_piece[k], 0) != hipSuccess) { rc = ZKG_ERROR; break; }
        if (used[which] && hipStreamWaitEvent(s_hi, W.ev_acc_done, 0) != hipSuccess) { rc = ZKG_ERROR; break; }
        rc = msm_job_launch(&W, &piece, 1, d_sc + 8 * cut[k], cut[k + 1] - cut[k], mont, nullptr);
        if (rc == ZKG_OK && hipEventRecord(W.ev_acc_done, s) != hipSuccess) rc = ZKG_ERROR;
        used[which] = true;
    }
    J.resume = false; J.defer_reduce = false; J.window_hint = saved_hint; J.sort_stream = nullptr;
    K.resume = false; K.defer_reduce = false; K.window_hint = saved_hint_k; K.bucket_owner = nullptr; K.sort_stream = nullptr; K.stream = nullptr;
    if (rc != ZKG_OK) { (void)hipStreamSynchronize(J.copy); (void)hipStreamSynchronize(s_hi); (void)hipStreamSynchronize(s); return ZKG_ERROR; }
    return msm_job_finish(&J, out, nullptr);
}

int msm_g1(const G1Affine *d_bases, const uint32_t *d_scalars, size_t n, bool mont, G1 *out, hipStream_t s, bool mostly_bits) {
    return msm_shared(&d_bases, 1, nullptr, d_scalars, n, mont, out, nullptr, s, 0, 1, mostly_bits);
}
int msm_g2(const G2Affine *d_bases, const uint32_t *d_scalars, size_t n, bool mont, G2 *out, hipStream_t s, bool mostly_bits) {
    return msm_shared(nullptr, 0, d_bases, d_scalars, n, mont, nullptr, out, s, 0, 1, mostly_bits);
}

template <class F>
static int window_table_build_t(WindowTable &t, const Affine<F> *d_bases, size_t n, int c, hipStream_t s) {
    t.n = n; t.c = c; t.W = (SCALAR_BITS + c - 1) / c; t.g2 = sizeof(F) != sizeof(Fq);
    if (t.buf.reserve(std::max<size_t>(1, n) * t.W * sizeof(Affine<F>))) return ZKG_ERROR;
    if (!n) return ZKG_OK;
    Affine<F> *lv = t.buf.as<Affine<F>>();
    ZK_HIP(hipMemcpyAsync(lv, d_bases, n * sizeof(Affine<F>), hipMemcpyDeviceToDevice, s));
    constexpr int K = sizeof(F) != sizeof(Fq) ? 2 : 4;
    for (int w = 1; w < t.W; w += K)
        hipLaunchKernelGGL((k_table_levels<F, K>), dim3((unsigned)((n + 255) / 256)), dim3(256), 0, s, lv + (size_t)(w - 1) * n, lv + (size_t)w * n, n, (uint32_t)c,
                           std::min(K, t.W - w));
    if (hipGetLastError() != hipSuccess) { set_error("window table launch failed"); return ZKG_ERROR; }
    return ZKG_OK;
}
int window_table_build_g1(WindowTable &t, const G1Affine *d_bases, size_t n, int c, hipStream_t s) { return window_table_build_t<Fq>(t, d_bases, n, c, s); }
int window_table_records29(WindowTable &t, hipStream_t s) {
    if (t.g2) { set_error("window_table_records29: G1 tables only"); return ZKG_ERROR; }
    const size_t total = t.n * (size_t)t.W;
    if (t.rec29.reserve(std::max<size_t>(1, total) * sizeof(Rec64))) return ZKG_ERROR;
    if (total) hipLaunchKernelGGL(k_bases_to29, dim3((unsigned)((total + 255) / 256)), dim3(256), 0, s, t.buf.as<Affine<Fq>>(), total, t.rec29.as<Rec64>());
    if (hipGetLastError() != hipSuccess) { set_error("window table records launch failed"); return ZKG_ERROR; }
    return ZKG_OK;
}
int window_table_build_g2(WindowTable &t, const G2Affine *d_bases, size_t n, int c, hipStream_t s) { return window_table_build_t<Fq2>(t, d_bases, n, c, s); }

int witness_classify(const Fr *d_z, size_t n1, uint8_t *d_tags, uint32_t *d_listed, uint32_t *d_count, hipStream_t s, const uint32_t *d_subset_pos) {
    ZK_HIP(hipMemsetAsync(d_count, 0, 8, s));
    if (n1) hipLaunchKernelGGL(k_classify, dim3((unsigned)((n1 + 255) / 256)), dim3(256), 0, s, d_z, n1, d_tags, d_listed, d_count, d_subset_pos);
    return hipGetLastError() == hipSuccess ? ZKG_OK : ZKG_ERROR;
}
template <class F> static int gather_points_t(const Affine<F> *d_src, const uint32_t *d_idx, size_t count, uint32_t index_sub, Affine<F> *d_out, hipStream_t s) {
    if (count) hipLaunchKernelGGL(k_gather_points<F>, dim3((unsigned)((count + 255) / 256)), dim3(256), 0, s, d_src, d_idx, count, index_sub, d_out);
    return hipGetLastError() == hipSuccess ? ZKG_OK : ZKG_ERROR;
}
int gather_points_g1(const G1Affine *d_src, const uint32_t *d_idx, size_t count, uint32_t index_sub, G1Affine *d_out, hipStream_t s) { return gather_points_t<Fq>(d_src, d_idx, count, index_sub, d_out, s); }
int gather_points_g2(const G2Affine *d_src, const uint32_t *d_idx, size_t count, uint32_t index_sub, G2Affine *d_out, hipStream_t s) { return gather_points_t<Fq2>(d_src, d_idx, count, index_sub, d_out, s); }
template <class F> static int scatter_points_t(const Affine<F> *d_src, const uint32_t *d_idx, size_t count, Affine<F> *d_out, hipStream_t s) {
    if (count) hipLaunchKernelGGL(k_scatter_points<F>, dim3((unsigned)((count + 255) / 256)), dim3(256), 0, s, d_src, d_idx, count, d_out);
    return hipGetLastError() == hipSuccess ? ZKG_OK : ZKG_ERROR;
}
int scatter_points_g1(const G1Affine *d_src, const uint32_t *d_idx, size_t count, G1Affine *d_out, hipStream_t s) { return scatter_points_t<Fq>(d_src, d_idx, count, d_out, s); }
int scatter_points_g2(const G2Affine *d_src, const uint32_t *d_idx, size_t count, G2Affine *d_out, hipStream_t s) { return scatter_points_t<Fq2>(d_src, d_idx, count, d_out, s); }
template <class F>
static int ones_sum_launch_t(OnesSum &o, const MsmBases *sets, int nsets, const uint8_t *d_tags, size_t n1, hipStream_t s, size_t tag_stride = 0, uint32_t vecs = 1) {
    if (nsets < 1 || nsets > MSM_MAX_SETS) { set_error("ones-sum: bad set count"); return ZKG_ERROR; }
    const uint32_t span = (uint32_t)std::min<size_t>(8192, std::max<size_t>(1024, ((n1 + 255) / 256 + 255) / 256 * 256));
    const unsigned blocks = (unsigned)std::max<size_t>(1, (n1 + span - 1) / span);
    o.g2 = sizeof(F) != sizeof(Fq); o.nsets = nsets;
    const size_t vec_stride = (size_t)nsets * (blocks + 1), host_bytes = std::max<size_t>(MSM_MAX_SETS, (size_t)vecs * nsets) * sizeof(G2);
    if (o.partials.reserve(vecs * vec_stride * sizeof(XYZZ<F>))) return ZKG_ERROR;
    if (o.host_bytes < host_bytes) {
        if (o.host) (void)hipHostFree(o.host);
        o.host = nullptr; o.host_bytes = 0;
        if (!hip_ok(hipHostMalloc(&o.host, host_bytes, hipHostMallocDefault), "hipHostMalloc", __FILE__, __LINE__)) return ZKG_ERROR;
        o.host_bytes = host_bytes;
    }
    XYZZ<F> *part = o.partials.as<XYZZ<F>>();
    ViewSet<F> views;
    for (int i = 0; i < MSM_MAX_SETS; ++i) { const MsmBases &b = sets[i < nsets ? i : 0]; views.v[i] = BaseView<F>{reinterpret_cast<const Affine<F> *>(b.p), 0, nullptr, b.index_sub, 1, nullptr}; }
    hipLaunchKernelGGL(k_ones_sum<F>, dim3(blocks, (unsigned)nsets, vecs), dim3(256), 256 * sizeof(LdsPoint<F>) + (size_t)span * 4, s, views, d_tags, n1, span, part, tag_stride, vec_stride);
    hipLaunchKernelGGL(k_sum_partials<F>, dim3((unsigned)nsets, vecs), dim3(256), 256 * sizeof(LdsPoint<F>), s, part, blocks, vec_stride);
    if (hipGetLastError() != hipSuccess) { set_error("ones-sum launch failed"); return ZKG_ERROR; }
    if (vecs > 1) {
        ZK_HIP(hipMemcpy2DAsync(o.host, sizeof(XYZZ<F>), part + blocks, (blocks + 1) * sizeof(XYZZ<F>), sizeof(XYZZ<F>), (size_t)vecs * nsets, hipMemcpyDeviceToHost, s));
        return ZKG_OK;
    }
    for (int i = 0; i < nsets; ++i)
        ZK_HIP(hipMemcpyAsync((char *)o.host + (size_t)i * sizeof(XYZZ<F>), part + (size_t)i * (blocks + 1) + blocks, sizeof(XYZZ<F>), hipMemcpyDeviceToHost, s));
    return ZKG_OK;
}
int ones_sum_launch(OnesSum &o, const MsmBases *sets, int nsets, const uint8_t *d_tags, size_t n1, hipStream_t s) {
    for (int i = 1; i < nsets; ++i) if (sets[i].g2 != sets[0].g2) { set_error("ones-sum: one field per launch"); return ZKG_ERROR; }
    return sets[0].g2 ? ones_sum_launch_t<Fq2>(o, sets, nsets, d_tags, n1, s) : ones_sum_launch_t<Fq>(o, sets, nsets, d_tags, n1, s);
}
int ones_sum_launch_multi(OnesSum &o, const MsmBases *sets, int nsets, const uint8_t *d_tags, size_t tag_stride, size_t n1, uint32_t count, hipStream_t s) {
    for (int i = 1; i < nsets; ++i) if (sets[i].g2 != sets[0].g2) { set_error("ones-sum: one field per launch"); return ZKG_ERROR; }
    if (count < 1 || count > 65535) { set_error("ones-sum: bad witness count"); return ZKG_ERROR; }
    return sets[0].g2 ? ones_sum_launch_t<Fq2>(o, sets, nsets, d_tags, n1, s, tag_stride, count) : ones_sum_launch_t<Fq>(o, sets, nsets, d_tags, n1, s, tag_stride, count);
}
void OnesSum::release() { partials.release(); if (host) (void)hipHostFree(host); host = nullptr; host_bytes = 0; }

static constexpr int FB_WINDOWS = 32, FB_DIGITS = 255, FB_K = 4;
template <class F>
__global__ __launch_bounds__(256) void k_fixed_table(const Affine<F> *rows , Affine<F> *table) {
    const uint32_t t = blockIdx.x * blockDim.x + threadIdx.x;
    if (t >= FB_WINDOWS * FB_DIGITS) return;
    const uint32_t j = t / FB_DIGITS, d = t % FB_DIGITS + 1;
    const Affine<F> r = rows[j];
    XYZZ<F> acc = XYZZ<F>::inf();
    for (int bit = 7; bit >= 0; --bit) { acc = acc.dbl(); if ((d >> bit) & 1u) acc.madd(r); }
    XYZZ<F> fin = acc;
    table[t] = fin.to_affine().normalized();
}
template <class F>
__global__ __launch_bounds__(256) void k_fixed_base(const Affine<F> *table, const uint32_t *scalars, size_t n, int mont, Affine<F> *out) {
    const size_t lane = (size_t)blockIdx.x * blockDim.x + threadIdx.x, i0 = lane * FB_K;
    if (i0 >= n) return;
    F x[FB_K], y[FB_K], zz[FB_K], zzz[FB_K];
#pragma unroll
    for (int k = 0; k < FB_K; ++k) {
        XYZZ<F> acc = XYZZ<F>::inf();
        if (i0 + k < n) {
            Fr f;
            for (int j = 0; j < 8; ++j) f.v[j] = scalars[8 * (i0 + k) + j];
            if (mont) f = f.from_mont();
            else f = f.normalized();
            for (int j = 0; j < FB_WINDOWS; ++j) {
                const uint32_t d = (f.v[j >> 2] >> (8 * (j & 3))) & 255u;
                if (d) acc.madd(table[j * FB_DIGITS + d - 1]);
            }
        }
        x[k] = acc.x; y[k] = acc.y; zz[k] = acc.zz; zzz[k] = acc.zzz;
    }
    F pre[FB_K], run = F::one();
#pragma unroll
    for (int k = 0; k < FB_K; ++k) { pre[k] = run; if (!zzz[k].is_zero()) run = run * zzz[k]; }
    F inv = inverse_fast(run);
#pragma unroll
    for (int k = FB_K - 1; k >= 0; --k) {
        if (i0 + k >= n) continue;
        if (zzz[k].is_zero()) { out[i0 + k] = Affine<F>::inf(); continue; }
        F zi = inv * pre[k];
        inv = inv * zzz[k];
        F t = zi * zz[k];
        F zi2 = t.sqr();
        out[i0 + k] = Affine<F>{x[k] * zi2, y[k] * zi}.normalized();
    }
}

template <class F> struct FixedTableCache { std::mutex mu; std::vector<std::pair<Affine<F>, DevBuf>> entries; };
template <class F> static FixedTableCache<F> &fixed_cache() { static FixedTableCache<F> c; return c; }
template <class F>
static const Affine<F> *fixed_table_for(const Affine<F> &base, hipStream_t s) {
    FixedTableCache<F> &c = fixed_cache<F>();
    std::lock_guard<std::mutex> lk(c.mu);
    for (auto &e : c.entries) if (memcmp(&e.first, &base, sizeof(base)) == 0) return e.second.template as<Affine<F>>();
    std::vector<Affine<F>> rows(FB_WINDOWS);
    XYZZ<F> cur = XYZZ<F>::from_affine(base);
    for (int j = 0; j < FB_WINDOWS; ++j) { rows[j] = cur.to_affine(); for (int k = 0; k < 8; ++k) cur = cur.dbl(); }
    DevBuf d_rows, d_table;
    if (d_rows.reserve(rows.size() * sizeof(Affine<F>)) || d_table.reserve((size_t)FB_WINDOWS * FB_DIGITS * sizeof(Affine<F>))) return nullptr;
    if (!hip_ok(hipMemcpyAsync(d_rows.p, rows.data(), rows.size() * sizeof(Affine<F>), hipMemcpyHostToDevice, s), "H2D", __FILE__, __LINE__)) return nullptr;
    hipLaunchKernelGGL(k_fixed_table<F>, dim3((FB_WINDOWS * FB_DIGITS + 255) / 256), dim3(256), 0, s, d_rows.as<Affine<F>>(), d_table.as<Affine<F>>());
    const bool ok = hipGetLastError() == hipSuccess && hip_ok(hipStreamSynchronize(s), "sync", __FILE__, __LINE__);
    d_rows.release();
    if (!ok) { d_table.release(); set_error("fixed-base table build failed"); return nullptr; }
    c.entries.emplace_back(base, d_table);
    return c.entries.back().second.template as<Affine<F>>();
}
template <class F>
static int fixed_base(const Affine<F> &base, const uint32_t *d_scalars, size_t n, Affine<F> *d_out, hipStream_t s, bool mont) {
    const Affine<F> *table = fixed_table_for<F>(base, s);
    if (!table) return ZKG_ERROR;
    const size_t lanes = (n + FB_K - 1) / FB_K;
    if (n) hipLaunchKernelGGL(k_fixed_base<F>, dim3((unsigned)((lanes + 255) / 256)), dim3(256), 0, s, table, d_scalars, n, (int)mont, d_out);
    hipError_t e = hipGetLastError();
    ZK_HIP(hipStreamSynchronize(s));
    if (e != hipSuccess) { set_error("fixed_base launch failed"); return ZKG_ERROR; }
    return ZKG_OK;
}
int fixed_base_g1(const G1Affine &base, const uint32_t *d_scalars, size_t n, G1Affine *d_out, hipStream_t s, bool mont) { return fixed_base<Fq>(base, d_scalars, n, d_out, s, mont); }
int fixed_base_g2(const G2Affine &base, const uint32_t *d_scalars, size_t n, G2Affine *d_out, hipStream_t s, bool mont) { return fixed_base<Fq2>(base, d_scalars, n, d_out, s, mont); }
static void fixed_tables_release() {
    { auto &c = fixed_cache<Fq>(); std::lock_guard<std::mutex> lk(c.mu); for (auto &e : c.entries) e.second.release(); c.entries.clear(); }
    { auto &c = fixed_cache<Fq2>(); std::lock_guard<std::mutex> lk(c.mu); for (auto &e : c.entries) e.second.release(); c.entries.clear(); }
}

int msm_configure() {
    bool ok = hipFuncSetAttribute((const void *)k_bucket_reduce<Fq2, RED_L_LOG_SMALL>, hipFuncAttributeMaxDynamicSharedMemorySize, 2 * RedGeom<Fq2>::LANES * (int)sizeof(LdsPoint<Fq2>)) == hipSuccess;
    ok = ok && hipFuncSetAttribute((const void *)k_bucket_reduce<Fq2, RED_L_LOG_TINY>, hipFuncAttributeMaxDynamicSharedMemorySize, 2 * RedGeom<Fq2>::LANES * (int)sizeof(LdsPoint<Fq2>)) == hipSuccess;
    ok = ok && hipFuncSetAttribute((const void *)k_bucket_reduce<Fq2, RED_L_LOG_LARGE>, hipFuncAttributeMaxDynamicSharedMemorySize, 2 * RedGeom<Fq2>::LANES * (int)sizeof(LdsPoint<Fq2>)) == hipSuccess;
    ok = ok && hipFuncSetAttribute((const void *)k_heavy_parts<Fq2>, hipFuncAttributeMaxDynamicSharedMemorySize, 256 * (int)sizeof(LdsPoint<Fq2>)) == hipSuccess;
    ok = ok && hipFuncSetAttribute((const void *)k_heavy_merge<Fq2>, hipFuncAttributeMaxDynamicSharedMemorySize, 256 * (int)sizeof(LdsPoint<Fq2>)) == hipSuccess;
    ok = ok && hipFuncSetAttribute((const void *)k_bucket_fold<Fq2>, hipFuncAttributeMaxDynamicSharedMemorySize, (int)FOLD_THREADS * (int)sizeof(LdsPoint<Fq2>)) == hipSuccess;
    ok = ok && hipFuncSetAttribute((const void *)k_ones_sum<Fq2>, hipFuncAttributeMaxDynamicSharedMemorySize, 256 * (int)sizeof(LdsPoint<Fq2>) + 8192 * 4) == hipSuccess;
    ok = ok && hipFuncSetAttribute((const void *)k_ones_sum<Fq>, hipFuncAttributeMaxDynamicSharedMemorySize, 256 * (int)sizeof(LdsPoint<Fq>) + 8192 * 4) == hipSuccess;
    ok = ok && hipFuncSetAttribute((const void *)k_sum_partials<Fq2>, hipFuncAttributeMaxDynamicSharedMemorySize, 256 * (int)sizeof(LdsPoint<Fq2>)) == hipSuccess;
    ok = ok && hipFuncSetAttribute((const void *)k_hist, hipFuncAttributeMaxDynamicSharedMemorySize, (1 << (MAX_C - 1)) * 4) == hipSuccess;
    ok = ok && hipFuncSetAttribute((const void *)k_place, hipFuncAttributeMaxDynamicSharedMemorySize, (1 << (MAX_C - 1)) * 4) == hipSuccess;
    ok = ok && hipFuncSetAttribute((const void *)k_bucket_reduce29l, hipFuncAttributeMaxDynamicSharedMemorySize, 4 * RedGeom<Fq>::LANES * (int)sizeof(LdsPoint29)) == hipSuccess;
    ok = ok && hipFuncSetAttribute((const void *)k_rx_scatter<1024>, hipFuncAttributeMaxDynamicSharedMemorySize, (RX_SLICE + 4 * RX_MAX_CB + 8) * 4) == hipSuccess;
    ok = ok && hipFuncSetAttribute((const void *)k_rx_scatter<512>, hipFuncAttributeMaxDynamicSharedMemorySize, (512 * RX_PER_THREAD + 4 * RX_MAX_CB + 8) * 4) == hipSuccess;
    ok = ok && hipFuncSetAttribute((const void *)k_rx_fine<1024>, hipFuncAttributeMaxDynamicSharedMemorySize, (RX_FINE_MAX + 3 * 1024) * 4) == hipSuccess;
    ok = ok && hipFuncSetAttribute((const void *)k_rx_fine<512>, hipFuncAttributeMaxDynamicSharedMemorySize, (RX_FINE_MAX + 3 * 1024) * 4) == hipSuccess;
    return ok ? ZKG_OK : ZKG_ERROR;
}
void msm_release_all() {
    fixed_tables_release();
    MsmJob &j = g_default_job;
    std::lock_guard<std::mutex> lk(j.mu);
    for (DevBuf *b : {&j.digits, &j.hist, &j.counts, &j.offsets, &j.scan_sums, &j.class_hist, &j.order, &j.sorted, &j.rx_tmp, &j.rx_meta}) b->release();
    for (auto &gr : j.group) gr.release();
    if (j.aux) { (void)hipStreamSynchronize(j.aux); (void)hipStreamDestroy(j.aux); j.aux = nullptr; }
    j.hs_scalars.release();
    {
        MsmJob &k = g_piece_job;
        if (g_sort_hi) { (void)hipStreamSynchronize(g_sort_hi); (void)hipStreamDestroy(g_sort_hi); g_sort_hi = nullptr; }
        for (DevBuf *b : {&k.digits, &k.hist, &k.counts, &k.offsets, &k.scan_sums, &k.class_hist, &k.order, &k.sorted, &k.rx_tmp, &k.rx_meta}) b->release();
        for (auto &gr : k.group) gr.release();
        if (k.aux) { (void)hipStreamSynchronize(k.aux); (void)hipStreamDestroy(k.aux); k.aux = nullptr; }
        if (k.ev_fork) { (void)hipEventDestroy(k.ev_fork); k.ev_fork = nullptr; }
        if (k.ev_join) { (void)hipEventDestroy(k.ev_join); k.ev_join = nullptr; }
        for (MsmJob *w : {&j, &k}) {
            if (w->ev_sorted) { (void)hipEventDestroy(w->ev_sorted); w->ev_sorted = nullptr; }
            if (w->ev_acc_done) { (void)hipEventDestroy(w->ev_acc_done); w->ev_acc_done = nullptr; }
        }
        k.stream = nullptr;
    }
    if (j.copy) { (void)hipStreamSynchronize(j.copy); (void)hipStreamDestroy(j.copy); j.copy = nullptr; }
    for (auto &e : j.ev_piece) if (e) { (void)hipEventDestroy(e); e = nullptr; }
    if (j.ev_fork) { (void)hipEventDestroy(j.ev_fork); j.ev_fork = nullptr; }
    if (j.ev_join) { (void)hipEventDestroy(j.ev_join); j.ev_join = nullptr; }
}

}
```

Measured before the change: 57.81.

## Skip heavy-bucket kernels per piece when sort reports no heavy buckets

Splits the MSM launch into separate sort and accumulate enqueue steps. In the pipelined host-scalars path it reads back a heavy-bucket count from the sort (via pinned memory) and skips the heavy_parts/heavy_merge kernels when it is zero. It also removes the unconditional stream wait on the bases-to-29 conversion. The host now blocks on each piece's sort event before enqueueing accumulation. That adds CPU-GPU synchronization that may stall the pipeline, in exchange for dropping two kernel launches per piece. Stats for pieces and waits are exposed through a new API.

```diff
diff --git a/include/zkg.h b/include/zkg.h
--- a/include/zkg.h
+++ b/include/zkg.h
@@ -86,6 +86,7 @@
 int zkg_msm_g2_dev(const void *d_bases, const void *d_scalars, size_t n, int scalars_mont,
                    uint64_t out_jac[24], void *stream);
 int zkg_msm_g1_host_scalars(const void *d_bases, const uint64_t *scalars, size_t n, int scalars_mont, uint64_t out_jac[12], void *stream);
+int zkg_msm_host_scalars_stats(uint32_t *out, int n);
 typedef struct zkg_msm_bases zkg_msm_bases;
 zkg_msm_bases *zkg_msm_g1_bases_upload(const void *d_bases, size_t n);
 int zkg_msm_g1_resident(zkg_msm_bases *bases, const void *d_scalars, size_t n, int scalars_mont, uint64_t out_jac[12], void *stream);
diff --git a/zklaim_amd/__init__.py b/zklaim_amd/__init__.py
--- a/zklaim_amd/__init__.py
+++ b/zklaim_amd/__init__.py
@@ -1,7 +1,7 @@
 from .api import (ZkgError, device_info, evaluation_domain_size, fixed_base_g1_dev, fixed_base_g2_dev, g1_sum, g2_sum, init, lib, msm_g1, msm_g1_dev, msm_g1_windows_dev,
                   msm_g2, msm_g2_dev, ntt, ntt_dev, shutdown, timing_dominant_ms, timing_reset, Crs, PK, R1CS, make_r1cs, make_pk,
                   DECLARED_SYMBOLS, ZklaimCircuit, ZklaimCtx, make_ctx, zklaim_input_map, OPS, Keypair, groth16_verify, groth16_verify_batch, verify_batch_stats, groth16_prove_batch, prove_batch_stats, groth16_prove_batch_dev, prove_dev_stats, groth16_prove_batch_zklaim, zklaim_witness_stats, zklaim_witness_size, zklaim_witness_mirror, zklaim_witness_gpu, zklaim_witness_mirror_parallel, zklaim_witness_gpu_parallel, prove_zklaim_stats, pairing_product, pairing_probe, pairing_selfcheck,
-                  libsnark_trusted_setup, libsnark_prove, libsnark_verify, zklaim_prove_batch, zklaim_verify_batch, zklaim_verify_batch_stats, proof_decode_gpu, zklaim_input_sums_gpu, zklaim_input_map_mirror, ctx_blob, COMPAT_SYMBOLS, field_op, fr29_op, FR29_OPS, fq29_op, FQ29_OPS, g1_add_quad29, g1_add_pair29, curve_op, CURVE_OPS, OK, ERROR, UNSATISFIED, init_multi, MsmShards, pk_blob_inspect, ResidentBases, msm_g1_host_scalars, msm_resident_async_stats, msm_combine_gpu, ResidentBasesG2, msm_combine_g2_gpu,
+                  libsnark_trusted_setup, libsnark_prove, libsnark_verify, zklaim_prove_batch, zklaim_verify_batch, zklaim_verify_batch_stats, proof_decode_gpu, zklaim_input_sums_gpu, zklaim_input_map_mirror, ctx_blob, COMPAT_SYMBOLS, field_op, fr29_op, FR29_OPS, fq29_op, FQ29_OPS, g1_add_quad29, g1_add_pair29, curve_op, CURVE_OPS, OK, ERROR, UNSATISFIED, init_multi, MsmShards, pk_blob_inspect, ResidentBases, msm_g1_host_scalars, msm_host_scalars_stats, msm_resident_async_stats, msm_combine_gpu, ResidentBasesG2, msm_combine_g2_gpu,
                   groth16_verify_each, verify_each_stats, verify_each_set_chunk, pairing_each, final_exp, fq12_op, FQ12_OPS,
                   point_decompress, point_compress, zklaim_verify_each, zklaim_verify_each_stats, zklaim_ic_each,
                   Domain, domain_stats, Qap, qap_stats, qap_instance_stats)
diff --git a/zklaim_amd/api.py b/zklaim_amd/api.py
--- a/zklaim_amd/api.py
+++ b/zklaim_amd/api.py
@@ -36,6 +36,7 @@
     "zkg_qap_new", "zkg_qap_free", "zkg_qap_domain_size", "zkg_qap_num_variables", "zkg_qap_batch_max", "zkg_qap_set_batch_max",
     "zkg_qap_witness_h_async", "zkg_qap_stats",
     "zkg_qap_instance_async", "zkg_qap_set_column_segment", "zkg_qap_instance_stats", "zkg_groth16_setup_dev",
+    "zkg_msm_host_scalars_stats",
 ]
 COMPAT_SYMBOLS = ["libsnark_trusted_setup", "libsnark_prove", "libsnark_verify"]
 
@@ -408,6 +409,17 @@
     lib().zkg_msm_g1_host_scalars.argtypes = [C.c_void_p, C.c_void_p, C.c_size_t, C.c_int, C.c_void_p, C.c_void_p]
     _check(lib().zkg_msm_g1_host_scalars(_vp(d_bases), _vp(scalars_host_ptr), C.c_size_t(n), SCALARS_MONT if scalars_mont else 0, _p(out), _vp(stream)), "zkg_msm_g1_host_scalars")
     return out
+
+
+def msm_host_scalars_stats():
+    out = (C.c_uint32 * 18)()
+    words = lib().zkg_msm_host_scalars_stats(out, 18)
+    if words < 2:
+        return None
+    pieces = int(out[0])
+    return {"pieces": pieces, "stream_waits": int(out[1]),
+            "heavy": [None if out[2 + 2 * k] == 0xFFFFFFFF else int(out[2 + 2 * k]) for k in range(pieces)],
+            "pair": [bool(out[3 + 2 * k]) for k in range(pieces)]}
 
 
 class _ResidentBases:
diff --git a/zklaim_amd/csrc/capi.hip b/zklaim_amd/csrc/capi.hip
--- a/zklaim_amd/csrc/capi.hip
+++ b/zklaim_amd/csrc/capi.hip
@@ -759,6 +759,7 @@
     store_norm(out_jac, r);
     return ZKG_OK;
 }
+int zkg_msm_host_scalars_stats(uint32_t *out, int n) { return out && n >= 0 ? msm_host_scalars_stats(out, n) : 0; }
 int zkg_msm_g1_windows_dev(const void *d_bases, const void *d_scalars, size_t n, int scalars_mont, unsigned first_window, unsigned window_stride,
                            uint64_t out_jac[12], void *stream) {
     REQUIRE_INIT();
diff --git a/zklaim_amd/csrc/common.hpp b/zklaim_amd/csrc/common.hpp
--- a/zklaim_amd/csrc/common.hpp
+++ b/zklaim_amd/csrc/common.hpp
@@ -164,6 +164,7 @@
 int msm_g1(const G1Affine *d_bases, const uint32_t *d_scalars, size_t n, bool scalars_mont, G1 *out, hipStream_t s, bool mostly_bits = false);
 int msm_g2(const G2Affine *d_bases, const uint32_t *d_scalars, size_t n, bool scalars_mont, G2 *out, hipStream_t s, bool mostly_bits = false);
 int msm_g1_host_scalars(const G1Affine *d_bases, const uint32_t *h_scalars, size_t n, bool scalars_mont, G1 *out, hipStream_t s);
+int msm_host_scalars_stats(uint32_t *out, int n);
 int msm_shared(const G1Affine *const *d_g1_bases, int n_g1, const G2Affine *d_g2_bases, const uint32_t *d_scalars, size_t n,
                bool scalars_mont, G1 *out_g1, G2 *out_g2, hipStream_t s, uint32_t w0 = 0, uint32_t ws = 1,
                bool mostly_bits = false);
diff --git a/zklaim_amd/csrc/msm.hip b/zklaim_amd/csrc/msm.hip
--- a/zklaim_amd/csrc/msm.hip
+++ b/zklaim_amd/csrc/msm.hip
@@ -522,7 +522,7 @@
     for (uint32_t i = t; i < nc; i += 1024) if (h[i]) atomicAdd(&class_hist[i], h[i]);
 }
 __global__ __launch_bounds__(1024) void k_order_place(const uint32_t *counts, const uint32_t *offsets, size_t total, const uint32_t *class_hist, uint32_t *class_cursor,
-                                                       uint32_t *order) {
+                                                       uint32_t *order, uint32_t *heavy_out) {
     sort_wave_priority();
     __shared__ uint32_t h[HEAVY_T_MAX + 2], first[HEAVY_T_MAX + 2], wave_total[16], threshold;
     const uint32_t t = threadIdx.x, wave = t >> 6, lane = t & 63;
@@ -540,6 +540,7 @@
             if (2 * t < nc) v0 += copy[nc - 1 - 2 * t];
             if (2 * t + 1 < nc) v1 += copy[nc - 2 - 2 * t];
         }
+        if (heavy_out && blockIdx.x == 0 && t == 0) *heavy_out = v0;
         incl = v0 + v1;
         for (uint32_t d = 1; d < 64; d <<= 1) { const uint32_t y = __shfl_up(incl, d, 64); if (lane >= d) incl += y; }
     }
@@ -1186,11 +1187,13 @@
     bool dev_finish = false;
     uint32_t multi = 1; size_t multi_stride = 0;
     DevBuf hs_scalars; hipStream_t copy = nullptr; hipEvent_t ev_piece[8] = {nullptr};
+    uint32_t *heavy_words = nullptr, *heavy_out = nullptr;
+    uint32_t stream_waits = 0;
     std::mutex mu;
 };
 
 template <class F>
-static int launch_accumulate(MsmJob *job, MsmGroup &gr, const MsmBases *sets, const uint32_t *d_gather, bool time_it) {
+static int launch_accumulate(MsmJob *job, MsmGroup &gr, const MsmBases *sets, const uint32_t *d_gather, bool time_it, bool heavy_pair = true ) {
     const MsmGeom g = job->g; const size_t n = job->n, total_buckets = (size_t)g.W * g.B; const unsigned ns = (unsigned)gr.nsets;
     const uint32_t P = job->multi, BP = g.B * P, Wp = g.W / P;
     hipStream_t s = job->stream;
@@ -1228,6 +1231,7 @@
             if (sets[0].p29) rec29 = reinterpret_cast<const Rec64 *>(sets[0].p29);
             else {
                 ZK_HIP(hipStreamWaitEvent(s, job->ev_join, 0));
+                ++job->stream_waits;
                 rec29 = gr.bases29.as<Rec64>();
             }
         } else if (ns == 1 && !d_gather && sets[0].p29 && !sets[0].remap && sets[0].index_sub == 0) {
@@ -1258,10 +1262,12 @@
                            views, job->sorted.as<uint32_t>(), job->offsets.as<uint32_t>(), job->order.as<uint32_t>(), lanes, buckets,
                            gr.heavy_items.as<HeavyItem>(), gr.heavy_buckets.as<HeavyBucket>(), gr.heavy_counters.as<uint32_t>(), L);
     if (time_it) g_dominant_timer.end(s);
+    if (heavy_pair) {
     hipLaunchKernelGGL(k_heavy_parts<F>, dim3(HEAVY_PART_BLOCKS, ns), dim3(256), 256 * sizeof(LdsPoint<F>), s,
                        views, job->sorted.as<uint32_t>(), gr.heavy_items.as<HeavyItem>(), gr.heavy_counters.as<uint32_t>(), gr.heavy_partials.as<XYZZ<F>>(), buckets, L, (int)out29);
     hipLaunchKernelGGL(k_heavy_merge<F>, dim3(HEAVY_MERGE_BLOCKS, ns), dim3(256), 256 * sizeof(LdsPoint<F>), s,
                        gr.heavy_buckets.as<HeavyBucket>(), gr.heavy_counters.as<uint32_t>(), gr.heavy_partials.as<XYZZ<F>>(), buckets, L, (int)out29, resume);
+    }
     if (job->defer_reduce) {
         if (hipGetLastError() != hipSuccess) { set_error("msm kernel launch failed"); return ZKG_ERROR; }
         return ZKG_OK;
@@ -1510,7 +1516,7 @@
     hipLaunchKernelGGL(k_place, dim3(S, g.W), dim3(SORT_THREADS), g.B * 4, s, digits, n, g.B, S, slice_len, hist, offsets, job->sorted.as<uint32_t>());
     hipLaunchKernelGGL(k_class_hist, dim3((unsigned)((total + 1023) / 1024)), dim3(1024), 0, s, counts, offsets, total, chist);
     }
-    hipLaunchKernelGGL(k_order_place, dim3((unsigned)((total + 1023) / 1024)), dim3(1024), 0, s, counts, offsets, total, chist, chist + CLASS_HIST_COPIES * (HEAVY_T_MAX + 2), job->order.as<uint32_t>());
+    hipLaunchKernelGGL(k_order_place, dim3((unsigned)((total + 1023) / 1024)), dim3(1024), 0, s, counts, offsets, total, chist, chist + CLASS_HIST_COPIES * (HEAVY_T_MAX + 2), job->order.as<uint32_t>(), job->heavy_out);
     if (hipGetLastError() != hipSuccess) { set_error("msm sort launch failed"); return ZKG_ERROR; }
     return ZKG_OK;
 }
@@ -1547,11 +1553,16 @@
 static MsmJob g_default_job;
 static MsmJob g_piece_job;
 static hipStream_t g_sort_hi = nullptr;
-
-int msm_job_launch(MsmJob *job, const MsmBases *sets, int nsets, const uint32_t *d_scalars, size_t n, bool scalars_mont, const uint32_t *d_gather) {
-    static const bool dbg = getenv("ZKG_DEBUG_TIMING") != nullptr;
-    auto t0 = std::chrono::steady_clock::now();
-    auto lap = [&](const char *w) { if (dbg) fprintf(stderr, "[zkg]     %-18s %8.3f ms\n", w, std::chrono::duration<float, std::milli>(std::chrono::steady_clock::now() - t0).count()); };
+struct HostScalarsStats { uint32_t pieces = 0, waits = 0, heavy[8] = {0}, pair[8] = {0}; };
+static HostScalarsStats g_hs_stats;
+
+struct MsmLaunchSets { MsmBases by_field[2][MSM_MAX_SETS]; };
+static int msm_launch_failed(MsmJob *job) {
+    if (job->converted_aside) { (void)hipStreamSynchronize(job->aux); job->converted_aside = false; }
+    return ZKG_ERROR;
+}
+static int msm_job_enqueue_sort(MsmJob *job, const MsmBases *sets, int nsets, const uint32_t *d_scalars, size_t n, bool scalars_mont, const uint32_t *d_gather, MsmLaunchSets &ls) {
+    auto &by_field = ls.by_field;
     if (n >= ((size_t)1 << 31) || nsets < 0 || nsets > MSM_MAX_SETS) { set_error("msm: bad size"); return ZKG_ERROR; }
     bool any_table = false;
     for (int i = 0; i < nsets; ++i) any_table = any_table || sets[i].level_stride != 0;
@@ -1559,7 +1570,6 @@
     if (any_table && (job->w0 != 0 || job->ws != 1 || job->window_hint <= 0)) { set_error("msm: a table launch covers all windows at the table's window size"); return ZKG_ERROR; }
     job->g = pick_geom(n, job->window_hint, job->w0, job->ws); job->n = n;
     job->empty = false; job->multi = 1;
-    MsmBases by_field[2][MSM_MAX_SETS];
     for (MsmGroup &gr : job->group) gr.nsets = 0;
     job->group[0].g2 = false; job->group[1].g2 = true;
     for (int i = 0; i < nsets; ++i) { MsmGroup &gr = job->group[sets[i].g2 ? 1 : 0]; by_field[sets[i].g2 ? 1 : 0][gr.nsets] = sets[i]; gr.out_index[gr.nsets] = gr.nsets; ++gr.nsets; }
@@ -1585,18 +1595,32 @@
             job->converted_aside = true;
         }
     }
-    auto fail = [&] { if (job->converted_aside) { (void)hipStreamSynchronize(job->aux); job->converted_aside = false; } return ZKG_ERROR; };
-    if (sort_digits(job, d_scalars, scalars_mont, d_gather)) return fail();
-    if (job->sort_stream && job->sort_stream != job->stream) {
-        if (hipEventRecord(job->ev_sorted, job->sort_stream) != hipSuccess || hipStreamWaitEvent(job->stream, job->ev_sorted, 0) != hipSuccess) return fail();
-    }
+    if (sort_digits(job, d_scalars, scalars_mont, d_gather)) return msm_launch_failed(job);
+    if (job->sort_stream && job->sort_stream != job->stream && hipEventRecord(job->ev_sorted, job->sort_stream) != hipSuccess) return msm_launch_failed(job);
     if (job->merge > 1) {
         for (int k = 0; k < 2; ++k) for (int i = 0; i < job->group[k].nsets; ++i) by_field[k][i].level_stride *= job->merge;
     }
+    return ZKG_OK;
+}
+static int msm_job_enqueue_accumulate(MsmJob *job, MsmLaunchSets &ls, const uint32_t *d_gather, bool heavy_pair) {
+    if (job->empty) return ZKG_OK;
+    const bool timed_field_g2 = job->group[0].nsets == 0;
+    if (job->group[1].nsets && launch_accumulate<Fq2>(job, job->group[1], ls.by_field[1], d_gather, job == &g_default_job && timed_field_g2, heavy_pair)) return msm_launch_failed(job);
+    if (job->group[0].nsets && launch_accumulate<Fq>(job, job->group[0], ls.by_field[0], d_gather, job == &g_default_job || job == &g_piece_job, heavy_pair)) return msm_launch_failed(job);
+    return ZKG_OK;
+}
+int msm_job_launch(MsmJob *job, const MsmBases *sets, int nsets, const uint32_t *d_scalars, size_t n, bool scalars_mont, const uint32_t *d_gather) {
+    static const bool dbg = getenv("ZKG_DEBUG_TIMING") != nullptr;
+    auto t0 = std::chrono::steady_clock::now();
+    auto lap = [&](const char *w) { if (dbg) fprintf(stderr, "[zkg]     %-18s %8.3f ms\n", w, std::chrono::duration<float, std::milli>(std::chrono::steady_clock::now() - t0).count()); };
+    MsmLaunchSets ls;
+    if (msm_job_enqueue_sort(job, sets, nsets, d_scalars, n, scalars_mont, d_gather, ls)) return ZKG_ERROR;
+    if (!job->empty && job->sort_stream && job->sort_stream != job->stream) {
+        if (hipStreamWaitEvent(job->stream, job->ev_sorted, 0) != hipSuccess) return msm_launch_failed(job);
+        ++job->stream_waits;
+    }
     lap("sort enqueued");
-    const bool timed_field_g2 = job->group[0].nsets == 0;
-    if (job->group[1].nsets && launch_accumulate<Fq2>(job, job->group[1], by_field[1], d_gather, job == &g_default_job && timed_field_g2)) return fail();
-    if (job->group[0].nsets && launch_accumulate<Fq>(job, job->group[0], by_field[0], d_gather, job == &g_default_job || job == &g_piece_job)) return fail();
+    if (msm_job_enqueue_accumulate(job, ls, d_gather, true)) return ZKG_ERROR;
     lap("accum enqueued");
     return ZKG_OK;
 }
@@ -1748,11 +1772,14 @@
     uint32_t *d_sc = J.hs_scalars.as<uint32_t>();
     J.stream = s; J.w0 = 0; J.ws = 1; J.one_pass_sort = false;
     MsmBases set; set.p = d_bases;
+    g_hs_stats = HostScalarsStats(); J.stream_waits = 0; g_piece_job.stream_waits = 0;
     if (!pieces) {
         ZK_HIP(hipMemcpyAsync(d_sc, h_scalars, n * 32, hipMemcpyHostToDevice, s));
         if (msm_job_launch(&J, &set, 1, d_sc, n, mont, nullptr)) return ZKG_ERROR;
+        g_hs_stats.pieces = 1; g_hs_stats.waits = J.stream_waits; g_hs_stats.heavy[0] = 0xffffffffu; g_hs_stats.pair[0] = 1;
         return msm_job_finish(&J, out, nullptr);
     }
+    if (!J.heavy_words && hipHostMalloc(reinterpret_cast<void **>(&J.heavy_words), 8 * sizeof(uint32_t), hipHostMallocDefault) != hipSuccess) { J.heavy_words = nullptr; set_error("msm: pinned words"); return ZKG_ERROR; }
     size_t cut[9]; int P = max_pieces;
     cut[P] = n;
     for (int k = P - 1; k >= 1; --k) cut[k] = (cut[k + 1] / 2) & ~(size_t)255;
@@ -1781,30 +1808,57 @@
     ZK_HIP(hipStreamWaitEvent(J.aux, J.ev_fork, 0));
     hipLaunchKernelGGL(k_bases_to29, dim3((unsigned)((n + 255) / 256)), dim3(256), 0, J.aux, reinterpret_cast<const Affine<Fq> *>(d_bases), n, J.group[0].bases29.as<Rec64>());
     ZK_HIP(hipEventRecord(J.ev_join, J.aux));
-    ZK_HIP(hipStreamWaitEvent(s, J.ev_join, 0));
     ZK_HIP(hipStreamWaitEvent(s_hi, J.ev_fork, 0));
     const int c = (int)pick_geom(n, J.window_hint).c;
     const int saved_hint = J.window_hint, saved_hint_k = K.window_hint;
     J.window_hint = c; K.window_hint = c; K.bucket_owner = &J; K.w0 = 0; K.ws = 1; K.one_pass_sort = false; K.stream = s;
-    int rc = ZKG_OK; bool started = false; bool used[2] = {false, false};
-    for (int k = 0; k < P && rc == ZKG_OK; ++k) {
-        if (cut[k + 1] == cut[k] && k + 1 < P) continue;
-        const int which = (P - 1 - k) & 1;
-        MsmJob &W = which ? K : J;
+    int run[8], R = 0;
+    for (int k = 0; k < P; ++k) if (cut[k + 1] != cut[k] || k + 1 == P) run[R++] = k;
+    MsmLaunchSets ls[2];
+    int rc = ZKG_OK; bool used[2] = {false, false};
+    auto job_of = [&](int i) -> MsmJob & { return ((R - 1 - i) & 1) ? K : J; };
+    auto enqueue_sort = [&](int i) {
+        const int k = run[i], which = (R - 1 - i) & 1;
+        MsmJob &W = job_of(i);
         MsmBases piece = set; piece.p = reinterpret_cast<const char *>(d_bases) + cut[k] * sizeof(G1Affine);
         piece.p29 = J.group[0].bases29.as<Rec64>() + cut[k];
-        W.resume = started; W.defer_reduce = k + 1 < P; started = true;
-        W.sort_stream = s_hi;
-        if (hipStreamWaitEvent(s_hi, J.ev_piece[k], 0) != hipSuccess) { rc = ZKG_ERROR; break; }
-        if (used[which] && hipStreamWaitEvent(s_hi, W.ev_acc_done, 0) != hipSuccess) { rc = ZKG_ERROR; break; }
-        rc = msm_job_launch(&W, &piece, 1, d_sc + 8 * cut[k], cut[k + 1] - cut[k], mont, nullptr);
+        W.sort_stream = s_hi; W.heavy_out = J.heavy_words + i;
+        if (hipStreamWaitEvent(s_hi, J.ev_piece[k], 0) != hipSuccess) return ZKG_ERROR;
+        if (used[which] && hipStreamWaitEvent(s_hi, W.ev_acc_done, 0) != hipSuccess) return ZKG_ERROR;
+        return msm_job_enqueue_sort(&W, &piece, 1, d_sc + 8 * cut[k], cut[k + 1] - cut[k], mont, nullptr, ls[which]);
+    };
+    rc = enqueue_sort(0);
+    for (int i = 0; i < R && rc == ZKG_OK; ++i) {
+        const int which = (R - 1 - i) & 1;
+        MsmJob &W = job_of(i);
+        if (i + 1 < R && (rc = enqueue_sort(i + 1)) != ZKG_OK) break;
+        if (i == 0 && hipEventSynchronize(J.ev_join) != hipSuccess) { rc = ZKG_ERROR; break; }
+        uint32_t heavy = 0;
+        if (!W.empty) {
+            if (hipEventSynchronize(W.ev_sorted) != hipSuccess) { rc = ZKG_ERROR; break; }
+            heavy = *static_cast<volatile const uint32_t *>(J.heavy_words + i);
+        }
+        W.resume = i > 0; W.defer_reduce = i + 1 < R;
+        rc = msm_job_enqueue_accumulate(&W, ls[which], nullptr, heavy != 0);
         if (rc == ZKG_OK && hipEventRecord(W.ev_acc_done, s) != hipSuccess) rc = ZKG_ERROR;
         used[which] = true;
-    }
-    J.resume = false; J.defer_reduce = false; J.window_hint = saved_hint; J.sort_stream = nullptr;
-    K.resume = false; K.defer_reduce = false; K.window_hint = saved_hint_k; K.bucket_owner = nullptr; K.sort_stream = nullptr; K.stream = nullptr;
-    if (rc != ZKG_OK) { (void)hipStreamSynchronize(J.copy); (void)hipStreamSynchronize(s_hi); (void)hipStreamSynchronize(s); return ZKG_ERROR; }
+        g_hs_stats.heavy[i] = heavy; g_hs_stats.pair[i] = heavy != 0; g_hs_stats.pieces = (uint32_t)(i + 1);
+    }
+    g_hs_stats.waits = J.stream_waits + K.stream_waits;
+    J.resume = false; J.defer_reduce = false; J.window_hint = saved_hint; J.sort_stream = nullptr; J.heavy_out = nullptr;
+    K.resume = false; K.defer_reduce = false; K.window_hint = saved_hint_k; K.bucket_owner = nullptr; K.sort_stream = nullptr; K.stream = nullptr; K.heavy_out = nullptr;
+    if (rc != ZKG_OK) { (void)hipStreamSynchronize(J.copy); (void)hipStreamSynchronize(J.aux); (void)hipStreamSynchronize(s_hi); (void)hipStreamSynchronize(s); return ZKG_ERROR; }
     return msm_job_finish(&J, out, nullptr);
+}
+int msm_host_scalars_stats(uint32_t *out, int n) {
+    std::lock_guard<std::mutex> lk(g_default_job.mu);
+    const HostScalarsStats &st = g_hs_stats;
+    if (!st.pieces) return 0;
+    uint32_t rec[2 + 2 * 8] = {st.pieces, st.waits};
+    for (uint32_t k = 0; k < st.pieces; ++k) { rec[2 + 2 * k] = st.heavy[k]; rec[3 + 2 * k] = st.pair[k]; }
+    const int words = 2 + 2 * (int)st.pieces;
+    for (int i = 0; i < words && i < n; ++i) out[i] = rec[i];
+    return words;
 }
 
 int msm_g1(const G1Affine *d_bases, const uint32_t *d_scalars, size_t n, bool mont, G1 *out, hipStream_t s, bool mostly_bits) {
@@ -2024,6 +2078,7 @@
     }
     if (j.copy) { (void)hipStreamSynchronize(j.copy); (void)hipStreamDestroy(j.copy); j.copy = nullptr; }
     for (auto &e : j.ev_piece) if (e) { (void)hipEventDestroy(e); e = nullptr; }
+    if (j.heavy_words) { (void)hipHostFree(j.heavy_words); j.heavy_words = nullptr; }
     if (j.ev_fork) { (void)hipEventDestroy(j.ev_fork); j.ev_fork = nullptr; }
     if (j.ev_join) { (void)hipEventDestroy(j.ev_join); j.ev_join = nullptr; }
 }
```

New measurement: 58.93, median of 6. 1.02x the previous value.
